# Xharlie/pointnerf

Hardware: AMD Instinct MI355X
Metric: rays/sec (render+bwd) NeRF-synth lego 800^2, K=8, 128 samp/ray (higher is better)
Workload: dtype f32 in / out / accumulate; forward GEMM operands as 2 x f16 planes (22-bit) on the f16 MFMA, 3 products per multiply-add; input-gradient GEMMs: f16 leading product + e4m3 cross terms (csrc/mixq.h), 2 product equivalents; weight-gradient GEMM operands as one f16 plane each

## Files before the change

include/pnerf.h:

```cpp
#ifndef PNERF_H
#define PNERF_H
#include <stddef.h>
#include <stdint.h>

#ifdef __cplusplus
extern "C" {
#endif

#define PNERF_E_INVAL   (-1)
#define PNERF_E_WS      (-2)
#define PNERF_E_LAUNCH  (-3)
#define PNERF_E_UNSUP   (-4)

#define PNERF_MAX_K 16

typedef struct pnerf_grid_params {
    float ranges[6];
    float vsize[3];
    int32_t vdim[3];
    int32_t kernel_size[3];
    int32_t query_size[3];
    int32_t P;
    int32_t max_o;
    float radius;
} pnerf_grid_params;

enum { PNERF_GI_N_IN_GRID = 0, PNERF_GI_N_OCC = 1, PNERF_GI_MAX_CNT = 2, PNERF_GI_CELL0 = 3,
       PNERF_GI_FIRST_IDX = 4, PNERF_GI_OSTART_OFF = 5 , PNERF_GI_LEN = 8 };

int pnerf_version(void);
const char *pnerf_arch(void);

size_t pnerf_grid_workspace_bytes(const pnerf_grid_params *gp, int n_points);
int pnerf_grid_build(const pnerf_grid_params *gp, const float *d_xyz, int n_points,
                     void *d_grid_ws, size_t ws_bytes, void *stream);
int pnerf_grid_info(const void *d_grid_ws, int32_t *host_info, void *stream);
int pnerf_points_minmax(const float *d_xyz, int64_t n_points, float *d_out6, void *stream);

size_t pnerf_query_workspace_bytes(int R, int SR);
int pnerf_query(const pnerf_grid_params *gp, const void *d_grid_ws,
                const float *d_raypos,
                const float *campos3_host, const float *d_raydir, const float *d_mid,
                float near_depth, float far_depth, float jitter, uint64_t seed,
                int R, int D, int SR, int K,
                float *d_sample_loc, int32_t *d_sample_pidx, int32_t *d_sample_nn,
                int32_t *d_ray_hit, int32_t *d_valid_list, int32_t *d_counters,
                void *d_query_ws, size_t ws_bytes, void *stream);

int pnerf_gather_rows(const float *d_src, int n_src, int width, const int32_t *d_idx, int64_t n_idx,
                      float *d_dst, void *stream);
int pnerf_scatter_add_rows(const float *d_grad_rows, const int32_t *d_idx, int64_t n_idx, int width,
                           float *d_grad_src, int n_src, void *stream);

int pnerf_zero_one_blocks(int64_t n_idx);
int pnerf_zero_one_forward(const float *d_conf, int n_points, const int32_t *d_idx, int64_t n_idx, float eps,
                           float *d_partial, void *stream);
int pnerf_zero_one_backward(const float *d_conf, int n_points, const int32_t *d_idx, int64_t n_idx, float eps,
                            const float *d_gscale, float *d_grad_conf, void *stream);
int pnerf_zero_one_forward_rays(const float *d_conf, int n_points, const int32_t *d_idx, const int32_t *d_ray_hit, int R, int slots_per_ray, float eps,
                                float *d_partial, void *stream);
int pnerf_zero_one_backward_rays(const float *d_conf, int n_points, const int32_t *d_idx, const int32_t *d_ray_hit, int R, int slots_per_ray, float eps,
                                 const float *d_gscale, float *d_grad_conf, void *stream);
int pnerf_color_loss_blocks(int R);
int pnerf_color_loss_forward_rays(const float *d_ray_color, const float *d_gt, const int32_t *d_ray_hit, int R, float *d_partial, void *stream);
int pnerf_color_loss_backward_rays(const float *d_ray_color, const float *d_gt, const int32_t *d_ray_hit, int R, const float *d_gscale,
                                   float *d_grad_ray_color, void *stream);


#define PNERF_MLP_NTENSORS 18
int pnerf_mlp_layout(int feat_dim, int64_t *offsets );
size_t pnerf_mlp_packed_bytes(void);
int pnerf_mlp_pack(const float *d_params, void *d_packed, void *stream);

typedef struct pnerf_camera {
    float campos[3];
    float camrot[9];
    float rw2c[9];
    float vsize_z;
    int32_t raydist_mode_unit;
    float bg[3];
    int32_t has_bg;
} pnerf_camera;

typedef struct pnerf_points {
    const float *xyz;
    const float *embedding;
    const float *conf;
    const float *dir;
    const float *color;
    int32_t n, feat_dim;
} pnerf_points;

typedef struct pnerf_point_grads {
    float *embedding, *conf, *dir, *color;
    void *ready_event;
    const float *zero_one_gscale;
    float zero_one_eps;
    float *xyz;
} pnerf_point_grads;

size_t pnerf_agg_saved_bytes(int64_t n_valid_samples, int K);
size_t pnerf_agg_workspace_bytes(int64_t n_valid_max, int K);
size_t pnerf_render_backward_workspace_bytes(int R, int SR);

int pnerf_render_forward(const pnerf_camera *cam, const pnerf_points *pts, const void *d_packed_mlp,
                         const float *d_params, const float *d_raydir, const float *d_sample_loc, const int32_t *d_sample_pidx,
                         const int32_t *d_sample_nn, const int32_t *d_valid_list, const int32_t *d_counters,
                         int R, int SR, int K,
                         float *d_decoded, float *d_weight, float *d_ray_color, float *d_opacity,
                         float *d_bg_trans, float *d_blend_w,
                         void *d_saved, int64_t n_valid_max, void *d_ws, size_t ws_bytes, void *stream);

int pnerf_set_inference_products(int n);

int pnerf_set_wgrad_planes(int n);
int pnerf_set_cross_terms(int bits);
int pnerf_set_cross_terms_where(int mask);

int pnerf_render_backward(const pnerf_camera *cam, const pnerf_points *pts, const void *d_packed_mlp,
                          const float *d_params,
                          const float *d_raydir, const float *d_sample_loc, const int32_t *d_sample_pidx,
                          const int32_t *d_sample_nn, const int32_t *d_valid_list, const int32_t *d_counters,
                          int R, int SR, int K, int64_t n_valid,
                          const float *d_decoded, const float *d_weight, const float *d_opacity,
                          const float *d_grad_ray_color,
                          void *d_saved, float *d_grad_params, const pnerf_point_grads *pg,
                          void *d_ws, size_t ws_bytes, void *stream);


size_t pnerf_compact_workspace_bytes(int64_t n);
int pnerf_touched_flags(const int32_t *d_pidx, int64_t n, int32_t n_points, int32_t *d_flags, void *stream);
int pnerf_compact_valid(const int32_t *d_nn, int64_t n, int32_t *d_list, int32_t *d_counters, void *d_ws, size_t ws_bytes, void *stream);

int pnerf_agg_forward(const pnerf_camera *cam, const pnerf_points *pts, const void *d_packed_mlp, const float *d_params,
                      const float *d_raydir, const float *d_sample_loc, const float *d_xyz_pers, const float *d_loc_pers,
                      const int32_t *d_sample_pidx, const int32_t *d_valid_list, const int32_t *d_counters,
                      int R, int SR, int K, float *d_decoded, float *d_weight,
                      void *d_saved, int64_t n_valid_max, void *d_ws, size_t ws_bytes, void *stream);
int pnerf_agg_backward(const pnerf_camera *cam, const pnerf_points *pts, const void *d_packed_mlp, const float *d_params,
                       const float *d_raydir, const float *d_sample_loc, const int32_t *d_sample_pidx,
                       const int32_t *d_valid_list, const int32_t *d_counters, int R, int SR, int K, int64_t n_valid,
                       const float *d_decoded, const float *d_weight, const float *d_grad_decoded,
                       void *d_saved, float *d_grad_params, const pnerf_point_grads *pg, void *d_ws, size_t ws_bytes, void *stream);

int pnerf_raymarch_forward(const float *d_ray_dist, const uint8_t *d_ray_valid, const float *d_features, const float *bg3_host,
                           int R, int SR, float *d_ray_color, float *d_opacity, float *d_acc_trans, float *d_blend_w,
                           float *d_bg_trans, void *stream);
int pnerf_raymarch_backward(const float *d_ray_dist, const uint8_t *d_ray_valid, const float *d_features, const float *bg3_host,
                            int R, int SR, const float *d_grad_ray_color, float *d_grad_features, void *stream);

int pnerf_adam_step(float *d_param, const float *d_grad, float *d_exp_avg, float *d_exp_avg_sq, int64_t n,
                    double lr, double beta1, double beta2, double eps, int64_t step, void *stream);
typedef struct pnerf_adam_tensor {
    float *param; const float *grad; float *exp_avg; float *exp_avg_sq;
    int64_t n; double lr; int64_t step;
} pnerf_adam_tensor;
int pnerf_adam_step_multi(const pnerf_adam_tensor *tensors, int count, double beta1, double beta2, double eps, void *stream);

size_t pnerf_voxel_downsample_workspace_bytes(int64_t n_points, int rx, int ry, int rz);
int pnerf_voxel_downsample(const float *d_xyz, int64_t n_points, const float *space_min3_host, const float *vox_size3_host,
                           int rx, int ry, int rz, float *d_centroid, int32_t *d_grid_idx, int64_t *d_min_idx, int32_t *d_counts,
                           void *d_ws, size_t ws_bytes, void *stream);

#define PNERF_EX2D_MAX_VIEWS 8
#define PNERF_EX2D_MAX_MAPS 32
typedef struct pnerf_view_desc {
    float c2w[16];
    float w2c[16];
    float intrinsic[9];
    int32_t has_w2c;
} pnerf_view_desc;
typedef struct pnerf_map_desc {
    const float *d_map;
    int32_t view;
    int32_t C, H, W;
    int32_t out_col;
    int32_t is_color;
    int32_t first_of_view;
} pnerf_map_desc;
size_t pnerf_extract_2d_workspace_bytes(int64_t n_points, int n_views, int HD, int WD, int depth_occ);
int pnerf_extract_2d(const float *d_cam_xyz, int64_t n_points, const pnerf_view_desc *views, int n_views, const pnerf_map_desc *maps,
                     int n_maps, int HD, int WD, int depth_occ, float tolerate, float *d_feats, int feat_cols, float *d_colors,
                     int color_cols, uint8_t *d_mask, void *d_ws, size_t ws_bytes, void *stream);
int pnerf_point_dirs(const float *d_cam_xyz, int64_t n_points, const float *cam_pos_cam_host, int n_views, const float *rot1_host9,
                     const float *rot2_host9, float *d_dirs, void *stream);

int pnerf_debug_mfma_f16(const void *d_a, const void *d_b, float *d_out, void *stream);
int pnerf_debug_mix_gemm(const float *d_w, int K, const float *d_x, void *d_img, float *d_out, void *stream);
int pnerf_debug_mfma_rate(int mode, int iters, float *d_scratch, double *flop_out, void *stream);
int pnerf_debug_uniform(uint64_t seed, uint64_t first, int64_t n, float *d_out, void *stream);
int pnerf_debug_split(const float *d_x, int64_t n, void *d_h, void *d_m, int sat, void *stream);
int pnerf_debug_pe(const float *d_x, int64_t n, int nfreq, float *d_out, void *stream);

int pnerf_prof_enable(int on);
int pnerf_prof_kernel_count(void);
const char *pnerf_prof_kernel_name(int id);
int pnerf_prof_collect(double *total_ms, int64_t *launches);

#ifdef __cplusplus
}
#endif
#endif
```

pointnerf_amd/_lib.py:

```python
import ctypes
import os

import torch

_HERE = os.path.dirname(os.path.abspath(__file__))
LIB_PATH = os.path.join(_HERE, "libpnerf_hip.so")

c_int, c_i64, c_f32, c_void_p, c_size_t = ctypes.c_int, ctypes.c_int64, ctypes.c_float, ctypes.c_void_p, ctypes.c_size_t

PNERF_MAX_K = 16
GI_N_IN_GRID, GI_N_OCC, GI_MAX_CNT, GI_CELL0, GI_FIRST_IDX, GI_LEN = 0, 1, 2, 3, 4, 8
MLP_NTENSORS = 18

ERRORS = {-1: "PNERF_E_INVAL (bad argument)", -2: "PNERF_E_WS (workspace too small)",
          -3: "PNERF_E_LAUNCH (HIP launch/runtime error)", -4: "PNERF_E_UNSUP (unsupported configuration)"}


class GridParams(ctypes.Structure):
    _fields_ = [("ranges", c_f32 * 6), ("vsize", c_f32 * 3), ("vdim", ctypes.c_int32 * 3),
                ("kernel_size", ctypes.c_int32 * 3), ("query_size", ctypes.c_int32 * 3),
                ("P", ctypes.c_int32), ("max_o", ctypes.c_int32), ("radius", c_f32)]


class Camera(ctypes.Structure):
    _fields_ = [("campos", c_f32 * 3), ("camrot", c_f32 * 9), ("rw2c", c_f32 * 9), ("vsize_z", c_f32),
                ("raydist_mode_unit", ctypes.c_int32), ("bg", c_f32 * 3), ("has_bg", ctypes.c_int32)]


class Points(ctypes.Structure):
    _fields_ = [("xyz", c_void_p), ("embedding", c_void_p), ("conf", c_void_p), ("dir", c_void_p),
                ("color", c_void_p), ("n", ctypes.c_int32), ("feat_dim", ctypes.c_int32)]


class AdamTensor(ctypes.Structure):
    _fields_ = [("param", c_void_p), ("grad", c_void_p), ("exp_avg", c_void_p), ("exp_avg_sq", c_void_p),
                ("n", ctypes.c_int64), ("lr", ctypes.c_double), ("step", ctypes.c_int64)]


class ViewDesc(ctypes.Structure):
    _fields_ = [("c2w", c_f32 * 16), ("w2c", c_f32 * 16), ("intrinsic", c_f32 * 9), ("has_w2c", ctypes.c_int32)]


class MapDesc(ctypes.Structure):
    _fields_ = [("d_map", c_void_p), ("view", ctypes.c_int32), ("C", ctypes.c_int32), ("H", ctypes.c_int32), ("W", ctypes.c_int32),
                ("out_col", ctypes.c_int32), ("is_color", ctypes.c_int32), ("first_of_view", ctypes.c_int32)]


class PointGrads(ctypes.Structure):
    _fields_ = [("embedding", c_void_p), ("conf", c_void_p), ("dir", c_void_p), ("color", c_void_p), ("ready_event", c_void_p),
                ("zero_one_gscale", c_void_p), ("zero_one_eps", c_f32), ("xyz", c_void_p)]


PROTOTYPES = {
    "pnerf_version": (c_int, []),
    "pnerf_arch": (ctypes.c_char_p, []),
    "pnerf_grid_workspace_bytes": (c_size_t, [ctypes.POINTER(GridParams), c_int]),
    "pnerf_grid_build": (c_int, [ctypes.POINTER(GridParams), c_void_p, c_int, c_void_p, c_size_t, c_void_p]),
    "pnerf_grid_info": (c_int, [c_void_p, ctypes.POINTER(ctypes.c_int32), c_void_p]),
    "pnerf_points_minmax": (c_int, [c_void_p, c_i64, c_void_p, c_void_p]),
    "pnerf_query_workspace_bytes": (c_size_t, [c_int, c_int]),
    "pnerf_query": (c_int, [ctypes.POINTER(GridParams), c_void_p, c_void_p, ctypes.POINTER(c_f32), c_void_p, c_void_p,
                            c_f32, c_f32, c_f32, ctypes.c_uint64, c_int, c_int, c_int, c_int,
                            c_void_p, c_void_p, c_void_p, c_void_p, c_void_p, c_void_p, c_void_p, c_size_t, c_void_p]),
    "pnerf_gather_rows": (c_int, [c_void_p, c_int, c_int, c_void_p, c_i64, c_void_p, c_void_p]),
    "pnerf_scatter_add_rows": (c_int, [c_void_p, c_void_p, c_i64, c_int, c_void_p, c_int, c_void_p]),
    "pnerf_zero_one_blocks": (c_int, [c_i64]),
    "pnerf_zero_one_forward": (c_int, [c_void_p, c_int, c_void_p, c_i64, c_f32, c_void_p, c_void_p]),
    "pnerf_zero_one_backward": (c_int, [c_void_p, c_int, c_void_p, c_i64, c_f32, c_void_p, c_void_p, c_void_p]),
    "pnerf_color_loss_blocks": (c_int, [c_int]),
    "pnerf_color_loss_forward_rays": (c_int, [c_void_p, c_void_p, c_void_p, c_int, c_void_p, c_void_p]),
    "pnerf_color_loss_backward_rays": (c_int, [c_void_p, c_void_p, c_void_p, c_int, c_void_p, c_void_p, c_void_p]),
    "pnerf_zero_one_forward_rays": (c_int, [c_void_p, c_int, c_void_p, c_void_p, c_int, c_int, c_f32, c_void_p, c_void_p]),
    "pnerf_zero_one_backward_rays": (c_int, [c_void_p, c_int, c_void_p, c_void_p, c_int, c_int, c_f32, c_void_p, c_void_p, c_void_p]),
    "pnerf_voxel_downsample_workspace_bytes": (c_size_t, [c_i64, c_int, c_int, c_int]),
    "pnerf_voxel_downsample": (c_int, [c_void_p, c_i64, c_void_p, c_void_p, c_int, c_int, c_int, c_void_p, c_void_p, c_void_p, c_void_p, c_void_p, c_size_t, c_void_p]),
    "pnerf_extract_2d_workspace_bytes": (c_size_t, [c_i64, c_int, c_int, c_int, c_int]),
    "pnerf_extract_2d": (c_int, [c_void_p, c_i64, ctypes.POINTER(ViewDesc), c_int, ctypes.POINTER(MapDesc), c_int, c_int, c_int, c_int, c_f32,
                                 c_void_p, c_int, c_void_p, c_int, c_void_p, c_void_p, c_size_t, c_void_p]),
    "pnerf_point_dirs": (c_int, [c_void_p, c_i64, ctypes.POINTER(c_f32), c_int, ctypes.POINTER(c_f32), ctypes.POINTER(c_f32), c_void_p, c_void_p]),
    "pnerf_adam_step": (c_int, [c_void_p, c_void_p, c_void_p, c_void_p, c_i64, ctypes.c_double, ctypes.c_double, ctypes.c_double, ctypes.c_double, c_i64, c_void_p]),
    "pnerf_adam_step_multi": (c_int, [ctypes.POINTER(AdamTensor), c_int, ctypes.c_double, ctypes.c_double, ctypes.c_double, c_void_p]),
    "pnerf_mlp_layout": (c_int, [c_int, ctypes.POINTER(c_i64)]),
    "pnerf_mlp_packed_bytes": (c_size_t, []),
    "pnerf_mlp_pack": (c_int, [c_void_p, c_void_p, c_void_p]),
    "pnerf_agg_saved_bytes": (c_size_t, [c_i64, c_int]),
    "pnerf_agg_workspace_bytes": (c_size_t, [c_i64, c_int]),
    "pnerf_render_backward_workspace_bytes": (c_size_t, [c_int, c_int]),
    "pnerf_render_forward": (c_int, [ctypes.POINTER(Camera), ctypes.POINTER(Points), c_void_p, c_void_p,
                                     c_void_p, c_void_p, c_void_p, c_void_p, c_void_p, c_void_p,
                                     c_int, c_int, c_int,
                                     c_void_p, c_void_p, c_void_p, c_void_p, c_void_p, c_void_p,
                                     c_void_p, c_i64, c_void_p, c_size_t, c_void_p]),
    "pnerf_set_inference_products": (c_int, [c_int]),
    "pnerf_set_wgrad_planes": (c_int, [c_int]),
    "pnerf_set_cross_terms": (c_int, [c_int]),
    "pnerf_set_cross_terms_where": (c_int, [c_int]),
    "pnerf_compact_workspace_bytes": (c_size_t, [c_i64]),
    "pnerf_touched_flags": (c_int, [c_void_p, c_i64, c_int, c_void_p, c_void_p]),
    "pnerf_compact_valid": (c_int, [c_void_p, c_i64, c_void_p, c_void_p, c_void_p, c_size_t, c_void_p]),
    "pnerf_agg_forward": (c_int, [ctypes.POINTER(Camera), ctypes.POINTER(Points), c_void_p, c_void_p,
                                  c_void_p, c_void_p, c_void_p, c_void_p, c_void_p, c_void_p, c_void_p,
                                  c_int, c_int, c_int, c_void_p, c_void_p, c_void_p, c_i64, c_void_p, c_size_t, c_void_p]),
    "pnerf_agg_backward": (c_int, [ctypes.POINTER(Camera), ctypes.POINTER(Points), c_void_p, c_void_p,
                                   c_void_p, c_void_p, c_void_p, c_void_p, c_void_p, c_int, c_int, c_int, c_i64,
                                   c_void_p, c_void_p, c_void_p, c_void_p, c_void_p, ctypes.POINTER(PointGrads),
                                   c_void_p, c_size_t, c_void_p]),
    "pnerf_raymarch_forward": (c_int, [c_void_p, c_void_p, c_void_p, ctypes.POINTER(c_f32), c_int, c_int,
                                       c_void_p, c_void_p, c_void_p, c_void_p, c_void_p, c_void_p]),
    "pnerf_raymarch_backward": (c_int, [c_void_p, c_void_p, c_void_p, ctypes.POINTER(c_f32), c_int, c_int,
                                        c_void_p, c_void_p, c_void_p]),
    "pnerf_debug_mfma_f16": (c_int, [c_void_p, c_void_p, c_void_p, c_void_p]),
    "pnerf_debug_mix_gemm": (c_int, [c_void_p, c_int, c_void_p, c_void_p, c_void_p, c_void_p]),
    "pnerf_debug_mfma_rate": (c_int, [c_int, c_int, c_void_p, ctypes.POINTER(ctypes.c_double), c_void_p]),
    "pnerf_debug_uniform": (c_int, [ctypes.c_uint64, ctypes.c_uint64, c_i64, c_void_p, c_void_p]),
    "pnerf_debug_split": (c_int, [c_void_p, c_i64, c_void_p, c_void_p, c_int, c_void_p]),
    "pnerf_debug_pe": (c_int, [c_void_p, c_i64, c_int, c_void_p, c_void_p]),
    "pnerf_prof_enable": (c_int, [c_int]),
    "pnerf_prof_kernel_count": (c_int, []),
    "pnerf_prof_kernel_name": (ctypes.c_char_p, [c_int]),
    "pnerf_prof_collect": (c_int, [ctypes.POINTER(ctypes.c_double), ctypes.POINTER(c_i64)]),
    "pnerf_render_backward": (c_int, [ctypes.POINTER(Camera), ctypes.POINTER(Points), c_void_p, c_void_p,
                                      c_void_p, c_void_p, c_void_p, c_void_p, c_void_p, c_void_p,
                                      c_int, c_int, c_int, c_i64,
                                      c_void_p, c_void_p, c_void_p, c_void_p,
                                      c_void_p, c_void_p, ctypes.POINTER(PointGrads),
                                      c_void_p, c_size_t, c_void_p]),
}

_lib = None


def lib():
    global _lib
    if _lib is None:
        if not os.path.exists(LIB_PATH):
            raise RuntimeError(
                "pointnerf_amd: %s not found. Build it with `python -c 'import __graft_entry__ as g; g.build()'` "
                "(hipcc --offload-arch=gfx950). There is no CPU/PyTorch fallback for this path." % LIB_PATH)
        handle = ctypes.CDLL(LIB_PATH)
        for name, (res, args) in PROTOTYPES.items():
            try:
                fn = getattr(handle, name)
            except AttributeError as e:
                raise RuntimeError("pointnerf_amd: libpnerf_hip.so lacks symbol %s (stale build?)" % name) from e
            fn.restype, fn.argtypes = res, args
        _lib = handle
    return _lib


def check(rc, what):
    if rc != 0:
        raise RuntimeError("pointnerf_amd: %s failed: %s" % (what, ERRORS.get(rc, rc)))
```

pointnerf_amd/csrc/aggregate.hip:

```cpp
#include "mixq.h"
#include <stdlib.h>

extern "C" int pnerf_mlp_layout(int feat_dim, int64_t *offsets) {
    if (feat_dim != PN_F || !offsets) return PNERF_E_UNSUP;
    const int64_t o[PNERF_MLP_NTENSORS + 1] = {PO_W1, PO_B1, PO_W2, PO_B2, PO_W3, PO_B3, PO_W4, PO_B4, PO_W5, PO_B5,
                                               PO_WC1, PO_BC1, PO_WC2, PO_BC2, PO_WC3, PO_BC3, PO_WC4, PO_BC4, PO_TOTAL};
    for (int i = 0; i <= PNERF_MLP_NTENSORS; ++i) offsets[i] = o[i];
    return 0;
}
extern "C" size_t pnerf_mlp_packed_bytes(void) { return (size_t)PKX_END; }

namespace {
struct PackHDesc { int src, ld, trans, Mreal, Kreal, NCH, MB, dst; };
struct PackHTable { PackHDesc d[15]; };
__global__ __launch_bounds__(256) void k_pack_h(PackHTable t, const float *__restrict__ params, char *__restrict__ packed) {
    const PackHDesc d = t.d[blockIdx.y];
    const int total = d.NCH * d.MB * 64;
    for (int e = blockIdx.x * 256 + threadIdx.x; e < total; e += gridDim.x * 256) {
        const int lane = e & 63, mb = (e >> 6) % d.MB, c = (e >> 6) / d.MB;
        const int m = 32 * mb + (lane & 31), k0 = 16 * c + 8 * (lane >> 5);
        unsigned h[4], lo[4];
#pragma unroll
        for (int j = 0; j < 4; ++j) {
            float v[2];
#pragma unroll
            for (int i = 0; i < 2; ++i) {
                const int k = k0 + 2 * j + i;
                v[i] = 0.f;
                if (m < d.Mreal && k < d.Kreal) v[i] = d.trans ? params[d.src + k * d.ld + m] : params[d.src + m * d.ld + k];
            }
            pn_split2_sat(v[0], v[1], h[j], lo[j]);
        }
        uint4 *o = reinterpret_cast<uint4 *>(packed + d.dst) + ((size_t)(c * d.MB + mb) * 2) * 64 + lane;
        o[0] = make_uint4(h[0], h[1], h[2], h[3]);
        o[64] = make_uint4(lo[0], lo[1], lo[2], lo[3]);
    }
}

struct PackMDesc { int src, ld, trans, Mreal, Kreal, NT, MB, dst; };
struct PackMTable { PackMDesc d[9]; };
__global__ __launch_bounds__(256) void k_pack_mix(PackMTable t, const float *__restrict__ params, char *__restrict__ packed) {
    pn_mode_saturate();
    const PackMDesc d = t.d[blockIdx.y];
    auto W = [&](int m, int k) -> float { return (m < d.Mreal && k < d.Kreal) ? (d.trans ? params[d.src + k * d.ld + m] : params[d.src + m * d.ld + k]) : 0.f; };
    uint4 *img = reinterpret_cast<uint4 *>(packed + d.dst);
    unsigned *sc = reinterpret_cast<unsigned *>(img + PN_MIMG_U4(d.NT, d.MB));
    const int nsup = PN_MIX_NS * d.MB * 64, ntail = d.NT * d.MB * 64;
    for (int e = blockIdx.x * 256 + threadIdx.x; e < nsup + ntail; e += gridDim.x * 256) {
        if (e < nsup) {
            const int lane = e & 63, mb = (e >> 6) % d.MB, s = (e >> 6) / d.MB, m = 32 * mb + (lane & 31), hf = lane >> 5;
            uint4 *o = img + ((size_t)(s * d.MB + mb) * 8) * 64 + lane;
#pragma unroll
            for (int r = 0; r < 4; ++r) {
                const int k0 = 64 * s + 16 * r + 8 * hf;
                unsigned h[4], lo[4];
#pragma unroll
                for (int j = 0; j < 4; ++j) pn_split2_rne(W(m, k0 + 2 * j), W(m, k0 + 2 * j + 1), h[j], lo[j]);
                o[r * 64] = make_uint4(h[0], h[1], h[2], h[3]);
            }
            unsigned scw = 0u;
#pragma unroll
            for (int j = 0; j < 2; ++j) {
                float wh[16], wm[16], mx = 0.f;
#pragma unroll
                for (int i = 0; i < 32; ++i) {
                    const float w = W(m, 64 * s + 32 * j + i);
#ifdef PN_EMU
                    const float wc = fmaxf(fminf(w, 65504.f), -65504.f);
#else
                    const float wc = w;
#endif
                    const float h = (float)(_Float16)wc;
                    mx = fmaxf(mx, fmaxf(fabsf(h), fabsf(w - h) * 2048.f));
                }
#pragma unroll
                for (int i = 0; i < 16; ++i) {
                    const float w = W(m, 8 * (8 * s + 4 * j + 2 * hf + (i >> 3)) + (i & 7));
#ifdef PN_EMU
                    const float wc = fmaxf(fminf(w, 65504.f), -65504.f);
#else
                    const float wc = w;
#endif
                    wh[i] = (float)(_Float16)wc; wm[i] = w - wh[i];
                }
                int ex = 0;
                const float fr = frexpf(mx, &ex);
                int be = mx > 0.f ? (fr > 0.875f ? ex - 8 : ex - 9) : 0;
                be = be < -100 ? -100 : (be > 100 ? 100 : be);
                const float sh = __uint_as_float((unsigned)(be + 127) << 23), sm = __uint_as_float((unsigned)(be + 127 - 11) << 23);
                scw |= (unsigned)(be + 127) << (8 * j);
#pragma unroll
                for (int tt = 0; tt < 2; ++tt) {
                    unsigned q[4];
#pragma unroll
                    for (int w4 = 0; w4 < 4; ++w4) {
                        const float *src = (w4 < 2 ? wm : wh) + 8 * tt + 4 * (w4 & 1);
                        const float scl = w4 < 2 ? sm : sh;
                        pn_s2 r = {0, 0};
                        r = __builtin_amdgcn_cvt_scalef32_pk_fp8_f32(r, src[0], src[1], scl, false);
                        r = __builtin_amdgcn_cvt_scalef32_pk_fp8_f32(r, src[2], src[3], scl, true);
                        q[w4] = __builtin_bit_cast(unsigned, r);
                    }
                    o[(4 + 2 * j + tt) * 64] = make_uint4(q[0], q[1], q[2], q[3]);
                }
            }
            sc[(size_t)(s * d.MB + mb) * 64 + lane] = scw;
        } else {
            const int e2 = e - nsup, lane = e2 & 63, mb = (e2 >> 6) % d.MB, tc = (e2 >> 6) / d.MB, m = 32 * mb + (lane & 31);
            const int k0 = 256 + 16 * tc + 8 * (lane >> 5);
            unsigned h[4], lo[4];
#pragma unroll
            for (int j = 0; j < 4; ++j) pn_split2_sat(W(m, k0 + 2 * j), W(m, k0 + 2 * j + 1), h[j], lo[j]);
            uint4 *o = img + (size_t)PN_MIX_NS * d.MB * 8 * 64 + ((size_t)(tc * d.MB + mb) * 2) * 64 + lane;
            o[0] = make_uint4(h[0], h[1], h[2], h[3]);
            o[64] = make_uint4(lo[0], lo[1], lo[2], lo[3]);
        }
    }
}
}

extern "C" int pnerf_mlp_pack(const float *d_params, void *d_packed, void *stream) {
    if (!d_params || !d_packed) return PNERF_E_INVAL;
    PackHTable th = {{
        {PO_W1, PN_IN1, 0, PN_H, PN_IN1, 18, 8, PKH_F1},
        {PO_W2, PN_H, 0, PN_H, PN_H, 16, 8, PKH_F2},
        {PO_W3, PN_IN3, 0, PN_H, PN_IN3, 17, 8, PKH_F3},
        {PO_W4, PN_H, 0, PN_H, PN_H, 16, 8, PKH_F4},
        {PO_W4, PN_H, 1, PN_H, PN_H, 16, 8, PKH_D4},
        {PO_W3, PN_IN3, 1, PN_IN3, PN_H, 16, 9, PKH_D3},
        {PO_W2, PN_H, 1, PN_H, PN_H, 16, 8, PKH_D2},
        {PO_W1, PN_IN1, 1, 32 * PN_MB_D1, PN_H, 16, PN_MB_D1, PKH_D1},
        {PO_WC1, PN_INC, 0, PN_HC, PN_INC, 18, 4, PKH_FC1},
        {PO_WC2, PN_HC, 0, PN_HC, PN_HC, 8, 4, PKH_FC2},
        {PO_WC3, PN_HC, 0, PN_HC, PN_HC, 8, 4, PKH_FC3},
        {PO_WC3, PN_HC, 1, PN_HC, PN_HC, 8, 4, PKH_DC3},
        {PO_WC2, PN_HC, 1, PN_HC, PN_HC, 8, 4, PKH_DC2},
        {PO_WC1, PN_INC, 1, PN_H, PN_HC, 8, 8, PKH_DC1},
        {PO_W1 + 32 * PN_MB_D1, PN_IN1, 1, PN_IN1 - 32 * PN_MB_D1, PN_H, 16, 2, PKH_D1T},
    }};
    PnProfScope prof(PNK_PACK, (hipStream_t)stream);
    hipLaunchKernelGGL(k_pack_h, dim3(40, 15), dim3(256), 0, (hipStream_t)stream, th, d_params, (char *)d_packed);
    PackMTable tm = {{
        {PO_W1, PN_IN1, 0, PN_H, PN_IN1, 2, 8, PKM_F1},
        {PO_W2, PN_H, 0, PN_H, PN_H, 0, 8, PKM_F2},
        {PO_W3, PN_IN3, 0, PN_H, PN_IN3, 1, 8, PKM_F3},
        {PO_W4, PN_H, 0, PN_H, PN_H, 0, 8, PKM_F4},
        {PO_W4, PN_H, 1, PN_H, PN_H, 0, 8, PKM_D4},
        {PO_W3, PN_IN3, 1, PN_IN3, PN_H, 0, 9, PKM_D3},
        {PO_W2, PN_H, 1, PN_H, PN_H, 0, 8, PKM_D2},
        {PO_W1, PN_IN1, 1, 32 * PN_MB_D1, PN_H, 0, PN_MB_D1, PKM_D1},
        {PO_W1 + 32 * PN_MB_D1, PN_IN1, 1, PN_IN1 - 32 * PN_MB_D1, PN_H, 0, 2, PKM_D1T},
    }};
    hipLaunchKernelGGL(k_pack_mix, dim3(12, 9), dim3(256), 0, (hipStream_t)stream, tm, d_params, (char *)d_packed);
    PN_CHECK_LAUNCH();
    return 0;
}

namespace {
template <int NT>
__global__ __launch_bounds__(256) void k_debug_mix_gemm(const float *__restrict__ x, const char *__restrict__ img, float *__restrict__ out) {
    extern __shared__ __attribute__((aligned(16))) char smem_d[];
    pn_mode_saturate();
    constexpr int K = 256 + 16 * NT;
    char *X = smem_d;
    const int tid = threadIdx.x, lane = tid & 63, wave = __builtin_amdgcn_readfirstlane(tid >> 6);
    for (int e = tid; e < PN_TILE * (K / 4); e += 256) {
        const int row = e / (K / 4), col = 4 * (e % (K / 4));
        const float4 v = *reinterpret_cast<const float4 *>(x + row * K + col);
        if (col < 256) pn_xq_store4(X, row, col, v.x, v.y, v.z, v.w);
        else pn_xt_store4(X, row, col, v.x, v.y, v.z, v.w);
    }
    __syncthreads();
    f32x16 acc[2][2];
#pragma unroll
    for (int i = 0; i < 2; ++i)
#pragma unroll
        for (int j = 0; j < 2; ++j)
#pragma unroll
            for (int r = 0; r < 16; ++r) acc[i][j][r] = 0.f;
    pn_gemm_mix<PN_MIX_NS, NT, 8, 2>(X, img, 2 * wave, lane, acc);
#pragma unroll
    for (int fb = 0; fb < 2; ++fb)
#pragma unroll
        for (int rb = 0; rb < 2; ++rb)
#pragma unroll
            for (int g = 0; g < 4; ++g)
#pragma unroll
                for (int i = 0; i < 4; ++i) out[(32 * rb + (lane & 31)) * PN_H + pn_d_feat(2 * wave + fb, g, lane) + i] = acc[fb][rb][4 * g + i];
}
}

extern "C" int pnerf_debug_mix_gemm(const float *d_w, int K, const float *d_x, void *d_img, float *d_out, void *stream) {
    if (!d_w || !d_x || !d_img || !d_out || (K != 256 && K != 272 && K != 288)) return PNERF_E_INVAL;
    hipStream_t s = (hipStream_t)stream;
    const int NT = (K - 256) / 16;
    PackMTable tm = {{{0, K, 0, PN_H, K, NT, 8, 0}}};
    hipLaunchKernelGGL(k_pack_mix, dim3(12, 1), dim3(256), 0, s, tm, d_w, (char *)d_img);
    const void *fn = NT == 0 ? (const void *)k_debug_mix_gemm<0> : NT == 1 ? (const void *)k_debug_mix_gemm<1> : (const void *)k_debug_mix_gemm<2>;
    if (hipFuncSetAttribute(fn, hipFuncAttributeMaxDynamicSharedMemorySize, PN_XBYTES) != hipSuccess) return PNERF_E_LAUNCH;
    if (NT == 0) hipLaunchKernelGGL(k_debug_mix_gemm<0>, dim3(1), dim3(256), PN_XBYTES, s, d_x, (const char *)d_img, d_out);
    else if (NT == 1) hipLaunchKernelGGL(k_debug_mix_gemm<1>, dim3(1), dim3(256), PN_XBYTES, s, d_x, (const char *)d_img, d_out);
    else hipLaunchKernelGGL(k_debug_mix_gemm<2>, dim3(1), dim3(256), PN_XBYTES, s, d_x, (const char *)d_img, d_out);
    PN_CHECK_LAUNCH();
    return 0;
}

namespace {
__global__ __launch_bounds__(64) void k_debug_mfma_f16(const uint4 *__restrict__ a, const uint4 *__restrict__ b, float *__restrict__ d) {
    f32x16 acc;
#pragma unroll
    for (int r = 0; r < 16; ++r) acc[r] = 0.f;
    acc = __builtin_amdgcn_mfma_f32_32x32x16_f16(__builtin_bit_cast(pn_h8, a[threadIdx.x]), __builtin_bit_cast(pn_h8, b[threadIdx.x]), acc, 0, 0, 0);
#pragma unroll
    for (int r = 0; r < 16; ++r) d[threadIdx.x * 16 + r] = acc[r];
}
}
namespace {
__global__ __launch_bounds__(256) void k_debug_split(const float *__restrict__ x, long long n, unsigned *__restrict__ h, unsigned *__restrict__ m, int sat) {
    for (long long i = (long long)blockIdx.x * 256 + threadIdx.x; 2 * i < n; i += (long long)gridDim.x * 256) {
        unsigned hh, mm;
        if (sat) pn_split2_sat(x[2 * i], x[2 * i + 1], hh, mm);
        else pn_split2(x[2 * i], x[2 * i + 1], hh, mm);
        h[i] = hh; m[i] = mm;
    }
}
}
extern "C" int pnerf_debug_split(const float *d_x, int64_t n, void *d_h, void *d_m, int sat, void *stream) {
    if (!d_x || !d_h || !d_m || n < 0 || (n & 1)) return PNERF_E_INVAL;
    if (n == 0) return 0;
    hipLaunchKernelGGL(k_debug_split, dim3(64), dim3(256), 0, (hipStream_t)stream, d_x, (long long)n, (unsigned *)d_h, (unsigned *)d_m, sat);
    PN_CHECK_LAUNCH();
    return 0;
}

namespace {
template <int NF> __global__ __launch_bounds__(256) void k_debug_pe(const float *__restrict__ x, long long n, float *__restrict__ out) {
    for (long long i = (long long)blockIdx.x * 256 + threadIdx.x; i < n; i += (long long)gridDim.x * 256) {
        float s[NF], c[NF];
        pn_pe_octaves<NF>(x[i], s, c);
#pragma unroll
        for (int f = 0; f < NF; ++f) { out[(i * NF + f) * 2] = s[f]; out[(i * NF + f) * 2 + 1] = c[f]; }
    }
}
}
extern "C" int pnerf_debug_pe(const float *d_x, int64_t n, int nfreq, float *d_out, void *stream) {
    if (!d_x || !d_out || n < 0 || nfreq < 1 || nfreq > 5) return PNERF_E_INVAL;
    if (n == 0) return 0;
    hipStream_t s = (hipStream_t)stream;
    switch (nfreq) {
        case 1: hipLaunchKernelGGL(k_debug_pe<1>, dim3(64), dim3(256), 0, s, d_x, (long long)n, d_out); break;
        case 2: hipLaunchKernelGGL(k_debug_pe<2>, dim3(64), dim3(256), 0, s, d_x, (long long)n, d_out); break;
        case 3: hipLaunchKernelGGL(k_debug_pe<3>, dim3(64), dim3(256), 0, s, d_x, (long long)n, d_out); break;
        case 4: hipLaunchKernelGGL(k_debug_pe<4>, dim3(64), dim3(256), 0, s, d_x, (long long)n, d_out); break;
        default: hipLaunchKernelGGL(k_debug_pe<5>, dim3(64), dim3(256), 0, s, d_x, (long long)n, d_out); break;
    }
    PN_CHECK_LAUNCH();
    return 0;
}

extern "C" int pnerf_debug_mfma_f16(const void *d_a, const void *d_b, float *d_out, void *stream) {
    if (!d_a || !d_b || !d_out) return PNERF_E_INVAL;
    hipLaunchKernelGGL(k_debug_mfma_f16, dim3(1), dim3(64), 0, (hipStream_t)stream, (const uint4 *)d_a, (const uint4 *)d_b, d_out);
    PN_CHECK_LAUNCH();
    return 0;
}

size_t pn_saved_bytes(long long n_valid, int K, long long *rows_out, long long *samples_out) {
    const int TS = pn_tile_samples(K);
    const long long tiles = (n_valid + TS - 1) / TS + 2 * PN_NCLS + 1;
    const long long rows = tiles * PN_TILE;
    const long long samples = ((tiles * TS + PN_CTILE - 1) / PN_CTILE + 1) * PN_CTILE;
    if (rows_out) *rows_out = rows;
    if (samples_out) *samples_out = samples;
    size_t b = 0;
    b += 2 * pn_align((size_t)rows / 8 * PN_NF1 * 16) + 2 * pn_align((size_t)rows / 8 * PN_H * 16);
    b += 4 * pn_align((size_t)rows / 8 * PN_H * 16) + pn_align((size_t)rows * 32 * 32);
    b += pn_align((size_t)rows * 4) + pn_align((size_t)rows * 16) + pn_align((size_t)tiles * 3 * 512 * 4) + pn_align(16);
    b += pn_cls_bytes(samples);
    b += 2 * pn_align((size_t)samples * PN_H * 4) + pn_align((size_t)samples * PN_HC * 4);
    b += pn_align((size_t)samples / 8 * PN_NF1 * 16) + 2 * pn_align((size_t)samples / 8 * PN_HC * 16);
    b += 3 * pn_align((size_t)samples / 8 * PN_HC * 16) + pn_align((size_t)samples / PN_CTILE * 2 * 256 * 4);
    if (pn_wgrad_planes() == 2) {
        b += 2 * pn_align((size_t)rows / 8 * PN_NF1 * 16) + 6 * pn_align((size_t)rows / 8 * PN_H * 16);
        b += pn_align((size_t)samples / 8 * PN_NF1 * 16) + 5 * pn_align((size_t)samples / 8 * PN_HC * 16);
    }
    return b;
}

PnSaved pn_saved_carve(void *base, long long n_valid, int K) {
    PnSaved s;
    size_t total = pn_saved_bytes(n_valid, K, &s.rows, &s.samples);
    PnCarver cv(base, total);
    const size_t rg = (size_t)s.rows / 8;
    s.x0k = cv.take<uint4>(rg * PN_NF1); s.h2k = cv.take<uint4>(rg * PN_NF1);
    s.h1k = cv.take<uint4>(rg * PN_H); s.h3k = cv.take<uint4>(rg * PN_H);
    s.dy1k = cv.take<uint4>(rg * PN_H); s.dy2k = cv.take<uint4>(rg * PN_H);
    s.dy3k = cv.take<uint4>(rg * PN_H); s.dy4k = cv.take<uint4>(rg * PN_H);
    s.h4r = cv.take<uint4>((size_t)s.rows * 32 * 2);
    s.arow = cv.take<float>((size_t)s.rows); s.rmeta = cv.take<int4>((size_t)s.rows);
    s.lmask = cv.take<unsigned>((size_t)(s.rows / PN_TILE) * 3 * 512);
    s.gscale = cv.take<unsigned>(4);
    s.fs = cv.take<float>((size_t)s.samples * PN_H); s.dfs = cv.take<float>((size_t)s.samples * PN_H);
    s.c3 = cv.take<float>((size_t)s.samples * PN_HC);
    const size_t rgc = (size_t)s.samples / 8;
    s.xck = cv.take<uint4>(rgc * PN_NF1); s.c1k = cv.take<uint4>(rgc * PN_HC); s.c2k = cv.take<uint4>(rgc * PN_HC);
    s.dc1k = cv.take<uint4>(rgc * PN_HC); s.dc2k = cv.take<uint4>(rgc * PN_HC); s.dc3k = cv.take<uint4>(rgc * PN_HC);
    s.cmask = cv.take<unsigned>((size_t)s.samples / PN_CTILE * 2 * 256);
    s.wg2 = pn_wgrad_planes() == 2 ? 1 : 0;
    s.x0m = s.h1m = s.h2m = s.h3m = s.dy1m = s.dy2m = s.dy3m = s.dy4m = nullptr;
    s.xcm = s.c1m = s.c2m = s.dc1m = s.dc2m = s.dc3m = nullptr;
    if (s.wg2) {
        s.x0m = cv.take<uint4>(rg * PN_NF1); s.h2m = cv.take<uint4>(rg * PN_NF1);
        s.h1m = cv.take<uint4>(rg * PN_H); s.h3m = cv.take<uint4>(rg * PN_H);
        s.dy1m = cv.take<uint4>(rg * PN_H); s.dy2m = cv.take<uint4>(rg * PN_H);
        s.dy3m = cv.take<uint4>(rg * PN_H); s.dy4m = cv.take<uint4>(rg * PN_H);
        s.xcm = cv.take<uint4>(rgc * PN_NF1); s.c1m = cv.take<uint4>(rgc * PN_HC); s.c2m = cv.take<uint4>(rgc * PN_HC);
        s.dc1m = cv.take<uint4>(rgc * PN_HC); s.dc2m = cv.take<uint4>(rgc * PN_HC); s.dc3m = cv.take<uint4>(rgc * PN_HC);
    }
    pn_cls_carve(cv.take<char>(pn_cls_bytes(s.samples)), s.samples, s);
    return s;
}

size_t pn_cls_bytes(long long samples) {
    return pn_align((size_t)samples * 4) + pn_align(PN_CI_WORDS * 4) + pn_align(((size_t)2 * samples + pn_scan_scratch_ints(samples) + 8) * 4);
}
void pn_cls_carve(void *base, long long samples, PnSaved &s) {
    PnCarver cv(base, pn_cls_bytes(samples));
    s.cls_list = cv.take<int>((size_t)samples);
    s.cls_info = cv.take<int>(PN_CI_WORDS);
    s.cls_tmp = cv.take<int>((size_t)2 * samples + pn_scan_scratch_ints(samples) + 8);
}

extern "C" size_t pnerf_agg_saved_bytes(int64_t n_valid_samples, int K) {
    if (K <= 0 || K > PNERF_MAX_K || n_valid_samples < 0) return 0;
    return pn_saved_bytes(n_valid_samples, K, nullptr, nullptr);
}

namespace {
constexpr int TPR = PN_TPR;
constexpr int EPT = PN_F / TPR;

struct FwdArgs {
    pnerf_camera cam;
    const float *xyz, *emb, *conf, *dir, *color;
    const float *params;
    const float4 *packed;
    const float *raydir, *sample_loc;
    const float *xyz_pers, *loc_pers;
    const int *pidx, *valid_list, *counters;
    const int *cls_list, *cls_info;
    int cls, Kstride;
    int save_x0;
    int R, SR, K, TS;
    long long cap_samples;
    float *decoded, *weight;
    PnSaved sv;
};

__device__ __forceinline__ void rot3(const float *M , float x, float y, float z, bool transpose, float &ox, float &oy, float &oz) {
    if (!transpose) { ox = x * M[0] + y * M[3] + z * M[6]; oy = x * M[1] + y * M[4] + z * M[7]; oz = x * M[2] + y * M[5] + z * M[8]; }
    else { ox = x * M[0] + y * M[1] + z * M[2]; oy = x * M[3] + y * M[4] + z * M[5]; oz = x * M[6] + y * M[7] + z * M[8]; }
}

template <int N> __device__ __forceinline__ float group_sum(float v) {
#pragma unroll
    for (int off = 1; off < N; off <<= 1) v += __shfl_xor(v, off, 64);
    return v;
}

namespace {
struct ClsArgs { const int *valid_list, *counters, *pidx; int K, n, ncls; int kc[PN_NCLS], ts[PN_NCLS]; };

__global__ void k_cls_flags(ClsArgs c, int which, int *__restrict__ flags) {
    const int vs = blockIdx.x * blockDim.x + threadIdx.x;
    if (vs >= c.n) return;
    const int Ns = c.counters[0] < c.n ? c.counters[0] : c.n;
    int f = 0;
    if (vs < Ns) {
        const long long si = c.valid_list[vs];
        int hv = 0;
        for (int k = 0; k < c.K; ++k)
            if (c.pidx[si * c.K + k] >= 0) hv = k + 1;
        int cl = 0;
        for (int j = 1; j < c.ncls; ++j)
            if (hv <= c.kc[j]) cl = j;
        f = cl == which;
    }
    flags[vs] = f;
}

__global__ void k_cls_gather(ClsArgs c, int which, const int *__restrict__ pos, const int *__restrict__ count, int *__restrict__ cls_list,
                             int *__restrict__ info) {
    const int n = *count, base = info[PN_CI_VBASE + which];
    for (int i = blockIdx.x * blockDim.x + threadIdx.x; i < n; i += gridDim.x * blockDim.x) cls_list[base + i] = c.valid_list[pos[i]];
    if (blockIdx.x == 0 && threadIdx.x == 0) {
        const int tiles = (n + c.ts[which] - 1) / c.ts[which], tb = info[PN_CI_TBASE + which];
        info[PN_CI_COUNT + which] = n;
        if (which + 1 < PN_NCLS) { info[PN_CI_VBASE + which + 1] = base + n; info[PN_CI_TBASE + which + 1] = tb + tiles + 1; }
        info[PN_CI_TILES] = tb + tiles + 1;
    }
}

__global__ void k_cls_zero_gaps(PnSaved sv, int ncls, int save_x0) {
    const int c = blockIdx.y;
    if (c >= ncls) return;
    if ((blockIdx.x == 0 && !save_x0) || (blockIdx.x == 8 && save_x0)) return;
    const long long gap = (c + 1 < PN_NCLS ? sv.cls_info[PN_CI_TBASE + c + 1] : sv.cls_info[PN_CI_TILES]) - 1;
    uint4 *arrs[9] = {sv.x0k, sv.h2k, sv.h1k, sv.h3k, sv.dy1k, sv.dy2k, sv.dy3k, sv.dy4k, sv.x0k};
    uint4 *arrm[9] = {sv.x0m, sv.h2m, sv.h1m, sv.h3m, sv.dy1m, sv.dy2m, sv.dy3m, sv.dy4m, nullptr};
    const int which = blockIdx.x;
    const int nf = which == 8 ? 64 : which < 2 ? PN_NF1 : PN_H;
    uint4 *p = arrs[which] + gap * 8 * nf;
    for (int i = threadIdx.x; i < 8 * nf; i += blockDim.x) p[i] = make_uint4(0u, 0u, 0u, 0u);
    if (sv.wg2 && arrm[which]) {
        uint4 *pm = arrm[which] + gap * 8 * nf;
        for (int i = threadIdx.x; i < 8 * nf; i += blockDim.x) pm[i] = make_uint4(0u, 0u, 0u, 0u);
    }
}
}

}

int pn_class_slots(int K, int kc[PN_NCLS]) {
    if (K % 4 == 0) { kc[0] = K; kc[1] = K / 2; kc[2] = K / 4; return 3; }
    kc[0] = K; kc[1] = kc[2] = 0;
    return 1;
}

int pn_classify(const PnSaved &sv, const int32_t *d_valid_list, const int32_t *d_counters, const int32_t *d_pidx, int K, long long n_valid,
                bool train, bool save_x0, hipStream_t s) {
    ClsArgs c;
    c.valid_list = d_valid_list; c.counters = d_counters; c.pidx = d_pidx; c.K = K; c.n = (int)n_valid;
    c.ncls = pn_class_slots(K, c.kc);
    for (int j = 0; j < PN_NCLS; ++j) c.ts[j] = c.kc[j] > 0 ? pn_tile_samples(c.kc[j]) : 1;
    if (hipMemsetAsync(sv.cls_info, 0, PN_CI_WORDS * sizeof(int), s) != hipSuccess) return PNERF_E_LAUNCH;
    if (n_valid <= 0) return 0;
    int *flags = sv.cls_tmp, *pos = flags + n_valid, *cnt = pos + n_valid, *scratch = cnt + 8;
    PnProfScope prof(PNK_COMPACT, s);
    for (int j = 0; j < c.ncls; ++j) {
        hipLaunchKernelGGL(k_cls_flags, dim3(pn_cdiv(n_valid, 256)), dim3(256), 0, s, c, j, flags);
        int rc = pn_compact_gt0_i32(flags, n_valid, pos, cnt, scratch, s);
        if (rc) return rc;
        hipLaunchKernelGGL(k_cls_gather, dim3(256), dim3(256), 0, s, c, j, pos, cnt, sv.cls_list, sv.cls_info);
    }
    if (train) hipLaunchKernelGGL(k_cls_zero_gaps, dim3(9, c.ncls), dim3(256), 0, s, sv, c.ncls, save_x0 ? 1 : 0);
    PN_CHECK_LAUNCH();
    return 0;
}


namespace {

constexpr int FL_EX = PN_XBYTES, FL_W5 = FL_EX + PN_TILE * 8 * 4, FL_ROW = FL_W5 + PN_H * 4, FL_BYTES = FL_ROW + 4 * PN_TILE * 4;
static_assert(2 * FL_BYTES <= 160 * 1024, "two forward workgroups must fit the 160 KB LDS");

struct FGather {
    float4 e0, e1;
    float px, py, pz, lx, ly, lz, cf;
    float ppx, ppy, ppz, lpx, lpy, lpz;
    float dxv, dyv, dzv, cx, cy, cz, rx, ry, rz;
};

__device__ __forceinline__ int f_sample_of(const FwdArgs &a, long long tile, int row, int Ns, unsigned kinv) {
    const int ls = pn_row_div(row, kinv);
    const long long vs = tile * a.TS + ls;
    return (ls < a.TS && vs < Ns) ? a.valid_list[vs] : -1;
}

template <bool PERS>
__device__ __forceinline__ void f_gather(const FwdArgs &a, FGather &G, int si_, int p_, int q) {
    const int p = p_ > 0 ? p_ : 0, si = si_ > 0 ? si_ : 0;
    const float *ep = a.emb + (long long)p * PN_F + EPT * q;
    G.e0 = *reinterpret_cast<const float4 *>(ep); G.e1 = *reinterpret_cast<const float4 *>(ep + 4);
    G.px = a.xyz[3 * p]; G.py = a.xyz[3 * p + 1]; G.pz = a.xyz[3 * p + 2];
    G.lx = a.sample_loc[(long long)si * 3]; G.ly = a.sample_loc[(long long)si * 3 + 1]; G.lz = a.sample_loc[(long long)si * 3 + 2];
    if (PERS) {
        G.ppx = a.xyz_pers[3 * p]; G.ppy = a.xyz_pers[3 * p + 1]; G.ppz = a.xyz_pers[3 * p + 2];
        G.lpx = a.loc_pers[(long long)si * 3]; G.lpy = a.loc_pers[(long long)si * 3 + 1]; G.lpz = a.loc_pers[(long long)si * 3 + 2];
    }
    G.cf = a.conf[p];
    if (q == 0) {
        const int r = si / a.SR;
        G.dxv = a.dir[3 * p]; G.dyv = a.dir[3 * p + 1]; G.dzv = a.dir[3 * p + 2];
        G.cx = a.color[3 * p]; G.cy = a.color[3 * p + 1]; G.cz = a.color[3 * p + 2];
        G.rx = a.raydir[3 * r]; G.ry = a.raydir[3 * r + 1]; G.rz = a.raydir[3 * r + 2];
    }
}

template <bool PERS, bool MIX = false, bool HR = false>
__device__ __forceinline__ void f_build(const FwdArgs &a, const FGather &G, char *X, float *exb, float *wraw, int *sidx, int si, int p, int row, int q) {
    const float dwx = G.px - G.lx, dwy = G.py - G.ly, dwz = G.pz - G.lz;
    float ppx, ppy, pcz, spx, spy, scz;
    if (PERS) {
        ppx = G.ppx; ppy = G.ppy; pcz = G.ppz; spx = G.lpx; spy = G.lpy; scz = G.lpz;
    } else {
        float pcx, pcy, scx, scy;
        rot3(a.cam.camrot, G.px - a.cam.campos[0], G.py - a.cam.campos[1], G.pz - a.cam.campos[2], false, pcx, pcy, pcz);
        rot3(a.cam.camrot, G.lx - a.cam.campos[0], G.ly - a.cam.campos[1], G.lz - a.cam.campos[2], false, scx, scy, scz);
        ppx = pcx / pcz; ppy = pcy / pcz; spx = scx / scz; spy = scy / scz;
    }
    float d0, d1, d2;
    rot3(a.cam.rw2c, dwx, dwy, dwz, true, d0, d1, d2);
    const float d3 = ppx * pcz - spx * scz, d4 = ppy * pcz - spy * scz, d5 = pcz - scz;
    const float da = q == 0 ? d0 : q == 1 ? d1 : q == 2 ? d2 : d3;
    const float db = q == 0 ? d4 : d5;
    const float e[8] = {G.e0.x, G.e0.y, G.e0.z, G.e0.w, G.e1.x, G.e1.y, G.e1.z, G.e1.w};
    if (MIX) {
        pn_xq_store4(X, row, EPT * q, e[0], e[1], e[2], e[3]);
        pn_xq_store4(X, row, EPT * q + 4, e[4], e[5], e[6], e[7]);
#pragma unroll
        for (int i = 0; i < 8; i += 2) {
            const int col = PN_F + (EPT * q + i) * 6;
            float s0[3], c0[3], s1[3], c1[3];
            pn_pe_octaves<3>(e[i], s0, c0);
            pn_pe_octaves<3>(e[i + 1], s1, c1);
            pn_xq_store4(X, row, col, s0[0], c0[0], s0[1], c0[1]);
            pn_xq_store4(X, row, col + 4, s0[2], c0[2], s1[0], c1[0]);
            pn_xq_store4(X, row, col + 8, s1[1], c1[1], s1[2], c1[2]);
        }
    } else {
    if (HR) { pn_xt_store4(X, row, EPT * q, e[0], e[1], e[2], e[3]); pn_xt_store4(X, row, EPT * q + 4, e[4], e[5], e[6], e[7]); }
    else { pn_x_store4<false>(X, row, EPT * q, e[0], e[1], e[2], e[3]); pn_x_store4<false>(X, row, EPT * q + 4, e[4], e[5], e[6], e[7]); }
#pragma unroll
    for (int i = 0; i < 8; ++i) {
        const int dd = EPT * q + i;
        float s[3], c[3];
        pn_pe_octaves<3>(e[i], s, c);
        if (HR) {
            pn_xt_store2(X, row, PN_F + dd * 6, s[0], c[0]);
            pn_xt_store2(X, row, PN_F + dd * 6 + 2, s[1], c[1]);
            pn_xt_store2(X, row, PN_F + dd * 6 + 4, s[2], c[2]);
        } else {
            pn_x_store2(X, row, PN_F + dd * 6, s[0], c[0]);
            pn_x_store2(X, row, PN_F + dd * 6 + 2, s[1], c[1]);
            pn_x_store2(X, row, PN_F + dd * 6 + 4, s[2], c[2]);
        }
    }
    }
#pragma unroll
    for (int j = 0; j < 2; ++j) {
        const int comp = q + 4 * j;
        if (comp < 6) {
            float s[5], c[5];
            pn_pe_octaves<5>(j == 0 ? da : db, s, c);
#pragma unroll
            for (int f = 0; f < 5; ++f) {
                if (MIX) pn_xa_store2(X, row, PN_F * 7 + (comp * 5 + f) * 2, s[f], c[f]);
                else if (HR) pn_xt_store2(X, row, PN_F * 7 + (comp * 5 + f) * 2, s[f], c[f]);
                else pn_x_store2(X, row, PN_F * 7 + (comp * 5 + f) * 2, s[f], c[f]);
            }
        }
    }
    if (q == 3) {
        if (MIX || HR) pn_xt_store4(X, row, PN_ONES1, 1.f, 0.f, 0.f, 0.f);
        else pn_x_store4<false>(X, row, PN_ONES1, 1.f, 0.f, 0.f, 0.f);
    }
    if (q == 0) {
        float vx, vy, vz, qx, qy, qz;
        rot3(a.cam.rw2c, G.rx, G.ry, G.rz, true, vx, vy, vz);
        rot3(a.cam.rw2c, G.dxv, G.dyv, G.dzv, true, qx, qy, qz);
        float *ex = exb + row * 8;
        *reinterpret_cast<float4 *>(ex) = make_float4(G.cx, G.cy, G.cz, qx - vx);
        *reinterpret_cast<float4 *>(ex + 4) = make_float4(qy - vy, qz - vz, qx * vx + qy * vy + qz * vz, 1.f);
        wraw[row] = p >= 0 ? 1.0f / fmaxf(sqrtf(dwx * dwx + dwy * dwy + dwz * dwz), 1e-6f) : 0.f;
        sidx[row] = si;
    }
}

__device__ __forceinline__ void f_acc_bias(const float *__restrict__ bias, int wave, int lane, f32x16 (&acc)[PN_NFB][2]) {
#pragma unroll
    for (int fb = 0; fb < PN_NFB; ++fb)
#pragma unroll
        for (int g = 0; g < 4; ++g) {
            const float4 b = *reinterpret_cast<const float4 *>(bias + pn_d_feat(PN_NFB * wave + fb, g, lane));
#pragma unroll
            for (int rb = 0; rb < 2; ++rb) { acc[fb][rb][4 * g] = b.x; acc[fb][rb][4 * g + 1] = b.y; acc[fb][rb][4 * g + 2] = b.z; acc[fb][rb][4 * g + 3] = b.w; }
        }
}
template <bool BITS, bool MIX = false, bool HR = false>
__device__ __forceinline__ void f_epilogue(const f32x16 (&acc)[PN_NFB][2], char *X, int wave, int lane, unsigned (&mw)[PN_NFB]) {
#pragma unroll
    for (int fb = 0; fb < PN_NFB; ++fb) mw[fb] = 0u;
#pragma unroll
    for (int fb = 0; fb < PN_NFB; ++fb)
#pragma unroll
        for (int rb = 0; rb < 2; ++rb)
#pragma unroll
            for (int g = 0; g < 4; ++g) {
                const int f0 = pn_d_feat(PN_NFB * wave + fb, g, lane);
                float v[4] = {acc[fb][rb][4 * g], acc[fb][rb][4 * g + 1], acc[fb][rb][4 * g + 2], acc[fb][rb][4 * g + 3]};
                if (BITS) {
#pragma unroll
                    for (int i = 0; i < 4; ++i) mw[fb] = __builtin_amdgcn_alignbit(mw[fb], __float_as_uint(v[i]), 31);
                }
#pragma unroll
                for (int i = 0; i < 4; ++i) v[i] = fmaxf(v[i], 0.01f * v[i]);
                if (MIX) pn_xq_store4(X, 32 * rb + (lane & 31), f0, v[0], v[1], v[2], v[3]);
                else if (HR) pn_xt_store4(X, 32 * rb + (lane & 31), f0, v[0], v[1], v[2], v[3]);
                else pn_x_store4<false>(X, 32 * rb + (lane & 31), f0, v[0], v[1], v[2], v[3]);
            }
}
__device__ __forceinline__ void f_store_masks(unsigned *__restrict__ lmask, long long gtile, int layer, int wave, int lane, const unsigned (&mw)[PN_NFB]) {
#pragma unroll
    for (int fb = 0; fb < PN_NFB; ++fb) lmask[((gtile * 3 + layer) * 8 + PN_NFB * wave + fb) * 64 + lane] = mw[fb];
}

__device__ __forceinline__ void f_acc_zero(f32x16 (&acc)[PN_NFB][2]) {
#pragma unroll
    for (int i = 0; i < PN_NFB; ++i)
#pragma unroll
        for (int j = 0; j < 2; ++j)
#pragma unroll
            for (int r = 0; r < 16; ++r) acc[i][j][r] = 0.f;
}

__device__ __forceinline__ float pn_softplus(float x) {
#ifdef PN_EMU
    return x > 20.f ? x : log1pf(expf(x));
#else
    return x > 20.f ? x : __logf(1.0f + __expf(x));
#endif
}

template <int KC, bool TRAIN>
__device__ __forceinline__ void f_tail(const FwdArgs &a, const char *X, const float *w5s, const float *wrow, const int *sidx, float b5,
                                       long long tile, long long gtile, int tid, float *wraw = nullptr) {
    constexpr int NS = KC == 0 ? 1 : 8 / (KC == 0 ? 1 : KC);
    const int lane = tid & 63, cg = tid & 31, r0 = 8 * (tid >> 5);
    const float4 wa = *reinterpret_cast<const float4 *>(w5s + 8 * cg), wb = *reinterpret_cast<const float4 *>(w5s + 8 * cg + 4);
    float pa[8];
    float4 fa[NS], fb[NS];
#pragma unroll
    for (int j = 0; j < NS; ++j) fa[j] = fb[j] = make_float4(0.f, 0.f, 0.f, 0.f);
#pragma unroll
    for (int i = 0; i < 8; ++i) {
        const int r = r0 + i;
        const uint4 h = *reinterpret_cast<const uint4 *>(X + r * PN_XRS + cg * 16);
        const uint4 m = *reinterpret_cast<const uint4 *>(X + PN_XPLANE + r * PN_XRS + cg * 16);
        if (TRAIN) {
            pn_f4 th = {__uint_as_float(h.x), __uint_as_float(h.y), __uint_as_float(h.z), __uint_as_float(h.w)};
            pn_f4 tm = {__uint_as_float(m.x), __uint_as_float(m.y), __uint_as_float(m.z), __uint_as_float(m.w)};
            PN_STREAM_STORE(th, reinterpret_cast<pn_f4 *>(a.sv.h4r + (gtile * PN_TILE + r) * 32 + cg));
            PN_STREAM_STORE(tm, reinterpret_cast<pn_f4 *>(a.sv.h4r + (a.sv.rows + gtile * PN_TILE + r) * 32 + cg));
        }
        float s = 0.f;
        s = pn_fma2_lo(h.x, m.x, wa.x, s); s = pn_fma2_hi(h.x, m.x, wa.y, s); s = pn_fma2_lo(h.y, m.y, wa.z, s); s = pn_fma2_hi(h.y, m.y, wa.w, s);
        s = pn_fma2_lo(h.z, m.z, wb.x, s); s = pn_fma2_hi(h.z, m.z, wb.y, s); s = pn_fma2_lo(h.w, m.w, wb.z, s); s = pn_fma2_hi(h.w, m.w, wb.w, s);
        pa[i] = s;
        if (KC != 0) {
            const float w = wrow[r];
            float4 &f0 = fa[i / (KC == 0 ? 1 : KC)], &f1 = fb[i / (KC == 0 ? 1 : KC)];
            f0.x = pn_fma2_lo(h.x, m.x, w, f0.x); f0.y = pn_fma2_hi(h.x, m.x, w, f0.y); f0.z = pn_fma2_lo(h.y, m.y, w, f0.z); f0.w = pn_fma2_hi(h.y, m.y, w, f0.w);
            f1.x = pn_fma2_lo(h.z, m.z, w, f1.x); f1.y = pn_fma2_hi(h.z, m.z, w, f1.y); f1.z = pn_fma2_lo(h.w, m.w, w, f1.z); f1.w = pn_fma2_hi(h.w, m.w, w, f1.w);
        }
    }
#pragma unroll
    for (int j = 0; j < (KC == 0 ? 0 : NS); ++j) {
        const long long vs = tile * (PN_TILE / (KC == 0 ? 1 : KC)) + (r0 / (KC == 0 ? 1 : KC)) + j;
        if (vs < a.cap_samples) {
            *reinterpret_cast<float4 *>(a.sv.fs + vs * PN_H + 8 * cg) = fa[j];
            *reinterpret_cast<float4 *>(a.sv.fs + vs * PN_H + 8 * cg + 4) = fb[j];
        }
    }
    {
        const bool b4 = lane & 16, b3 = lane & 8, b2 = lane & 4;
#pragma unroll
        for (int j = 0; j < 4; ++j) { const float send = b4 ? pa[j] : pa[j + 4], keep = b4 ? pa[j + 4] : pa[j]; pa[j] = keep + __shfl_xor(send, 16, 64); }
#pragma unroll
        for (int j = 0; j < 2; ++j) { const float send = b3 ? pa[j] : pa[j + 2], keep = b3 ? pa[j + 2] : pa[j]; pa[j] = keep + __shfl_xor(send, 8, 64); }
        { const float send = b2 ? pa[0] : pa[1], keep = b2 ? pa[1] : pa[0]; pa[0] = keep + __shfl_xor(send, 4, 64); }
        pa[0] += __shfl_xor(pa[0], 2, 64);
        pa[0] += __shfl_xor(pa[0], 1, 64);
        const int i = ((lane >> 4) & 1) * 4 + ((lane >> 3) & 1) * 2 + ((lane >> 2) & 1), r = r0 + i;
        const float x = pa[0] + b5 - 1.0f;
        float sg = pn_softplus(x) * wrow[r];
        if (TRAIN && (lane & 3) == 0) a.sv.arow[gtile * PN_TILE + r] = x;
        if (KC == 0) {
            if ((lane & 3) == 0) wraw[r] = sg;
            return;
        }
        if (KC >= 2) sg += __shfl_xor(sg, 4, 64);
        if (KC >= 4) sg += __shfl_xor(sg, 8, 64);
        if (KC >= 8) sg += __shfl_xor(sg, 16, 64);
        if ((lane & 3) == 0 && (i % (KC == 0 ? 1 : KC)) == 0) {
            const int si = sidx[r];
            if (si >= 0) a.decoded[(long long)si * 4] = sg;
        }
    }
}

#ifdef PN_PHASE_TRACE
PN_TR_DECL(pn_trace_fwd);
#endif
template <bool TRAIN, bool PERS, int NP, bool WG2 = false>
__global__ __launch_bounds__(PN_NTHR, PN_NW / 2) void k_agg_forward(FwdArgs a) {
    constexpr bool MIX = NP == 4;
    constexpr bool HR = !MIX;
    constexpr bool HC = TRAIN && !WG2;
    constexpr int NPC = MIX ? 3 : NP;
    static_assert(!(MIX && WG2), "the two-plane weight-gradient mode keeps f16x3.h's arithmetic everywhere");
    pn_mode_saturate();
    extern __shared__ __attribute__((aligned(16))) char smem_f[];
    char *X = smem_f;
    float *exb = reinterpret_cast<float *>(smem_f + FL_EX), *w5s = reinterpret_cast<float *>(smem_f + FL_W5);
    float *wraw = reinterpret_cast<float *>(smem_f + FL_ROW), *wrow = wraw + PN_TILE, *wnrm = wrow + PN_TILE;
    int *sidx = reinterpret_cast<int *>(wnrm + PN_TILE);
    const int tid0 = threadIdx.x;
    const int K = a.K, TS = a.TS;
    const unsigned kinv = pn_kinv(K);
    const int Ns = a.cls_info[PN_CI_COUNT + a.cls];
    const long long vb = a.cls_info[PN_CI_VBASE + a.cls], tb = a.cls_info[PN_CI_TBASE + a.cls];
    a.valid_list = a.cls_list + vb; a.cap_samples = Ns;
    a.sv.fs += vb * PN_H;
    const long long ntiles = ((long long)Ns + TS - 1) / TS;
    const float *P = a.params;
    const char *img = reinterpret_cast<const char *>(a.packed);
    if (tid0 < PN_H) w5s[tid0] = P[PO_W5 + tid0];
    const float b5 = P[PO_B5];
    const long long stride = gridDim.x, tile_first = blockIdx.x, tile_last = ntiles;
    if (tile_first >= tile_last) return;

    long long tile = tile_first;
    int si0, si1, si2, p0, p1;
    FGather G;
    {
        const int row = tid0 / TPR, q = tid0 % TPR, k = row - pn_row_div(row, kinv) * K;
        si0 = f_sample_of(a, tile, row, Ns, kinv); si1 = tile + stride < tile_last ? f_sample_of(a, tile + stride, row, Ns, kinv) : -1;
        si2 = tile + 2 * stride < tile_last ? f_sample_of(a, tile + 2 * stride, row, Ns, kinv) : -1;
        p0 = si0 >= 0 ? a.pidx[(long long)si0 * a.Kstride + k] : -1;
        p1 = si1 >= 0 ? a.pidx[(long long)si1 * a.Kstride + k] : -1;
        f_gather<PERS>(a, G, si0, p0, q);
    }

    f32x16 acc[PN_NFB][2];
    PN_TR_ITER_DECL;
    for (; tile < tile_last; tile += stride) {
        PN_TR_ITER_NEXT;
        int tid = threadIdx.x;
        asm volatile("" : "+v"(tid));
        const int lane = tid & 63, wave = __builtin_amdgcn_readfirstlane(tid >> 6);
        const int row = tid / TPR, q = tid % TPR, k = row - pn_row_div(row, kinv) * K;
        const long long gtile = tb + tile;
        PN_LDS_BARRIER();
        PN_TR(pn_trace_fwd, 0); PN_TR_HWID(pn_trace_fwd);
        f_build<PERS, MIX, HR>(a, G, X, exb, wraw, sidx, si0, p0, row, q);
        f_acc_bias(P + PO_B1, wave, lane, acc);
        PnGemmW<18, 8, PN_NFB, PN_WPF, NPC> W1;
        PnMixW<PN_MIX_NS, 2, 8, PN_NFB> M1;
        if constexpr (MIX) M1.prefetch(img + PKM_F1, PN_NFB * wave, lane);
        else W1.prefetch(reinterpret_cast<const uint4 *>(img + PKH_F1), PN_NFB * wave, lane);
        PN_LDS_BARRIER();
        if (q == 0) {
            const int ls = pn_row_div(row, kinv);
            float wn = 0.f, w = 0.f;
            if (si0 >= 0) {
                float sum = 0.f;
                for (int kk = 0; kk < K; ++kk) sum += wraw[ls * K + kk];
                wn = wraw[row] / fmaxf(sum, 1e-8f);
                w = wn * fminf(fmaxf(G.cf, 1e-4f), 1.0f);
                a.weight[(long long)si0 * a.Kstride + k] = wn;
            }
            wnrm[row] = wn; wrow[row] = w;
            if (TRAIN) a.sv.rmeta[gtile * PN_TILE + row] = make_int4(si0, si0 >= 0 ? p0 : -1, __float_as_int(wn), __float_as_int(w));
        }
        unsigned mask[PN_NFB];
        PN_TR(pn_trace_fwd, 1);
        PN_TR(pn_trace_fwd, 2);
        if constexpr (MIX) pn_gemm_mix_run<PN_MIX_NS, 2, 8, PN_NFB>(X, M1, lane, acc);
        else pn_gemm_f16x3_run<18, 8, PN_NFB, PN_WPF, NPC>(X, W1, lane, acc);
        if (TRAIN) {
            if (HC) {
                if (a.save_x0) pn_copy_out_kmajor_h<PN_NF1>(X, a.sv.x0k, gtile * 8, tid);
                else pn_copy_out_kmajor_cols64_h<224>(X, a.sv.x0k, gtile * 8, tid);
            } else if (WG2) pn_copy_out_kmajor<PN_NF1, true>(X, a.sv.x0k, gtile * 8, tid, a.sv.x0m);
            else if (a.save_x0) pn_copy_out_kmajor<PN_NF1, false>(X, a.sv.x0k, gtile * 8, tid);
            else pn_copy_out_kmajor_cols64<224>(X, a.sv.x0k, gtile * 8, tid);
        }
        PN_LDS_BARRIER();
        PN_TR(pn_trace_fwd, 3);
        f_epilogue<TRAIN, MIX, HR>(acc, X, wave, lane, mask);
        if (TRAIN) f_store_masks(a.sv.lmask, gtile, 0, wave, lane, mask);
        f_acc_bias(P + PO_B2, wave, lane, acc);
        PnGemmW<16, 8, PN_NFB, PN_WPF, NPC> W2;
        PnMixW<PN_MIX_NS, 0, 8, PN_NFB> M2;
        if constexpr (MIX) M2.prefetch(img + PKM_F2, PN_NFB * wave, lane);
        else W2.prefetch(reinterpret_cast<const uint4 *>(img + PKH_F2), PN_NFB * wave, lane);
        PN_LDS_BARRIER();
        PN_TR(pn_trace_fwd, 4);
        PN_TR(pn_trace_fwd, 5);
        if constexpr (MIX) pn_gemm_mix_run<PN_MIX_NS, 0, 8, PN_NFB>(X, M2, lane, acc);
        else pn_gemm_f16x3_run<16, 8, PN_NFB, PN_WPF, NPC>(X, W2, lane, acc);
        if (TRAIN) {
            if (HC) pn_copy_out_kmajor_h<PN_H>(X, a.sv.h1k, gtile * 8, tid);
            else pn_copy_out_kmajor<PN_H, WG2>(X, a.sv.h1k, gtile * 8, tid, a.sv.h1m);
        }
        PN_LDS_BARRIER();
        PN_TR(pn_trace_fwd, 6);
        f_epilogue<TRAIN, MIX, HR>(acc, X, wave, lane, mask);
        if (TRAIN) f_store_masks(a.sv.lmask, gtile, 1, wave, lane, mask);
        if (tid < PN_TILE) {
            const float4 u = *reinterpret_cast<const float4 *>(exb + tid * 8), v = *reinterpret_cast<const float4 *>(exb + tid * 8 + 4);
            if (MIX || HR) {
                pn_xt_store4(X, tid, PN_H, u.x, u.y, u.z, u.w);
                pn_xt_store4(X, tid, PN_H + 4, v.x, v.y, v.z, v.w);
                pn_xt_store4(X, tid, PN_H + 8, 0.f, 0.f, 0.f, 0.f);
                pn_xt_store4(X, tid, PN_H + 12, 0.f, 0.f, 0.f, 0.f);
            } else {
                pn_x_store4<false>(X, tid, PN_H, u.x, u.y, u.z, u.w);
                pn_x_store4<false>(X, tid, PN_H + 4, v.x, v.y, v.z, v.w);
                pn_x_store4<false>(X, tid, PN_H + 8, 0.f, 0.f, 0.f, 0.f);
                pn_x_store4<false>(X, tid, PN_H + 12, 0.f, 0.f, 0.f, 0.f);
            }
        }
        f_acc_bias(P + PO_B3, wave, lane, acc);
        PnGemmW<17, 8, PN_NFB, PN_WPF, NPC> W3;
        PnMixW<PN_MIX_NS, 1, 8, PN_NFB> M3;
        if constexpr (MIX) M3.prefetch(img + PKM_F3, PN_NFB * wave, lane);
        else W3.prefetch(reinterpret_cast<const uint4 *>(img + PKH_F3), PN_NFB * wave, lane);
        PN_LDS_BARRIER();
        PN_TR(pn_trace_fwd, 7);
        PN_TR(pn_trace_fwd, 8);
        if constexpr (MIX) pn_gemm_mix_run<PN_MIX_NS, 1, 8, PN_NFB>(X, M3, lane, acc);
        else pn_gemm_f16x3_run<17, 8, PN_NFB, PN_WPF, NPC>(X, W3, lane, acc);
        if (TRAIN) {
            if (HC) pn_copy_out_kmajor_h<PN_NF1>(X, a.sv.h2k, gtile * 8, tid);
            else pn_copy_out_kmajor<PN_NF1, WG2>(X, a.sv.h2k, gtile * 8, tid, a.sv.h2m);
        }
        PN_LDS_BARRIER();
        PN_TR(pn_trace_fwd, 9);
        f_epilogue<TRAIN, MIX, HR>(acc, X, wave, lane, mask);
        if (TRAIN) f_store_masks(a.sv.lmask, gtile, 2, wave, lane, mask);
        f_acc_bias(P + PO_B4, wave, lane, acc);
        PnGemmW<16, 8, PN_NFB, PN_WPF, NPC> W4;
        PnMixW<PN_MIX_NS, 0, 8, PN_NFB> M4;
        if constexpr (MIX) M4.prefetch(img + PKM_F4, PN_NFB * wave, lane);
        else W4.prefetch(reinterpret_cast<const uint4 *>(img + PKH_F4), PN_NFB * wave, lane);
        PN_LDS_BARRIER();
        PN_TR(pn_trace_fwd, 10);
        PN_TR(pn_trace_fwd, 11);
        if constexpr (MIX) pn_gemm_mix_run<PN_MIX_NS, 0, 8, PN_NFB>(X, M4, lane, acc);
        else pn_gemm_f16x3_run<16, 8, PN_NFB, PN_WPF, NPC>(X, W4, lane, acc);
        if (TRAIN) {
            if (HC) pn_copy_out_kmajor_h<PN_H>(X, a.sv.h3k, gtile * 8, tid);
            else pn_copy_out_kmajor<PN_H, WG2>(X, a.sv.h3k, gtile * 8, tid, a.sv.h3m);
        }
        PN_TR(pn_trace_fwd, 12);
        const float cf_cur = G.cf;
        (void)cf_cur;
        const int si_next = si1, p_next = p1;
        if (tile + stride < tile_last) f_gather<PERS>(a, G, si1, p1, q);
        const int p2 = si2 >= 0 ? a.pidx[(long long)si2 * a.Kstride + k] : -1;
        const int si3 = tile + 3 * stride < tile_last ? f_sample_of(a, tile + 3 * stride, row, Ns, kinv) : -1;
        PN_LDS_BARRIER();
        PN_TR(pn_trace_fwd, 13);
        f_epilogue<false>(acc, X, wave, lane, mask);
        PN_LDS_BARRIER();
        PN_TR(pn_trace_fwd, 14);
        if (K == 8 || K == 4 || K == 2 || K == 1) {
            if (K == 8) f_tail<8, TRAIN>(a, X, w5s, wrow, sidx, b5, tile, gtile, tid);
            else if (K == 4) f_tail<4, TRAIN>(a, X, w5s, wrow, sidx, b5, tile, gtile, tid);
            else if (K == 2) f_tail<2, TRAIN>(a, X, w5s, wrow, sidx, b5, tile, gtile, tid);
            else f_tail<1, TRAIN>(a, X, w5s, wrow, sidx, b5, tile, gtile, tid);
            PN_TR(pn_trace_fwd, 15);
        } else {
        f_tail<0, TRAIN>(a, X, w5s, wrow, sidx, b5, tile, gtile, tid, wraw);
        PN_LDS_BARRIER();
        PN_TR(pn_trace_fwd, 15);
        for (int e = tid; e < TS * 32; e += PN_NTHR) {
            const int ls = e >> 5, cg = e & 31;
            float4 f0 = make_float4(0.f, 0.f, 0.f, 0.f), f1 = f0;
            for (int kk = 0; kk < K; ++kk) {
                const int r = ls * K + kk;
                const uint4 h = *reinterpret_cast<const uint4 *>(X + r * PN_XRS + cg * 16);
                const uint4 m = *reinterpret_cast<const uint4 *>(X + PN_XPLANE + r * PN_XRS + cg * 16);
                const float w = wrow[r];
                f0.x = pn_fma2_lo(h.x, m.x, w, f0.x); f0.y = pn_fma2_hi(h.x, m.x, w, f0.y); f0.z = pn_fma2_lo(h.y, m.y, w, f0.z); f0.w = pn_fma2_hi(h.y, m.y, w, f0.w);
                f1.x = pn_fma2_lo(h.z, m.z, w, f1.x); f1.y = pn_fma2_hi(h.z, m.z, w, f1.y); f1.z = pn_fma2_lo(h.w, m.w, w, f1.z); f1.w = pn_fma2_hi(h.w, m.w, w, f1.w);
            }
            const long long vs = tile * TS + ls;
            if (vs < a.cap_samples) {
                *reinterpret_cast<float4 *>(a.sv.fs + vs * PN_H + 8 * cg) = f0;
                *reinterpret_cast<float4 *>(a.sv.fs + vs * PN_H + 8 * cg + 4) = f1;
            }
        }
        if (tid < TS) {
            const int si = sidx[tid * K];
            if (si >= 0) {
                float sg = 0.f;
                for (int kk = 0; kk < K; ++kk) sg += wraw[tid * K + kk];
                a.decoded[(long long)si * 4] = sg;
            }
        }
        }
        si0 = si_next; p0 = p_next; si1 = si2; p1 = p2; si2 = si3;
        PN_TR(pn_trace_fwd, 16);
    }
}

constexpr int CL_W4 = PN_XBYTES, CL_BYTES = CL_W4 + 3 * PN_HC * 4;
static_assert(2 * CL_BYTES <= 160 * 1024, "two colour workgroups must fit the 160 KB LDS");

__device__ __forceinline__ void c_load_bias(const float *__restrict__ bias, int wave, int lane, float4 (&b)[4]) {
#pragma unroll
    for (int g = 0; g < 4; ++g) {
        const float *p = bias + pn_d_feat(wave, g, lane);
        b[g] = make_float4(p[0], p[1], p[2], p[3]);
    }
}
template <bool TRAIN, bool SAVE32>
__device__ __forceinline__ unsigned c_epilogue(const f32x16 (&acc)[2][2], const float4 (&bias)[4], char *X, int wave, int lane, float *__restrict__ save, long long grow0) {
    unsigned mw = 0u;
#pragma unroll
    for (int rb = 0; rb < 2; ++rb)
#pragma unroll
        for (int g = 0; g < 4; ++g) {
            const int f0 = pn_d_feat(wave, g, lane), row = 32 * rb + (lane & 31);
            const float4 b = bias[g];
            float v[4] = {acc[0][rb][4 * g] + b.x, acc[0][rb][4 * g + 1] + b.y, acc[0][rb][4 * g + 2] + b.z, acc[0][rb][4 * g + 3] + b.w};
            if (TRAIN && !SAVE32) {
#pragma unroll
                for (int i = 0; i < 4; ++i) mw = __builtin_amdgcn_alignbit(mw, __float_as_uint(v[i]), 31);
            }
#pragma unroll
            for (int i = 0; i < 4; ++i) v[i] = fmaxf(v[i], 0.01f * v[i]);
            if (TRAIN && SAVE32) {
                pn_f4 t = {v[0], v[1], v[2], v[3]};
                PN_REG_STORE(t, reinterpret_cast<pn_f4 *>(save + (grow0 + row) * PN_HC + f0));
            }
            pn_x_store4<false>(X, row, f0, v[0], v[1], v[2], v[3]);
        }
    return mw;
}
__device__ __forceinline__ void c_acc_zero(f32x16 (&acc)[2][2]) {
#pragma unroll
    for (int j = 0; j < 2; ++j)
#pragma unroll
        for (int r = 0; r < 16; ++r) acc[0][j][r] = 0.f;
}

template <bool TRAIN, int NP, bool WG2 = false>
__global__ __launch_bounds__(256, 2) void k_color_forward(FwdArgs a) {
    extern __shared__ __attribute__((aligned(16))) char smem_c[];
    char *X = smem_c;
    float *w4s = reinterpret_cast<float *>(smem_c + CL_W4);
    const int Ns = a.counters[0] < a.cap_samples ? a.counters[0] : (int)a.cap_samples;
    const float *P = a.params;
    const char *img = reinterpret_cast<const char *>(a.packed);
    for (int i = threadIdx.x; i < 3 * PN_HC; i += 256) w4s[i] = P[PO_WC4 + i];
    const float b40 = P[PO_BC4], b41 = P[PO_BC4 + 1], b42 = P[PO_BC4 + 2];

    f32x16 acc[2][2];
    for (long long tile = blockIdx.x; tile * PN_CTILE < Ns; tile += gridDim.x) {
        int tid = threadIdx.x;
        asm volatile("" : "+v"(tid));
        const int lane = tid & 63, wave = __builtin_amdgcn_readfirstlane(tid >> 6), row = tid >> 2, q = tid & 3;
        const long long grow0 = tile * PN_CTILE, vs = grow0 + row;
        const int si = vs < Ns ? a.valid_list[vs] : -1;
        PnGemmW<18, 4, 1, 7, NP> WC1;
        WC1.prefetch(reinterpret_cast<const uint4 *>(img + PKH_FC1), wave, lane);
        PN_LDS_BARRIER();
        if (si >= 0) {
            const float4 *f = reinterpret_cast<const float4 *>(a.sv.fs + vs * PN_H);
            float4 fv[16];
#pragma unroll
            for (int c = 0; c < 16; ++c) fv[c] = f[4 * c + q];
#pragma unroll
            for (int c = 0; c < 16; ++c) pn_x_store4<false>(X, row, 16 * c + 4 * q, fv[c].x, fv[c].y, fv[c].z, fv[c].w);
            {
                const int r = si / a.SR;
                float v[3], sn[4], cs[4];
                rot3(a.cam.rw2c, a.raydir[3 * r], a.raydir[3 * r + 1], a.raydir[3 * r + 2], true, v[0], v[1], v[2]);
                const float vq = q == 0 ? v[0] : (q == 1 ? v[1] : v[2]);
                pn_pe_octaves<4>(vq, sn, cs);
                if (q < 3) {
                    pn_x_store4<false>(X, row, PN_H + 4 * q, sn[0], sn[1], sn[2], sn[3]);
                    pn_x_store4<false>(X, row, PN_H + 12 + 4 * q, cs[0], cs[1], cs[2], cs[3]);
                } else {
                    pn_x_store4<false>(X, row, PN_H + 24, 0.f, 0.f, 0.f, 0.f);
                    pn_x_store4<false>(X, row, PN_H + 28, 0.f, 0.f, 0.f, 0.f);
                }
            }
        } else {
#pragma unroll
            for (int c = 0; c < 18; ++c) pn_x_store4<false>(X, row, 16 * c + 4 * q, 0.f, 0.f, 0.f, 0.f);
        }
        PN_LDS_BARRIER();
        float4 bias[4];
        if (TRAIN) pn_copy_out_kmajor<PN_NF1, WG2>(X, a.sv.xck, tile * 8, tid, a.sv.xcm);
        c_acc_zero(acc);
        pn_gemm_f16x3_run<18, 4, 1, 7, NP>(X, WC1, lane, acc);
        c_load_bias(P + PO_BC1, wave, lane, bias);
        PN_LDS_BARRIER();
        unsigned mw = c_epilogue<TRAIN, false>(acc, bias, X, wave, lane, nullptr, grow0);
        if (TRAIN) a.sv.cmask[(tile * 2 + 0) * 256 + tid] = mw;
        PnGemmW<8, 4, 1, 7, NP> WC2;
        WC2.prefetch(reinterpret_cast<const uint4 *>(img + PKH_FC2), wave, lane);
        PN_LDS_BARRIER();
        if (TRAIN) pn_copy_out_kmajor<PN_HC, WG2>(X, a.sv.c1k, tile * 8, tid, a.sv.c1m);
        c_acc_zero(acc);
        pn_gemm_f16x3_run<8, 4, 1, 7, NP>(X, WC2, lane, acc);
        c_load_bias(P + PO_BC2, wave, lane, bias);
        PN_LDS_BARRIER();
        mw = c_epilogue<TRAIN, false>(acc, bias, X, wave, lane, nullptr, grow0);
        if (TRAIN) a.sv.cmask[(tile * 2 + 1) * 256 + tid] = mw;
        PnGemmW<8, 4, 1, 7, NP> WC3;
        WC3.prefetch(reinterpret_cast<const uint4 *>(img + PKH_FC3), wave, lane);
        PN_LDS_BARRIER();
        if (TRAIN) pn_copy_out_kmajor<PN_HC, WG2>(X, a.sv.c2k, tile * 8, tid, a.sv.c2m);
        c_acc_zero(acc);
        pn_gemm_f16x3_run<8, 4, 1, 7, NP>(X, WC3, lane, acc);
        c_load_bias(P + PO_BC3, wave, lane, bias);
        PN_LDS_BARRIER();
        c_epilogue<TRAIN, true>(acc, bias, X, wave, lane, a.sv.c3, grow0);
        PN_LDS_BARRIER();
        {
            float o0 = 0.f, o1 = 0.f, o2 = 0.f;
#pragma unroll
            for (int j = 0; j < 4; ++j) {
                const int c0 = q * 32 + 8 * j;
                o0 = pn_x_dot8(X, row, c0, *reinterpret_cast<const float4 *>(w4s + c0), *reinterpret_cast<const float4 *>(w4s + c0 + 4), o0);
                o1 = pn_x_dot8(X, row, c0, *reinterpret_cast<const float4 *>(w4s + PN_HC + c0), *reinterpret_cast<const float4 *>(w4s + PN_HC + c0 + 4), o1);
                o2 = pn_x_dot8(X, row, c0, *reinterpret_cast<const float4 *>(w4s + 2 * PN_HC + c0), *reinterpret_cast<const float4 *>(w4s + 2 * PN_HC + c0 + 4), o2);
            }
            o0 = group_sum<4>(o0); o1 = group_sum<4>(o1); o2 = group_sum<4>(o2);
            if (q == 0 && si >= 0) {
                float *o = a.decoded + (long long)si * 4;
                o[1] = 1.0f / (1.0f + expf(-(o0 + b40))) * 1.002f - 0.001f;
                o[2] = 1.0f / (1.0f + expf(-(o1 + b41))) * 1.002f - 0.001f;
                o[3] = 1.0f / (1.0f + expf(-(o2 + b42))) * 1.002f - 0.001f;
            }
        }
    }
}
}

static int pn_inference_products = 3;
extern "C" int pnerf_set_inference_products(int n) {
    if (n != 2 && n != 3) return PNERF_E_INVAL;
    const int old = pn_inference_products;
    pn_inference_products = n;
    return old;
}

static int pn_wgrad_planes_ = 1;
int pn_wgrad_planes() { return pn_wgrad_planes_; }
extern "C" int pnerf_set_wgrad_planes(int n) {
    if (n != 1 && n != 2) return PNERF_E_INVAL;
    const int old = pn_wgrad_planes_;
    pn_wgrad_planes_ = n;
    return old;
}

static int pn_cross_terms_ = 8;
int pn_cross_terms() { return pn_cross_terms_; }
extern "C" int pnerf_set_cross_terms(int bits) {
    if (bits != 8 && bits != 16) return PNERF_E_INVAL;
    const int old = pn_cross_terms_;
    pn_cross_terms_ = bits;
    return old;
}
#ifndef PN_MIX_DEFAULT_MASK
#define PN_MIX_DEFAULT_MASK 4
#endif
static int pn_mix_mask_ = -1;
int pn_mix_mask() {
    if (pn_mix_mask_ < 0) {
        const char *e = getenv("PNERF_MIX_MASK");
        pn_mix_mask_ = e ? atoi(e) & 7 : PN_MIX_DEFAULT_MASK;
    }
    return pn_cross_terms_ == 8 ? pn_mix_mask_ : 0;
}
extern "C" int pnerf_set_cross_terms_where(int mask) {
    if (mask < 0 || mask > 7) return PNERF_E_INVAL;
    (void)pn_mix_mask();
    const int old = pn_mix_mask_;
    pn_mix_mask_ = mask;
    return old;
}

int pn_agg_forward_launch(const pnerf_camera *cam, const pnerf_points *pts, const float *d_params, const void *d_packed,
                          const float *d_raydir, const float *d_sample_loc, const float *d_xyz_pers, const float *d_loc_pers,
                          const int32_t *d_sample_pidx,
                          const int32_t *d_valid_list, const int32_t *d_counters, int R, int SR, int K,
                          float *d_decoded, float *d_weight, const PnSaved &sv, long long cap_samples, bool train, bool save_x0,
                          hipStream_t s) {
    FwdArgs a;
    const bool wg2 = train && sv.wg2;
    if (wg2) save_x0 = true;
    a.save_x0 = save_x0 ? 1 : 0;
    a.cam = *cam;
    a.xyz = pts->xyz; a.emb = pts->embedding; a.conf = pts->conf; a.dir = pts->dir; a.color = pts->color;
    a.params = d_params; a.packed = (const float4 *)d_packed;
    a.raydir = d_raydir; a.sample_loc = d_sample_loc; a.xyz_pers = d_xyz_pers; a.loc_pers = d_loc_pers; a.pidx = d_sample_pidx; a.valid_list = d_valid_list; a.counters = d_counters;
    a.R = R; a.SR = SR; a.K = K; a.TS = pn_tile_samples(K);
    a.cap_samples = cap_samples;
    a.decoded = d_decoded; a.weight = d_weight; a.sv = sv;
    int dev = 0, ncu = 256;
    if (hipGetDevice(&dev) != hipSuccess) return PNERF_E_LAUNCH;
    if (hipDeviceGetAttribute(&ncu, hipDeviceAttributeMultiprocessorCount, dev) != hipSuccess) ncu = 256;
    const long long ctiles = (cap_samples + PN_CTILE - 1) / PN_CTILE;
    const int grid_c = (int)(ctiles < 2 * ncu ? (ctiles > 0 ? ctiles : 1) : 2 * ncu);
    const size_t lds_a = FL_BYTES, lds_c = CL_BYTES;
    const bool pers = d_xyz_pers != nullptr;
    const bool np2 = !train && pn_inference_products == 2;
    const bool mix = !wg2 && !np2 && (pn_mix_mask() & (train ? 2 : 1));
    using FwdKernel = void (*)(FwdArgs);
    const FwdKernel kfn = wg2   ? (pers ? k_agg_forward<true, true, 3, true> : k_agg_forward<true, false, 3, true>)
                        : mix   ? (train ? (pers ? k_agg_forward<true, true, 4> : k_agg_forward<true, false, 4>)
                                         : (pers ? k_agg_forward<false, true, 4> : k_agg_forward<false, false, 4>))
                        : train ? (pers ? k_agg_forward<true, true, 3> : k_agg_forward<true, false, 3>)
                        : np2   ? (pers ? k_agg_forward<false, true, 2> : k_agg_forward<false, false, 2>)
                                : (pers ? k_agg_forward<false, true, 3> : k_agg_forward<false, false, 3>);
    const FwdKernel cfn = wg2 ? k_color_forward<true, 3, true> : train ? k_color_forward<true, 3> : np2 ? k_color_forward<false, 2> : k_color_forward<false, 3>;
    if (hipFuncSetAttribute(reinterpret_cast<const void *>(kfn), hipFuncAttributeMaxDynamicSharedMemorySize, (int)lds_a) != hipSuccess) return PNERF_E_LAUNCH;
    if (hipFuncSetAttribute(reinterpret_cast<const void *>(cfn), hipFuncAttributeMaxDynamicSharedMemorySize, (int)lds_c) != hipSuccess) return PNERF_E_LAUNCH;
    int rc = pn_classify(sv, d_valid_list, d_counters, d_sample_pidx, K, cap_samples, train, save_x0, s);
    if (rc) return rc;
    a.cls_list = sv.cls_list; a.cls_info = sv.cls_info; a.Kstride = K;
    int kc[PN_NCLS];
    const int ncls = pn_class_slots(K, kc);
    {
        PnProfScope prof(PNK_AGG_FWD, s);
        for (int j = 0; j < ncls; ++j) {
            a.cls = j; a.K = kc[j]; a.TS = pn_tile_samples(kc[j]);
            const long long tiles = (cap_samples + a.TS - 1) / a.TS;
            const int grid_a = (int)(tiles < 2LL * ncu ? (tiles > 0 ? tiles : 1) : 2LL * ncu);
            hipLaunchKernelGGL(kfn, dim3(grid_a), dim3(PN_NTHR), lds_a, s, a);
        }
    }
    a.K = K; a.TS = pn_tile_samples(K); a.valid_list = sv.cls_list;
    {
        PnProfScope prof(PNK_COLOR_FWD, s);
        hipLaunchKernelGGL(cfn, dim3(grid_c), dim3(256), lds_c, s, a);
    }
    PN_CHECK_LAUNCH();
    return 0;
}

#ifdef PN_PHASE_TRACE
extern "C" int pnerf_debug_trace_fwd(void *host, size_t bytes) {
    return hipMemcpyFromSymbol(host, HIP_SYMBOL(pn_trace_fwd), bytes < sizeof(pn_trace_fwd) ? bytes : sizeof(pn_trace_fwd)) == hipSuccess ? 0 : -1;
}
#endif
```

pointnerf_amd/csrc/pn_common.h:

```cpp
#pragma once
#include <hip/hip_runtime.h>
#include <stdint.h>
#include <stddef.h>
#include "pnerf.h"

#define PN_WAVE 64

#define PN_CHECK_LAUNCH()                                         \
    do {                                                          \
        if (hipGetLastError() != hipSuccess) return PNERF_E_LAUNCH; \
    } while (0)

static inline size_t pn_align(size_t x, size_t a = 256) { return (x + a - 1) / a * a; }
static inline int pn_cdiv(long long a, long long b) { return (int)((a + b - 1) / b); }

struct PnCarver {
    char *base; size_t off, cap;
    PnCarver(void *p, size_t c) : base((char *)p), off(0), cap(c) {}
    template <class T> T *take(size_t n) {
        T *r = (T *)(base + off);
        off += pn_align(n * sizeof(T));
        return r;
    }
    bool ok() const { return off <= cap; }
};

enum PnKernelId { PNK_GRID = 0, PNK_PROBE, PNK_NEIGHBORS, PNK_COMPACT, PNK_PACK, PNK_AGG_FWD, PNK_COLOR_FWD, PNK_RAYMARCH_FWD,
                  PNK_RAYMARCH_BWD, PNK_COLOR_BWD, PNK_AGG_BWD, PNK_WGRAD, PNK_WGRAD_REDUCE, PNK_GATHER, PNK_ADAM, PNK_COUNT };
extern int pn_prof_enabled;
void pn_prof_mark(int id, bool begin, hipStream_t s);
struct PnProfScope {
    int id; hipStream_t s;
    PnProfScope(int id_, hipStream_t s_) : id(id_), s(s_) { if (pn_prof_enabled) pn_prof_mark(id, true, s); }
    ~PnProfScope() { if (pn_prof_enabled) pn_prof_mark(id, false, s); }
};

size_t pn_scan_scratch_ints(long long n);
int pn_exclusive_scan_i32(const int *in, int *out, long long n, int *scratch, hipStream_t s);
int pn_compact_gt0_i32(const int *in, long long n, int *list, int *count_out, int *scratch, hipStream_t s);

struct PnGridDev {
    float ox, oy, oz;
    float vx, vy, vz;
    int gx, gy, gz;
    int by, bz;
    int P;
    const char *base;
    const int *info;
    const uint4 *bricks;
    const uint32_t *occ;
    const float4 *pts;
};

struct PnGridLayout {
    size_t info, bricks, occ, pts, ostart, keys, cnt, tmp_idx, ocell, bocc, bpts, brank, bbase, scan, total;
    long long G, NB;
};
PnGridLayout pn_grid_layout(const pnerf_grid_params *gp, int n);
PnGridDev pn_grid_dev(const pnerf_grid_params *gp, const void *ws, int n_unused);

__device__ __forceinline__ int pn_cell(float p, float o, float v) {
    return (int)floorf((p - o) / v);
}
__host__ __device__ __forceinline__ int pn_brick_of(int x, int y, int z, int by, int bz) { return ((x >> 2) * by + (y >> 2)) * bz + (z >> 2); }
__host__ __device__ __forceinline__ int pn_cell_in_brick(int x, int y, int z) { return ((x & 3) << 4) | ((y & 3) << 2) | (z & 3); }
__device__ __forceinline__ const int *pn_grid_ostart(const PnGridDev &g) { return (const int *)(g.base + (size_t)g.info[PNERF_GI_OSTART_OFF] * 256); }
__device__ __forceinline__ int pn_cell_points(const PnGridDev &g, const int *__restrict__ ostart, int cell0, int x, int y, int z, int &st) {
    const int brick = pn_brick_of(x, y, z, g.by, g.bz), local = pn_cell_in_brick(x, y, z);
    const uint4 rec = g.bricks[brick];
    const unsigned long long bits = ((unsigned long long)rec.y << 32) | rec.x;
    if (!((bits >> local) & 1ull) || brick * 64 + local == cell0) return 0;
    const int o = (int)rec.z + __popcll(bits & ((1ull << local) - 1ull));
    st = ostart[o];
    return min(g.P, ostart[o + 1] - st);
}
```

pointnerf_amd/csrc/prof.hip:

```cpp
#include <vector>
#include "pn_common.h"

int pn_prof_enabled = 0;
namespace {
struct Rec { int id; hipEvent_t a, b; };
std::vector<Rec> g_recs;
std::vector<hipEvent_t> g_pool;
hipEvent_t g_open[PNK_COUNT];
hipEvent_t get_event() {
    if (!g_pool.empty()) { hipEvent_t e = g_pool.back(); g_pool.pop_back(); return e; }
    hipEvent_t e;
    if (hipEventCreate(&e) != hipSuccess) return nullptr;
    return e;
}
const char *kNames[PNK_COUNT] = {"grid_build", "probe", "neighbors", "compact", "mlp_pack", "agg_forward", "color_forward",
                                 "raymarch_forward", "raymarch_backward", "color_backward", "agg_backward", "wgrad",
                                 "wgrad_reduce", "gather", "adam"};
}

void pn_prof_mark(int id, bool begin, hipStream_t s) {
    if (id < 0 || id >= PNK_COUNT) return;
    hipEvent_t e = get_event();
    if (!e) return;
    (void)hipEventRecord(e, s);
    if (begin) g_open[id] = e;
    else { g_recs.push_back({id, g_open[id], e}); g_open[id] = nullptr; }
}

extern "C" int pnerf_prof_enable(int on) {
    pn_prof_enabled = on ? 1 : 0;
    return 0;
}

extern "C" int pnerf_prof_kernel_count(void) { return PNK_COUNT; }
extern "C" const char *pnerf_prof_kernel_name(int id) { return (id >= 0 && id < PNK_COUNT) ? kNames[id] : ""; }

extern "C" int pnerf_prof_collect(double *total_ms, int64_t *launches) {
    if (!total_ms || !launches) return PNERF_E_INVAL;
    if (hipDeviceSynchronize() != hipSuccess) return PNERF_E_LAUNCH;
    for (int i = 0; i < PNK_COUNT; ++i) { total_ms[i] = 0.0; launches[i] = 0; }
    for (const Rec &r : g_recs) {
        float ms = 0.f;
        if (r.a && r.b && hipEventElapsedTime(&ms, r.a, r.b) == hipSuccess) { total_ms[r.id] += ms; launches[r.id] += 1; }
        if (r.a) g_pool.push_back(r.a);
        if (r.b) g_pool.push_back(r.b);
    }
    g_recs.clear();
    return 0;
}

namespace {
typedef _Float16 pk_h8 __attribute__((ext_vector_type(8)));
typedef float pk_f16v __attribute__((ext_vector_type(16)));
__device__ __forceinline__ unsigned pk_prn(unsigned x) { x ^= x >> 16; x *= 0x7feb352du; x ^= x >> 15; x *= 0x846ca68bu; x ^= x >> 16; return x; }
__global__ __launch_bounds__(256, 2) void k_mfma_rate(int mode, int iters, float *__restrict__ out) {
    uint4 ra[4], rb[4];
    for (int i = 0; i < 4; ++i) {
        unsigned w[8];
        for (int j = 0; j < 8; ++j) {
            const unsigned r = pk_prn(threadIdx.x * 64 + blockIdx.x * 7919 + i * 8 + j);
            w[j] = mode == 0 ? 0u : mode == 1 ? 0x2c002c00u : ((r & 0x83ff83ffu) | 0x38003800u);
        }
        ra[i] = make_uint4(w[0], w[1], w[2], w[3]); rb[i] = make_uint4(w[4], w[5], w[6], w[7]);
    }
    pk_f16v acc[4];
    for (int i = 0; i < 4; ++i) for (int r = 0; r < 16; ++r) acc[i][r] = 0.f;
    for (int it = 0; it < iters; ++it) {
#pragma unroll
        for (int s = 0; s < 4; ++s) {
            const pk_h8 a = __builtin_bit_cast(pk_h8, ra[s]), b = __builtin_bit_cast(pk_h8, rb[(s + it) & 3]);
#pragma unroll
            for (int k = 0; k < 4; ++k) acc[k] = __builtin_amdgcn_mfma_f32_32x32x16_f16(a, b, acc[k], 0, 0, 0);
#pragma unroll
            for (int k = 0; k < 4; ++k) acc[k] = __builtin_amdgcn_mfma_f32_32x32x16_f16(b, a, acc[k], 0, 0, 0);
        }
        if ((it & 63) == 63) for (int k = 0; k < 4; ++k) for (int r = 0; r < 16; ++r) acc[k][r] *= 1e-3f;
    }
    float s = 0.f;
    for (int k = 0; k < 4; ++k) for (int r = 0; r < 16; ++r) s += acc[k][r];
    if (s == 123.456f) out[threadIdx.x] = s;
}
}

extern "C" int pnerf_debug_mfma_rate(int mode, int iters, float *d_scratch, double *flop_out, void *stream) {
    if (mode < 0 || mode > 2 || iters <= 0 || !d_scratch) return PNERF_E_INVAL;
    int dev = 0, cus = 256;
    if (hipGetDevice(&dev) == hipSuccess) (void)hipDeviceGetAttribute(&cus, hipDeviceAttributeMultiprocessorCount, dev);
    const int wgs = 2 * cus;
    hipLaunchKernelGGL(k_mfma_rate, dim3(wgs), dim3(256), 0, (hipStream_t)stream, mode, iters, d_scratch);
    PN_CHECK_LAUNCH();
    if (flop_out) *flop_out = (double)wgs * 4.0 * iters * 32.0 * (2.0 * 32 * 32 * 16);
    return 0;
}
```

pointnerf_amd/csrc/render.hip:

```cpp
#include "mlp_common.h"

int pn_agg_forward_launch(const pnerf_camera *cam, const pnerf_points *pts, const float *d_params, const void *d_packed,
                          const float *d_raydir, const float *d_sample_loc, const float *d_xyz_pers, const float *d_loc_pers,
                          const int32_t *d_sample_pidx,
                          const int32_t *d_valid_list, const int32_t *d_counters, int R, int SR, int K,
                          float *d_decoded, float *d_weight, const PnSaved &sv, long long cap_samples, bool train, bool save_x0,
                          hipStream_t s);
int pn_agg_backward_launch(const pnerf_camera *cam, const pnerf_points *pts, const float *d_params, const void *d_packed,
                           const float *d_raydir, const float *d_sample_loc, const int32_t *d_sample_pidx,
                           const int32_t *d_valid_list, const int32_t *d_counters, int R, int SR, int K,
                           const float *d_decoded, const float *d_weight, const float *d_grad_decoded,
                           const PnSaved &sv, long long n_valid, float *d_grad_params, const pnerf_point_grads *pg,
                           float *d_partials, bool x0_saved, hipStream_t s);
size_t pn_wgrad_partials_bytes();

namespace {
constexpr int TPB = 256;

struct RmArgs {
    pnerf_camera cam;
    const float *sample_loc, *decoded;
    const int *nn;
    const float *ray_dist;
    const unsigned char *valid8;
    int R, SR;
};

__device__ __forceinline__ float wave_incl_max(float v, int lane) {
#pragma unroll
    for (int off = 1; off < 64; off <<= 1) { float y = __shfl_up(v, off, 64); if (lane >= off) v = fmaxf(v, y); }
    return v;
}
__device__ __forceinline__ float wave_incl_prod(float v, int lane) {
#pragma unroll
    for (int off = 1; off < 64; off <<= 1) { float y = __shfl_up(v, off, 64); if (lane >= off) v *= y; }
    return v;
}
__device__ __forceinline__ float wave_incl_sum(float v, int lane) {
#pragma unroll
    for (int off = 1; off < 64; off <<= 1) { float y = __shfl_up(v, off, 64); if (lane >= off) v += y; }
    return v;
}
__device__ __forceinline__ float wave_sum(float v) {
#pragma unroll
    for (int off = 32; off > 0; off >>= 1) v += __shfl_xor(v, off, 64);
    return v;
}

__device__ __forceinline__ float pers_z(const pnerf_camera &c, const float *p) {
    return (p[0] - c.campos[0]) * c.camrot[2] + (p[1] - c.campos[1]) * c.camrot[5] + (p[2] - c.campos[2]) * c.camrot[8];
}

__device__ __forceinline__ void chunk_raydist(const RmArgs &a, int r, int s, int lane, float &cm_prev, float &delta, bool &valid) {
    const int SR = a.SR;
    if (a.ray_dist) {
        valid = s < SR && a.valid8[(long long)r * SR + s] != 0;
        delta = s < SR ? a.ray_dist[(long long)r * SR + s] : 0.f;
        return;
    }
    float z = -INFINITY, znext = -INFINITY;
    if (s < SR) z = pers_z(a.cam, a.sample_loc + ((long long)r * SR + s) * 3);
    if (s + 1 < SR) znext = pers_z(a.cam, a.sample_loc + ((long long)r * SR + s + 1) * 3);
    float cm = fmaxf(wave_incl_max(z, lane), cm_prev);
    const float vs = a.cam.vsize_z;
    float d = (s + 1 < SR) ? fmaxf(cm, znext) - cm : vs;
    bool m = d < 1e-8f;
    if (a.cam.raydist_mode_unit > 0) m = m || (d > 2.f * vs);
    if (m) d = vs;
    valid = s < SR && a.nn[(long long)r * SR + s] > 0;
    delta = valid ? d : 0.f;
    cm_prev = __shfl(cm, 63, 64);
}

__global__ __launch_bounds__(TPB) void k_raymarch_forward(RmArgs a, float *__restrict__ ray_color, float *__restrict__ opacity_out,
                                                          float *__restrict__ bg_trans, float *__restrict__ blend_w,
                                                          float *__restrict__ acc_trans) {
    const int lane = threadIdx.x & 63;
    const int r = blockIdx.x * (TPB / 64) + (threadIdx.x >> 6);
    if (r >= a.R) return;
    const int SR = a.SR;
    float cm_prev = -INFINITY, T_carry = 1.f;
    float cr = 0.f, cg = 0.f, cb = 0.f;
    for (int base = 0; base < SR; base += 64) {
        const int s = base + lane;
        float delta; bool valid;
        chunk_raydist(a, r, s, lane, cm_prev, delta, valid);
        float sigma = 0.f, rr = 0.f, gg = 0.f, bb = 0.f;
        if (s < SR) {
            const float4 f = *reinterpret_cast<const float4 *>(a.decoded + ((long long)r * SR + s) * 4);
            sigma = valid ? f.x : 0.f; rr = f.y; gg = f.z; bb = f.w;
        }
        const float op = 1.f - expf(-sigma * delta);
        const float u = s < SR ? (1.f - op + 1e-10f) : 1.f;
        const float incl = wave_incl_prod(u, lane);
        float Tx = __shfl_up(incl, 1, 64);
        if (lane == 0) Tx = 1.f;
        Tx *= T_carry;
        const float bw = op * Tx;
        if (s < SR) {
            opacity_out[(long long)r * SR + s] = op;
            blend_w[(long long)r * SR + s] = bw;
            if (acc_trans) acc_trans[(long long)r * SR + s] = Tx;
        }
        cr += bw * rr; cg += bw * gg; cb += bw * bb;
        T_carry *= __shfl(incl, 63, 64);
    }
    cr = wave_sum(cr); cg = wave_sum(cg); cb = wave_sum(cb);
    if (lane == 0) {
        if (a.cam.has_bg) { cr += a.cam.bg[0] * T_carry; cg += a.cam.bg[1] * T_carry; cb += a.cam.bg[2] * T_carry; }
        ray_color[3 * r] = cr; ray_color[3 * r + 1] = cg; ray_color[3 * r + 2] = cb;
        bg_trans[r] = T_carry;
    }
}

__global__ __launch_bounds__(TPB) void k_raymarch_backward(RmArgs a, const float *__restrict__ grad_color, float *__restrict__ grad_decoded) {
    const int lane = threadIdx.x & 63;
    const int r = blockIdx.x * (TPB / 64) + (threadIdx.x >> 6);
    if (r >= a.R) return;
    const int SR = a.SR;
    const float g0 = grad_color[3 * r], g1 = grad_color[3 * r + 1], g2 = grad_color[3 * r + 2];
    float cm_prev = -INFINITY, T_carry = 1.f, tot = 0.f;
    for (int base = 0; base < SR; base += 64) {
        const int s = base + lane;
        float delta; bool valid;
        chunk_raydist(a, r, s, lane, cm_prev, delta, valid);
        float sigma = 0.f, c = 0.f;
        if (s < SR) {
            const float4 f = *reinterpret_cast<const float4 *>(a.decoded + ((long long)r * SR + s) * 4);
            sigma = valid ? f.x : 0.f; c = g0 * f.y + g1 * f.z + g2 * f.w;
        }
        const float op = 1.f - expf(-sigma * delta);
        const float u = s < SR ? (1.f - op + 1e-10f) : 1.f;
        const float incl = wave_incl_prod(u, lane);
        float Tx = __shfl_up(incl, 1, 64);
        if (lane == 0) Tx = 1.f;
        Tx *= T_carry;
        tot += op * Tx * c;
        T_carry *= __shfl(incl, 63, 64);
    }
    tot = wave_sum(tot);
    const float T_end = T_carry;
    const float gbg = a.cam.has_bg ? (g0 * a.cam.bg[0] + g1 * a.cam.bg[1] + g2 * a.cam.bg[2]) * T_end : 0.f;
    cm_prev = -INFINITY; T_carry = 1.f;
    float pre_carry = 0.f;
    for (int base = 0; base < SR; base += 64) {
        const int s = base + lane;
        float delta; bool valid;
        chunk_raydist(a, r, s, lane, cm_prev, delta, valid);
        float sigma = 0.f, c = 0.f;
        if (s < SR) {
            const float4 f = *reinterpret_cast<const float4 *>(a.decoded + ((long long)r * SR + s) * 4);
            sigma = valid ? f.x : 0.f; c = g0 * f.y + g1 * f.z + g2 * f.w;
        }
        const float e = expf(-sigma * delta);
        const float op = 1.f - e;
        const float u = s < SR ? (1.f - op + 1e-10f) : 1.f;
        const float incl = wave_incl_prod(u, lane);
        float Tx = __shfl_up(incl, 1, 64);
        if (lane == 0) Tx = 1.f;
        Tx *= T_carry;
        const float bwc = op * Tx * c;
        const float incl_sum = wave_incl_sum(bwc, lane) + pre_carry;
        const float suffix = tot - incl_sum + gbg;
        const float dop = Tx * c - suffix / u;
        if (s < SR) {
            const float bw = op * Tx;
            float4 o;
            o.x = valid ? dop * delta * e : 0.f;
            o.y = bw * g0; o.z = bw * g1; o.w = bw * g2;
            *reinterpret_cast<float4 *>(grad_decoded + ((long long)r * SR + s) * 4) = o;
        }
        pre_carry = __shfl(incl_sum, 63, 64);
        T_carry *= __shfl(incl, 63, 64);
    }
}

__global__ __launch_bounds__(TPB) void k_gather_rows(const float *__restrict__ src, int n_src, int width, const int *__restrict__ idx,
                                                     long long n_idx, float *__restrict__ dst) {
    const long long total = n_idx * width;
    for (long long e = (long long)blockIdx.x * TPB + threadIdx.x; e < total; e += (long long)gridDim.x * TPB) {
        const long long i = e / width;
        const int c = (int)(e - i * width);
        int p = idx[i];
        p = p < 0 ? 0 : (p >= n_src ? n_src - 1 : p);
        dst[e] = src[(long long)p * width + c];
    }
}
template <int W4>
__global__ __launch_bounds__(TPB) void k_gather_rows_v4(const float4 *__restrict__ src, int n_src, const int *__restrict__ idx, long long n_idx, float4 *__restrict__ dst) {
    const int c = threadIdx.x & (W4 - 1);
    for (long long i = ((long long)blockIdx.x * TPB + threadIdx.x) / W4; i < n_idx; i += (long long)gridDim.x * (TPB / W4)) {
        int p = idx[i];
        p = p < 0 ? 0 : (p >= n_src ? n_src - 1 : p);
        const float4 v = src[(long long)p * W4 + c];
        pn_f4 t = {v.x, v.y, v.z, v.w};
        __builtin_nontemporal_store(t, reinterpret_cast<pn_f4 *>(dst + i * W4 + c));
    }
}
__global__ __launch_bounds__(TPB) void k_scatter_add_rows(const float *__restrict__ grad_rows, const int *__restrict__ idx, long long n_idx,
                                                          int width, float *__restrict__ grad_src, int n_src) {
    __shared__ float row0[64];
    const bool use_lds = width <= 64;
    if (use_lds && threadIdx.x < 64) row0[threadIdx.x] = 0.f;
    __syncthreads();
    const long long total = n_idx * width;
    for (long long e = (long long)blockIdx.x * TPB + threadIdx.x; e < total; e += (long long)gridDim.x * TPB) {
        const long long i = e / width;
        const int c = (int)(e - i * width);
        int p = idx[i];
        const float g = grad_rows[e];
        if (p <= 0 && use_lds) { atomicAdd(&row0[c], g); continue; }
        p = p < 0 ? 0 : (p >= n_src ? n_src - 1 : p);
        atomicAdd(&grad_src[(long long)p * width + c], g);
    }
    __syncthreads();
    if (use_lds && threadIdx.x < width && row0[threadIdx.x] != 0.f) atomicAdd(&grad_src[threadIdx.x], row0[threadIdx.x]);
}

__device__ __forceinline__ float pn_zero_one_value(const float *__restrict__ conf, int n, int p, float eps, bool &inside) {
    p = p < 0 ? 0 : (p >= n ? n - 1 : p);
    const float c = fminf(fmaxf(conf[p], 1e-4f), 1.0f);
    inside = c >= eps && c <= 1.f - eps;
    return fminf(fmaxf(c, eps), 1.f - eps);
}
__global__ __launch_bounds__(TPB) void k_zero_one_forward(const float *__restrict__ conf, int n, const int *__restrict__ idx, long long n_idx, float eps,
                                                          float *__restrict__ partial) {
    __shared__ float red[TPB / 64];
    float acc = 0.f;
    for (long long e = (long long)blockIdx.x * TPB + threadIdx.x; e < n_idx; e += (long long)gridDim.x * TPB) {
        bool inside;
        const float v = pn_zero_one_value(conf, n, idx[e], eps, inside);
        acc += logf(v) + logf(1.f - v);
    }
#pragma unroll
    for (int off = 32; off > 0; off >>= 1) acc += __shfl_xor(acc, off, 64);
    if ((threadIdx.x & 63) == 0) red[threadIdx.x >> 6] = acc;
    __syncthreads();
    if (threadIdx.x == 0) {
        float t = 0.f;
        for (int w = 0; w < TPB / 64; ++w) t += red[w];
        partial[blockIdx.x] = t;
    }
}
__global__ __launch_bounds__(TPB) void k_zero_one_backward(const float *__restrict__ conf, int n, const int *__restrict__ idx, long long n_idx, float eps,
                                                           const float *__restrict__ gscale, float *__restrict__ grad_conf) {
    __shared__ float row0;
    if (threadIdx.x == 0) row0 = 0.f;
    __syncthreads();
    const float gs = gscale[0];
    float mine0 = 0.f;
    for (long long e = (long long)blockIdx.x * TPB + threadIdx.x; e < n_idx; e += (long long)gridDim.x * TPB) {
        const int p = idx[e];
        bool inside;
        const float v = pn_zero_one_value(conf, n, p, eps, inside);
        if (!inside) continue;
        const float g = gs * (1.f / v - 1.f / (1.f - v));
        if (p <= 0) mine0 += g;
        else atomicAdd(&grad_conf[p >= n ? n - 1 : p], g);
    }
#pragma unroll
    for (int off = 32; off > 0; off >>= 1) mine0 += __shfl_xor(mine0, off, 64);
    if ((threadIdx.x & 63) == 0 && mine0 != 0.f) atomicAdd(&row0, mine0);
    __syncthreads();
    if (threadIdx.x == 0 && row0 != 0.f) atomicAdd(&grad_conf[0], row0);
}
__global__ __launch_bounds__(TPB) void k_zero_one_forward_rays(const float *__restrict__ conf, int n, const int *__restrict__ idx, const int *__restrict__ hit, int R, int slots,
                                                               float eps, float *__restrict__ partial) {
    __shared__ float red[TPB / 64];
    float acc = 0.f;
    for (int r = blockIdx.x; r < R; r += gridDim.x) {
        if (hit[r] <= 0) continue;
        const int *row = idx + (long long)r * slots;
        for (int e = threadIdx.x; e < slots; e += TPB) {
            bool inside;
            const float v = pn_zero_one_value(conf, n, row[e], eps, inside);
            acc += logf(v) + logf(1.f - v);
        }
    }
#pragma unroll
    for (int off = 32; off > 0; off >>= 1) acc += __shfl_xor(acc, off, 64);
    if ((threadIdx.x & 63) == 0) red[threadIdx.x >> 6] = acc;
    __syncthreads();
    if (threadIdx.x == 0) {
        float t = 0.f;
        for (int w = 0; w < TPB / 64; ++w) t += red[w];
        partial[blockIdx.x] = t;
    }
}
__global__ __launch_bounds__(TPB) void k_zero_one_backward_rays(const float *__restrict__ conf, int n, const int *__restrict__ idx, const int *__restrict__ hit, int R, int slots,
                                                                float eps, const float *__restrict__ gscale, float *__restrict__ grad_conf) {
    __shared__ float row0;
    if (threadIdx.x == 0) row0 = 0.f;
    __syncthreads();
    const float gs = gscale[0];
    float mine0 = 0.f;
    for (int r = blockIdx.x; r < R; r += gridDim.x) {
        if (hit[r] <= 0) continue;
        const int *row = idx + (long long)r * slots;
        for (int e = threadIdx.x; e < slots; e += TPB) {
            const int p = row[e];
            bool inside;
            const float v = pn_zero_one_value(conf, n, p, eps, inside);
            if (!inside) continue;
            const float g = gs * (1.f / v - 1.f / (1.f - v));
            if (p <= 0) mine0 += g;
            else atomicAdd(&grad_conf[p >= n ? n - 1 : p], g);
        }
    }
#pragma unroll
    for (int off = 32; off > 0; off >>= 1) mine0 += __shfl_xor(mine0, off, 64);
    if ((threadIdx.x & 63) == 0 && mine0 != 0.f) atomicAdd(&row0, mine0);
    __syncthreads();
    if (threadIdx.x == 0 && row0 != 0.f) atomicAdd(&grad_conf[0], row0);
}
}

namespace {
__global__ __launch_bounds__(256) void k_color_loss_forward_rays(const float *__restrict__ col, const float *__restrict__ gt, const int *__restrict__ hit, int R,
                                                                 float *__restrict__ partial) {
    __shared__ float red[4];
    float acc = 0.f;
    for (int r = blockIdx.x * 256 + threadIdx.x; r < R; r += gridDim.x * 256)
        if (hit[r] > 0) {
            const float dx = col[3 * r] - gt[3 * r], dy = col[3 * r + 1] - gt[3 * r + 1], dz = col[3 * r + 2] - gt[3 * r + 2];
            acc += (dx * dx + dy * dy) + dz * dz;
        }
#pragma unroll
    for (int off = 32; off > 0; off >>= 1) acc += __shfl_xor(acc, off, 64);
    if ((threadIdx.x & 63) == 0) red[threadIdx.x >> 6] = acc;
    __syncthreads();
    if (threadIdx.x == 0) partial[blockIdx.x] = (red[0] + red[1]) + (red[2] + red[3]);
}
__global__ __launch_bounds__(256) void k_color_loss_backward_rays(const float *__restrict__ col, const float *__restrict__ gt, const int *__restrict__ hit, int R,
                                                                  const float *__restrict__ gscale, float *__restrict__ gcol) {
    const int r = blockIdx.x * 256 + threadIdx.x;
    if (r >= R) return;
    const float g = hit[r] > 0 ? 2.f * gscale[0] : 0.f;
#pragma unroll
    for (int c = 0; c < 3; ++c) gcol[3 * r + c] = g == 0.f ? 0.f : g * (col[3 * r + c] - gt[3 * r + c]);
}
}
extern "C" int pnerf_color_loss_blocks(int R) {
    const int b = (R + 255) / 256;
    return b < 1 ? 1 : (b > 1024 ? 1024 : b);
}
extern "C" int pnerf_color_loss_forward_rays(const float *d_ray_color, const float *d_gt, const int32_t *d_ray_hit, int R, float *d_partial, void *stream) {
    if (!d_ray_color || !d_gt || !d_ray_hit || !d_partial || R < 0) return PNERF_E_INVAL;
    PnProfScope prof(PNK_GATHER, (hipStream_t)stream);
    hipLaunchKernelGGL(k_color_loss_forward_rays, dim3(pnerf_color_loss_blocks(R)), dim3(256), 0, (hipStream_t)stream, d_ray_color, d_gt, d_ray_hit, R, d_partial);
    PN_CHECK_LAUNCH();
    return 0;
}
extern "C" int pnerf_color_loss_backward_rays(const float *d_ray_color, const float *d_gt, const int32_t *d_ray_hit, int R, const float *d_gscale,
                                              float *d_grad_ray_color, void *stream) {
    if (R == 0) return 0;
    if (!d_ray_color || !d_gt || !d_ray_hit || !d_gscale || !d_grad_ray_color || R < 0) return PNERF_E_INVAL;
    PnProfScope prof(PNK_GATHER, (hipStream_t)stream);
    hipLaunchKernelGGL(k_color_loss_backward_rays, dim3((R + 255) / 256), dim3(256), 0, (hipStream_t)stream, d_ray_color, d_gt, d_ray_hit, R, d_gscale, d_grad_ray_color);
    PN_CHECK_LAUNCH();
    return 0;
}

extern "C" int pnerf_zero_one_forward_rays(const float *d_conf, int n_points, const int32_t *d_idx, const int32_t *d_ray_hit, int R, int slots_per_ray, float eps,
                                           float *d_partial, void *stream) {
    if (!d_conf || !d_partial || !d_idx || !d_ray_hit || n_points <= 0 || R < 0 || slots_per_ray <= 0) return PNERF_E_INVAL;
    PnProfScope prof(PNK_GATHER, (hipStream_t)stream);
    hipLaunchKernelGGL(k_zero_one_forward_rays, dim3(pnerf_zero_one_blocks((int64_t)R * TPB)), dim3(TPB), 0, (hipStream_t)stream, d_conf, n_points, d_idx, d_ray_hit, R, slots_per_ray, eps, d_partial);
    PN_CHECK_LAUNCH();
    return 0;
}
extern "C" int pnerf_zero_one_backward_rays(const float *d_conf, int n_points, const int32_t *d_idx, const int32_t *d_ray_hit, int R, int slots_per_ray, float eps,
                                            const float *d_gscale, float *d_grad_conf, void *stream) {
    if (R == 0) return 0;
    if (!d_conf || !d_idx || !d_ray_hit || !d_gscale || !d_grad_conf || n_points <= 0 || R < 0 || slots_per_ray <= 0) return PNERF_E_INVAL;
    PnProfScope prof(PNK_GATHER, (hipStream_t)stream);
    hipLaunchKernelGGL(k_zero_one_backward_rays, dim3(pnerf_zero_one_blocks((int64_t)R * TPB)), dim3(TPB), 0, (hipStream_t)stream, d_conf, n_points, d_idx, d_ray_hit, R, slots_per_ray, eps, d_gscale, d_grad_conf);
    PN_CHECK_LAUNCH();
    return 0;
}

extern "C" int pnerf_zero_one_blocks(int64_t n_idx) {
    const long long b = (n_idx + TPB - 1) / TPB;
    return (int)(b < 1 ? 1 : (b > 2048 ? 2048 : b));
}
extern "C" int pnerf_zero_one_forward(const float *d_conf, int n_points, const int32_t *d_idx, int64_t n_idx, float eps, float *d_partial, void *stream) {
    if (!d_conf || !d_partial || n_points <= 0 || n_idx < 0 || (n_idx > 0 && !d_idx)) return PNERF_E_INVAL;
    PnProfScope prof(PNK_GATHER, (hipStream_t)stream);
    hipLaunchKernelGGL(k_zero_one_forward, dim3(pnerf_zero_one_blocks(n_idx)), dim3(TPB), 0, (hipStream_t)stream, d_conf, n_points, d_idx, (long long)n_idx, eps, d_partial);
    PN_CHECK_LAUNCH();
    return 0;
}
extern "C" int pnerf_zero_one_backward(const float *d_conf, int n_points, const int32_t *d_idx, int64_t n_idx, float eps, const float *d_gscale,
                                       float *d_grad_conf, void *stream) {
    if (n_idx == 0) return 0;
    if (!d_conf || !d_idx || !d_gscale || !d_grad_conf || n_points <= 0 || n_idx < 0) return PNERF_E_INVAL;
    PnProfScope prof(PNK_GATHER, (hipStream_t)stream);
    hipLaunchKernelGGL(k_zero_one_backward, dim3(pnerf_zero_one_blocks(n_idx)), dim3(TPB), 0, (hipStream_t)stream, d_conf, n_points, d_idx, (long long)n_idx, eps, d_gscale, d_grad_conf);
    PN_CHECK_LAUNCH();
    return 0;
}

extern "C" int pnerf_gather_rows(const float *d_src, int n_src, int width, const int32_t *d_idx, int64_t n_idx, float *d_dst, void *stream) {
    if (n_idx == 0) return 0;
    if (!d_src || !d_idx || !d_dst || n_src <= 0 || width <= 0 || n_idx < 0) return PNERF_E_INVAL;
    long long total = n_idx * width;
    int grid = (int)((total + TPB - 1) / TPB < 16384 ? (total + TPB - 1) / TPB : 16384);
    PnProfScope prof(PNK_GATHER, (hipStream_t)stream);
    const bool al = ((uintptr_t)d_src % 16 == 0) && ((uintptr_t)d_dst % 16 == 0);
    const long long rows_per_block = TPB / (width / 4 > 0 ? width / 4 : 1);
    const int gridv = (int)((n_idx + rows_per_block - 1) / rows_per_block < 16384 ? (n_idx + rows_per_block - 1) / rows_per_block : 16384);
    if (al && width == 32) hipLaunchKernelGGL(k_gather_rows_v4<8>, dim3(gridv), dim3(TPB), 0, (hipStream_t)stream, (const float4 *)d_src, n_src, d_idx, (long long)n_idx, (float4 *)d_dst);
    else if (al && width == 4) hipLaunchKernelGGL(k_gather_rows_v4<1>, dim3(gridv), dim3(TPB), 0, (hipStream_t)stream, (const float4 *)d_src, n_src, d_idx, (long long)n_idx, (float4 *)d_dst);
    else hipLaunchKernelGGL(k_gather_rows, dim3(grid), dim3(TPB), 0, (hipStream_t)stream, d_src, n_src, width, d_idx, (long long)n_idx, d_dst);
    PN_CHECK_LAUNCH();
    return 0;
}

extern "C" int pnerf_scatter_add_rows(const float *d_grad_rows, const int32_t *d_idx, int64_t n_idx, int width, float *d_grad_src, int n_src, void *stream) {
    if (n_idx == 0) return 0;
    if (!d_grad_rows || !d_idx || !d_grad_src || n_src <= 0 || width <= 0 || n_idx < 0) return PNERF_E_INVAL;
    long long total = n_idx * width;
    int grid = (int)((total + TPB - 1) / TPB < 4096 ? (total + TPB - 1) / TPB : 4096);
    PnProfScope prof(PNK_GATHER, (hipStream_t)stream);
    hipLaunchKernelGGL(k_scatter_add_rows, dim3(grid), dim3(TPB), 0, (hipStream_t)stream, d_grad_rows, d_idx, (long long)n_idx, width, d_grad_src, n_src);
    PN_CHECK_LAUNCH();
    return 0;
}

namespace {
__global__ __launch_bounds__(256) void k_touched_flags(const int *__restrict__ pidx, long long n, int n_points, int *__restrict__ flags) {
    for (long long i = (long long)blockIdx.x * 256 + threadIdx.x; i < n; i += (long long)gridDim.x * 256) {
        const int p = pidx[i];
        if (p >= 0 && p < n_points) flags[p] = 1;
        else if (p < 0) flags[0] = 1;
    }
}
}
extern "C" int pnerf_touched_flags(const int32_t *d_pidx, int64_t n, int32_t n_points, int32_t *d_flags, void *stream) {
    if (n < 0 || n_points < 0 || (n > 0 && !d_pidx) || (n_points > 0 && !d_flags)) return PNERF_E_INVAL;
    hipStream_t s = (hipStream_t)stream;
    if (n_points == 0) return 0;
    if (hipMemsetAsync(d_flags, 0, (size_t)n_points * sizeof(int32_t), s) != hipSuccess) return PNERF_E_LAUNCH;
    if (n == 0) return 0;
    const long long blocks = (n + 255) / 256;
    PnProfScope prof(PNK_GATHER, s);
    hipLaunchKernelGGL(k_touched_flags, dim3((unsigned)(blocks < 8192 ? blocks : 8192)), dim3(256), 0, s, d_pidx, (long long)n, n_points, d_flags);
    PN_CHECK_LAUNCH();
    return 0;
}

extern "C" size_t pnerf_agg_workspace_bytes(int64_t n_valid_max, int K) {
    if (K <= 0 || K > PNERF_MAX_K || n_valid_max < 0) return 0;
    long long rows, samples;
    pn_saved_bytes(n_valid_max, K, &rows, &samples);
    return pn_align((size_t)samples * PN_H * sizeof(float)) + pn_cls_bytes(samples) + pn_wgrad_partials_bytes();
}

static int check_common(const pnerf_camera *cam, const pnerf_points *pts, int R, int SR, int K) {
    if (!cam || !pts || R < 0 || SR <= 0 || K <= 0 || K > PNERF_MAX_K) return PNERF_E_INVAL;
    if (pts->feat_dim != PN_F) return PNERF_E_UNSUP;
    if (!pts->xyz || !pts->embedding || !pts->conf || !pts->dir || !pts->color) return PNERF_E_UNSUP;
    return 0;
}

extern "C" int pnerf_render_forward(const pnerf_camera *cam, const pnerf_points *pts, const void *d_packed_mlp, const float *d_params,
                                    const float *d_raydir, const float *d_sample_loc, const int32_t *d_sample_pidx,
                                    const int32_t *d_sample_nn, const int32_t *d_valid_list, const int32_t *d_counters,
                                    int R, int SR, int K,
                                    float *d_decoded, float *d_weight, float *d_ray_color, float *d_opacity,
                                    float *d_bg_trans, float *d_blend_w,
                                    void *d_saved, int64_t n_valid_max, void *d_ws, size_t ws_bytes, void *stream) {
    int rc = check_common(cam, pts, R, SR, K);
    if (rc) return rc;
    if (!d_packed_mlp || !d_params || !d_raydir || !d_sample_loc || !d_sample_pidx || !d_sample_nn || !d_valid_list || !d_counters) return PNERF_E_INVAL;
    if (!d_decoded || !d_weight || !d_ray_color || !d_opacity || !d_bg_trans || !d_blend_w) return PNERF_E_INVAL;
    if (R == 0) return 0;
    hipStream_t s = (hipStream_t)stream;
    PnSaved sv;
    const bool train = d_saved != nullptr;
    if (train) sv = pn_saved_carve(d_saved, n_valid_max, K);
    else {
        if (!d_ws || ws_bytes < pnerf_agg_workspace_bytes(n_valid_max, K)) return PNERF_E_WS;
        sv = PnSaved();
        pn_saved_bytes(n_valid_max, K, &sv.rows, &sv.samples);
        sv.fs = (float *)d_ws;
        pn_cls_carve((char *)d_ws + pn_align((size_t)sv.samples * PN_H * sizeof(float)), sv.samples, sv);
    }
    if (hipMemsetAsync(d_decoded, 0, (size_t)R * SR * 4 * sizeof(float), s) != hipSuccess) return PNERF_E_LAUNCH;
    if (hipMemsetAsync(d_weight, 0, (size_t)R * SR * K * sizeof(float), s) != hipSuccess) return PNERF_E_LAUNCH;
    if (n_valid_max > 0) {
        rc = pn_agg_forward_launch(cam, pts, d_params, d_packed_mlp, d_raydir, d_sample_loc, nullptr, nullptr, d_sample_pidx, d_valid_list, d_counters,
                                   R, SR, K, d_decoded, d_weight, sv, n_valid_max, train, false, s);
        if (rc) return rc;
    }
    RmArgs ra;
    ra.cam = *cam; ra.sample_loc = d_sample_loc; ra.decoded = d_decoded; ra.nn = d_sample_nn; ra.ray_dist = nullptr; ra.valid8 = nullptr; ra.R = R; ra.SR = SR;
    { PnProfScope prof(PNK_RAYMARCH_FWD, s);
    hipLaunchKernelGGL(k_raymarch_forward, dim3(pn_cdiv(R, TPB / 64)), dim3(TPB), 0, s, ra, d_ray_color, d_opacity, d_bg_trans, d_blend_w, (float *)nullptr); }
    PN_CHECK_LAUNCH();
    return 0;
}

extern "C" int pnerf_render_backward(const pnerf_camera *cam, const pnerf_points *pts, const void *d_packed_mlp, const float *d_params,
                                     const float *d_raydir, const float *d_sample_loc, const int32_t *d_sample_pidx,
                                     const int32_t *d_sample_nn, const int32_t *d_valid_list, const int32_t *d_counters,
                                     int R, int SR, int K, int64_t n_valid,
                                     const float *d_decoded, const float *d_weight, const float *d_opacity,
                                     const float *d_grad_ray_color,
                                     void *d_saved, float *d_grad_params, const pnerf_point_grads *pg,
                                     void *d_ws, size_t ws_bytes, void *stream) {
    (void)d_opacity;
    int rc = check_common(cam, pts, R, SR, K);
    if (rc) return rc;
    if (!d_packed_mlp || !d_params || !d_raydir || !d_sample_loc || !d_sample_pidx || !d_sample_nn || !d_valid_list || !d_counters) return PNERF_E_INVAL;
    if (!d_decoded || !d_weight || !d_grad_ray_color || !d_saved || !d_grad_params || !pg || !d_ws) return PNERF_E_INVAL;
    const size_t gd_bytes = pn_align((size_t)R * SR * 4 * sizeof(float));
    if (ws_bytes < gd_bytes + pn_wgrad_partials_bytes()) return PNERF_E_WS;
    if (R == 0 || n_valid == 0) return 0;
    hipStream_t s = (hipStream_t)stream;
    float *grad_decoded = (float *)d_ws;
    float *partials = (float *)((char *)d_ws + gd_bytes);
    RmArgs ra;
    ra.cam = *cam; ra.sample_loc = d_sample_loc; ra.decoded = d_decoded; ra.nn = d_sample_nn; ra.ray_dist = nullptr; ra.valid8 = nullptr; ra.R = R; ra.SR = SR;
    { PnProfScope prof(PNK_RAYMARCH_BWD, s);
    hipLaunchKernelGGL(k_raymarch_backward, dim3(pn_cdiv(R, TPB / 64)), dim3(TPB), 0, s, ra, d_grad_ray_color, grad_decoded); }
    PN_CHECK_LAUNCH();
    PnSaved sv = pn_saved_carve(d_saved, n_valid, K);
    return pn_agg_backward_launch(cam, pts, d_params, d_packed_mlp, d_raydir, d_sample_loc, d_sample_pidx, d_valid_list, d_counters,
                                  R, SR, K, d_decoded, d_weight, grad_decoded, sv, n_valid, d_grad_params, pg, partials, false, s);
}

extern "C" size_t pnerf_render_backward_workspace_bytes(int R, int SR) {
    return pn_align((size_t)R * SR * 4 * sizeof(float)) + pn_wgrad_partials_bytes();
}


extern "C" size_t pnerf_compact_workspace_bytes(int64_t n) { return pn_align(pn_scan_scratch_ints(n) * sizeof(int)); }

extern "C" int pnerf_compact_valid(const int32_t *d_nn, int64_t n, int32_t *d_list, int32_t *d_counters, void *d_ws, size_t ws_bytes, void *stream) {
    if (!d_nn || !d_list || !d_counters || !d_ws || n < 0) return PNERF_E_INVAL;
    if (ws_bytes < pnerf_compact_workspace_bytes(n)) return PNERF_E_WS;
    hipStream_t s = (hipStream_t)stream;
    if (hipMemsetAsync(d_counters, 0, 8 * sizeof(int), s) != hipSuccess) return PNERF_E_LAUNCH;
    if (n == 0) return 0;
    PnProfScope prof(PNK_COMPACT, s);
    return pn_compact_gt0_i32(d_nn, n, d_list, d_counters, (int *)d_ws, s);
}

extern "C" int pnerf_agg_forward(const pnerf_camera *cam, const pnerf_points *pts, const void *d_packed_mlp, const float *d_params,
                                 const float *d_raydir, const float *d_sample_loc, const float *d_xyz_pers, const float *d_loc_pers,
                                 const int32_t *d_sample_pidx, const int32_t *d_valid_list, const int32_t *d_counters,
                                 int R, int SR, int K, float *d_decoded, float *d_weight,
                                 void *d_saved, int64_t n_valid_max, void *d_ws, size_t ws_bytes, void *stream) {
    int rc = check_common(cam, pts, R, SR, K);
    if (rc) return rc;
    if (!d_packed_mlp || !d_params || !d_raydir || !d_sample_loc || !d_sample_pidx || !d_valid_list || !d_counters || !d_decoded || !d_weight) return PNERF_E_INVAL;
    if ((d_xyz_pers == nullptr) != (d_loc_pers == nullptr)) return PNERF_E_INVAL;
    if (R == 0) return 0;
    hipStream_t s = (hipStream_t)stream;
    PnSaved sv;
    const bool train = d_saved != nullptr;
    if (train) sv = pn_saved_carve(d_saved, n_valid_max, K);
    else {
        if (!d_ws || ws_bytes < pnerf_agg_workspace_bytes(n_valid_max, K)) return PNERF_E_WS;
        sv = PnSaved();
        pn_saved_bytes(n_valid_max, K, &sv.rows, &sv.samples);
        sv.fs = (float *)d_ws;
        pn_cls_carve((char *)d_ws + pn_align((size_t)sv.samples * PN_H * sizeof(float)), sv.samples, sv);
    }
    if (hipMemsetAsync(d_decoded, 0, (size_t)R * SR * 4 * sizeof(float), s) != hipSuccess) return PNERF_E_LAUNCH;
    if (hipMemsetAsync(d_weight, 0, (size_t)R * SR * K * sizeof(float), s) != hipSuccess) return PNERF_E_LAUNCH;
    if (n_valid_max == 0) return 0;
    return pn_agg_forward_launch(cam, pts, d_params, d_packed_mlp, d_raydir, d_sample_loc, d_xyz_pers, d_loc_pers, d_sample_pidx,
                                 d_valid_list, d_counters, R, SR, K, d_decoded, d_weight, sv, n_valid_max, train, train, s);
}

extern "C" int pnerf_agg_backward(const pnerf_camera *cam, const pnerf_points *pts, const void *d_packed_mlp, const float *d_params,
                                  const float *d_raydir, const float *d_sample_loc, const int32_t *d_sample_pidx,
                                  const int32_t *d_valid_list, const int32_t *d_counters, int R, int SR, int K, int64_t n_valid,
                                  const float *d_decoded, const float *d_weight, const float *d_grad_decoded,
                                  void *d_saved, float *d_grad_params, const pnerf_point_grads *pg, void *d_ws, size_t ws_bytes, void *stream) {
    int rc = check_common(cam, pts, R, SR, K);
    if (rc) return rc;
    if (!d_packed_mlp || !d_params || !d_raydir || !d_sample_loc || !d_sample_pidx || !d_valid_list || !d_counters) return PNERF_E_INVAL;
    if (!d_decoded || !d_weight || !d_grad_decoded || !d_saved || !d_grad_params || !pg || !d_ws) return PNERF_E_INVAL;
    if (ws_bytes < pn_wgrad_partials_bytes()) return PNERF_E_WS;
    if (R == 0 || n_valid == 0) return 0;
    PnSaved sv = pn_saved_carve(d_saved, n_valid, K);
    return pn_agg_backward_launch(cam, pts, d_params, d_packed_mlp, d_raydir, d_sample_loc, d_sample_pidx, d_valid_list, d_counters,
                                  R, SR, K, d_decoded, d_weight, d_grad_decoded, sv, n_valid, d_grad_params, pg, (float *)d_ws,
                                  true, (hipStream_t)stream);
}

extern "C" int pnerf_raymarch_forward(const float *d_ray_dist, const uint8_t *d_ray_valid, const float *d_features, const float *bg3_host,
                                      int R, int SR, float *d_ray_color, float *d_opacity, float *d_acc_trans, float *d_blend_w,
                                      float *d_bg_trans, void *stream) {
    if (!d_ray_dist || !d_ray_valid || !d_features || !d_ray_color || !d_opacity || !d_acc_trans || !d_blend_w || !d_bg_trans || R < 0 || SR <= 0) return PNERF_E_INVAL;
    if (R == 0) return 0;
    RmArgs ra = {};
    ra.decoded = d_features; ra.ray_dist = d_ray_dist; ra.valid8 = d_ray_valid; ra.R = R; ra.SR = SR;
    ra.cam.has_bg = bg3_host ? 1 : 0;
    if (bg3_host) { ra.cam.bg[0] = bg3_host[0]; ra.cam.bg[1] = bg3_host[1]; ra.cam.bg[2] = bg3_host[2]; }
    hipStream_t s = (hipStream_t)stream;
    PnProfScope prof(PNK_RAYMARCH_FWD, s);
    hipLaunchKernelGGL(k_raymarch_forward, dim3(pn_cdiv(R, TPB / 64)), dim3(TPB), 0, s, ra, d_ray_color, d_opacity, d_bg_trans, d_blend_w, d_acc_trans);
    PN_CHECK_LAUNCH();
    return 0;
}

extern "C" int pnerf_raymarch_backward(const float *d_ray_dist, const uint8_t *d_ray_valid, const float *d_features, const float *bg3_host,
                                       int R, int SR, const float *d_grad_ray_color, float *d_grad_features, void *stream) {
    if (!d_ray_dist || !d_ray_valid || !d_features || !d_grad_ray_color || !d_grad_features || R < 0 || SR <= 0) return PNERF_E_INVAL;
    if (R == 0) return 0;
    RmArgs ra = {};
    ra.decoded = d_features; ra.ray_dist = d_ray_dist; ra.valid8 = d_ray_valid; ra.R = R; ra.SR = SR;
    ra.cam.has_bg = bg3_host ? 1 : 0;
    if (bg3_host) { ra.cam.bg[0] = bg3_host[0]; ra.cam.bg[1] = bg3_host[1]; ra.cam.bg[2] = bg3_host[2]; }
    hipStream_t s = (hipStream_t)stream;
    PnProfScope prof(PNK_RAYMARCH_BWD, s);
    hipLaunchKernelGGL(k_raymarch_backward, dim3(pn_cdiv(R, TPB / 64)), dim3(TPB), 0, s, ra, d_grad_ray_color, d_grad_features);
    PN_CHECK_LAUNCH();
    return 0;
}
```

pointnerf_amd/ops.py:

```python
import ctypes
import math

import numpy as np
import torch

from . import _lib as L


def _stream():
    return ctypes.c_void_p(torch.cuda.current_stream().cuda_stream)


def _ptr(t):
    if t is None:
        return ctypes.c_void_p(0)
    assert t.is_cuda and t.is_contiguous(), "pointnerf_amd ops need contiguous device tensors"
    return ctypes.c_void_p(t.data_ptr())


def host_array(t):
    if not isinstance(t, torch.Tensor):
        return np.asarray(t)
    if not t.is_cuda:
        return t.detach().numpy()
    cacheable = not isinstance(t, torch.nn.Parameter) and not t.requires_grad
    ver = None
    if cacheable:
        try:
            ver = t._version
        except Exception:
            cacheable = False
    if cacheable:
        c = getattr(t, "_pnerf_host", None)
        if c is not None and c[0] == ver and c[2] == t.data_ptr():
            return c[1]
    arr = t.detach().cpu().numpy()
    arr.setflags(write=False)
    if cacheable:
        try:
            t._pnerf_host = (ver, arr, t.data_ptr())
        except Exception:
            pass
    return arr


def _need_cuda(t, name):
    if not (isinstance(t, torch.Tensor) and t.is_cuda):
        raise RuntimeError("pointnerf_amd: %s must be a device tensor (this path has no CPU implementation)" % name)


def mid_depths(D, near, far):
    t = torch.linspace(0, 1, D + 1).view(1, -1)
    t = near * (1 - t) + far * t
    seg = (t[..., 1:] - t[..., :-1]) * (1 + 0.0 * (torch.zeros(1, 1, D) - 0.5))
    end = torch.cumsum(seg, dim=2)
    end = near + torch.cat([torch.zeros(1, 1, 1), end], dim=2)
    mid = (end[:, :, :-1] + end[:, :, 1:]) / 2
    return mid.reshape(-1).contiguous(), seg.reshape(-1).contiguous()


def grid_hyperparameters(opt, xyz):
    vsize64 = np.asarray(opt.vsize, dtype=np.float64)
    vscale = np.asarray(opt.vscale, dtype=np.int32)
    scaled_vsize = (np.asarray(opt.vsize) * vscale).astype(np.float32)
    radius = np.asarray(opt.radius_limit_scale * max(opt.vsize[0], opt.vsize[1])).astype(np.float32)
    _need_cuda(xyz, "xyz")
    xyz = xyz.contiguous()
    mm6 = torch.empty(6, dtype=torch.float32, device=xyz.device)
    L.check(L.lib().pnerf_points_minmax(_ptr(xyz), int(xyz.shape[0]), _ptr(mm6), _stream()), "pnerf_points_minmax")
    mm = mm6.cpu().numpy().reshape(2, 3)
    rmin = np.asarray(opt.ranges[:3], dtype=np.float32)
    rmax = np.asarray(opt.ranges[3:], dtype=np.float32)
    mn, mx = np.maximum(mm[0], rmin), np.minimum(mm[1], rmax)
    pad = (scaled_vsize * np.asarray(opt.kernel_size) / 2).astype(np.float32)
    mn, mx = (mn - pad).astype(np.float32), (mx + pad).astype(np.float32)
    vdim = (mx - mn).astype(np.float32) / vsize64
    scaled_vdim = np.ceil(vdim / vscale).astype(np.int32)
    ranges = np.concatenate([mn, mx]).astype(np.float32)
    return ranges, scaled_vsize, scaled_vdim, float(radius)


def make_grid_params(ranges, scaled_vsize, scaled_vdim, kernel_size, query_size, P, max_o, radius):
    gp = L.GridParams()
    gp.ranges[:] = [float(x) for x in ranges]
    gp.vsize[:] = [float(x) for x in scaled_vsize]
    gp.vdim[:] = [int(x) for x in scaled_vdim]
    gp.kernel_size[:] = [int(x) for x in kernel_size]
    gp.query_size[:] = [int(x) for x in query_size]
    gp.P, gp.max_o, gp.radius = int(P), int(max_o), float(radius)
    return gp


class VoxelGrid:

    def __init__(self, gp, ws, n_points):
        self.gp, self.ws, self.n_points = gp, ws, n_points
        self._info = None

    def info(self):
        if self._info is None:
            buf = (ctypes.c_int32 * L.GI_LEN)()
            L.check(L.lib().pnerf_grid_info(_ptr(self.ws), buf, _stream()), "pnerf_grid_info")
            self._info = dict(n_in_grid=buf[0], n_occ=buf[1], max_cnt=buf[2], cell0=buf[3], first_idx=buf[4],
                              overflow_max_o=buf[1] > self.gp.max_o, overflow_P=buf[2] > self.gp.P)
        return self._info


def build_grid(gp, xyz):
    _need_cuda(xyz, "xyz")
    xyz = xyz.detach().reshape(-1, 3).contiguous().float()
    n = xyz.shape[0]
    lib = L.lib()
    nbytes = lib.pnerf_grid_workspace_bytes(ctypes.byref(gp), n)
    ws = torch.empty(nbytes, dtype=torch.uint8, device=xyz.device)
    L.check(lib.pnerf_grid_build(ctypes.byref(gp), _ptr(xyz), n, _ptr(ws), nbytes, _stream()), "pnerf_grid_build")
    return VoxelGrid(gp, ws, n)


def query_dense(grid, R, D, SR, K, raypos=None, campos=None, raydir=None, mid=None, near=0.0, far=0.0,
                jitter=0.0, seed=0):
    dev = grid.ws.device
    lib = L.lib()
    loc = torch.empty(R, SR, 3, dtype=torch.float32, device=dev)
    pidx = torch.empty(R, SR, K, dtype=torch.int32, device=dev)
    nn = torch.empty(R, SR, dtype=torch.int32, device=dev)
    hit = torch.empty(R, dtype=torch.int32, device=dev)
    vlist = torch.empty(max(R * SR, 1), dtype=torch.int32, device=dev)
    counters = torch.empty(8, dtype=torch.int32, device=dev)
    nws = lib.pnerf_query_workspace_bytes(R, SR)
    ws = torch.empty(nws, dtype=torch.uint8, device=dev)
    cam = None
    if raypos is None:
        cam = (ctypes.c_float * 3)(*[float(x) for x in campos])
        _need_cuda(raydir, "raydir"); _need_cuda(mid, "mid")
    L.check(lib.pnerf_query(ctypes.byref(grid.gp), _ptr(grid.ws), _ptr(raypos), cam, _ptr(raydir), _ptr(mid),
                            float(near), float(far), float(jitter), int(seed) & (2 ** 64 - 1), R, D, SR, K,
                            _ptr(loc), _ptr(pidx), _ptr(nn), _ptr(hit), _ptr(vlist), _ptr(counters),
                            _ptr(ws), nws, _stream()), "pnerf_query")
    return dict(sample_loc=loc, sample_pidx=pidx, sample_nn=nn, ray_hit=hit, valid_list=vlist, counters=counters)


def jitter_uniforms(seed, R, D, device):
    out = torch.empty(1, R, D, dtype=torch.float32, device=device)
    L.check(L.lib().pnerf_debug_uniform(int(seed) & (2 ** 64 - 1), 0, R * D, _ptr(out), _stream()), "pnerf_debug_uniform")
    return out


def mlp_layout():
    offs = (ctypes.c_int64 * (L.MLP_NTENSORS + 1))()
    L.check(L.lib().pnerf_mlp_layout(32, offs), "pnerf_mlp_layout")
    names = ["block1.0", "block1.2", "block3.0", "block3.2", "alpha_branch.0",
             "color_branch.0", "color_branch.2", "color_branch.4", "color_branch.6"]
    shapes = [(256, 284), (256, 256), (256, 263), (256, 256), (1, 256), (128, 280), (128, 128), (128, 128), (3, 128)]
    out, i = {}, 0
    for n, shp in zip(names, shapes):
        out[n + ".weight"] = (offs[i], shp); out[n + ".bias"] = (offs[i + 1], (shp[0],)); i += 2
    return out, offs[L.MLP_NTENSORS]


def flatten_mlp(state, device):
    lay, total = mlp_layout()
    flat = torch.empty(total, dtype=torch.float32, device=device)
    for k, (o, shp) in lay.items():
        flat[o:o + int(np.prod(shp))] = state[k].detach().reshape(-1).to(device=device, dtype=torch.float32)
    return flat


def pack_mlp(flat, out=None):
    _need_cuda(flat, "mlp parameters")
    lib = L.lib()
    if out is None:
        out = torch.empty(lib.pnerf_mlp_packed_bytes(), dtype=torch.uint8, device=flat.device)
    L.check(lib.pnerf_mlp_pack(_ptr(flat), _ptr(out), _stream()), "pnerf_mlp_pack")
    return out


def make_camera(campos, camrot, vsize_z, raydist_mode_unit=1, bg=None, rw2c=None):
    c = L.Camera()
    c.campos[:] = [float(x) for x in np.asarray(campos, dtype=np.float64).reshape(-1)[:3]]
    c.camrot[:] = [float(x) for x in np.asarray(camrot, dtype=np.float64).reshape(-1)[:9]]
    r = np.eye(3) if rw2c is None else np.asarray(rw2c, dtype=np.float64)
    c.rw2c[:] = [float(x) for x in r.reshape(-1)[:9]]
    c.vsize_z = float(vsize_z)
    c.raydist_mode_unit = int(raydist_mode_unit)
    if bg is None:
        c.has_bg = 0
        c.bg[:] = [0.0, 0.0, 0.0]
    else:
        c.has_bg = 1
        c.bg[:] = [float(x) for x in np.asarray(bg, dtype=np.float64).reshape(-1)[:3]]
    return c


def make_points(xyz, emb, conf, pdir, color):
    for n, t in (("xyz", xyz), ("points_embeding", emb), ("points_conf", conf), ("points_dir", pdir), ("points_color", color)):
        _need_cuda(t, n)
        assert t.is_contiguous() and t.dtype == torch.float32, n
    p = L.Points()
    p.xyz, p.embedding, p.conf, p.dir, p.color = xyz.data_ptr(), emb.data_ptr(), conf.data_ptr(), pdir.data_ptr(), color.data_ptr()
    p.n, p.feat_dim = int(xyz.reshape(-1, 3).shape[0]), int(emb.shape[-1])
    return p


class Arena:

    def __init__(self):
        self.free, self.headroom = [], 1.15

    def take(self, nbytes, device):
        best = None
        for t in self.free:
            if t.numel() >= nbytes and t.device == device and (best is None or t.numel() < best.numel()):
                best = t
        if best is not None:
            self.free.remove(best)
            return best
        self.free = [t for t in self.free if t.device != device]
        return torch.empty(int(nbytes * self.headroom) + 256, dtype=torch.uint8, device=device)

    def give(self, t):
        if t is not None:
            self.free.append(t)

    def capacity_samples(self, K, device):
        best = max((t.numel() for t in self.free if t.device == torch.device(device)), default=0)
        if best <= 0:
            return 0
        key = (best, int(K))
        hit = getattr(self, "_cap_cache", {}).get(key)
        if hit is not None:
            return hit
        fn = L.lib().pnerf_agg_saved_bytes
        lo, hi = 0, best // 512
        while lo < hi:
            mid = (lo + hi + 1) // 2
            if fn(mid, int(K)) <= best:
                lo = mid
            else:
                hi = mid - 1
        self._cap_cache = {key: lo}
        return lo

    def reserve(self, nbytes, device):
        if not any(t.numel() >= nbytes and t.device == device for t in self.free):
            self.give(self.take(nbytes, device))


ARENA = Arena()


def arena_budget_bytes():
    import os
    return int(float(os.environ.get("PNERF_ARENA_BUDGET_GB", "160")) * (1 << 30))


def compact_valid(sample_nn):
    lib = L.lib()
    n = sample_nn.numel()
    dev = sample_nn.device
    vlist = torch.empty(max(n, 1), dtype=torch.int32, device=dev)
    counters = torch.empty(8, dtype=torch.int32, device=dev)
    nws = lib.pnerf_compact_workspace_bytes(n)
    ws = torch.empty(nws, dtype=torch.uint8, device=dev)
    L.check(lib.pnerf_compact_valid(_ptr(sample_nn), n, _ptr(vlist), _ptr(counters), _ptr(ws), nws, _stream()), "pnerf_compact_valid")
    return vlist, counters


def touched_flags(pidx, n_points):
    _need_cuda(pidx, "pidx")
    if pidx.dtype != torch.int32 or not pidx.is_contiguous():
        raise ValueError("touched_flags: a contiguous int32 neighbor table is expected")
    flags = torch.empty(max(int(n_points), 0), dtype=torch.int32, device=pidx.device)
    L.check(L.lib().pnerf_touched_flags(_ptr(pidx), pidx.numel(), int(n_points), _ptr(flags), _stream()), "pnerf_touched_flags")
    return flags


def reserve_pool(nbytes, device):
    t = torch.empty(int(nbytes), dtype=torch.uint8, device=device)
    del t


def render_forward(cam, pts, packed, flat, raydir, dense, R, SR, K, n_valid, train):
    dev = raydir.device
    lib = L.lib()
    f32 = dict(dtype=torch.float32, device=dev)
    decoded = torch.empty(R, SR, 4, **f32); weight = torch.empty(R, SR, K, **f32)
    ray_color = torch.empty(R, 3, **f32); opacity = torch.empty(R, SR, **f32)
    bg_trans = torch.empty(R, **f32); blend_w = torch.empty(R, SR, **f32)
    saved = ws = None
    if train:
        saved = ARENA.take(lib.pnerf_agg_saved_bytes(n_valid, K), dev)
        nws = 0
    else:
        nws = lib.pnerf_agg_workspace_bytes(n_valid, K)
        ws = torch.empty(nws, dtype=torch.uint8, device=dev)
    L.check(lib.pnerf_render_forward(ctypes.byref(cam), ctypes.byref(pts), _ptr(packed), _ptr(flat), _ptr(raydir),
                                     _ptr(dense["sample_loc"]), _ptr(dense["sample_pidx"]), _ptr(dense["sample_nn"]),
                                     _ptr(dense["valid_list"]), _ptr(dense["counters"]), R, SR, K,
                                     _ptr(decoded), _ptr(weight), _ptr(ray_color), _ptr(opacity), _ptr(bg_trans), _ptr(blend_w),
                                     _ptr(saved), n_valid, _ptr(ws), nws, _stream()), "pnerf_render_forward")
    return dict(decoded=decoded, weight=weight, ray_color=ray_color, opacity=opacity, bg_trans=bg_trans,
                blend_w=blend_w, saved=saved)


def render_backward(cam, pts, packed, flat, raydir, dense, R, SR, K, n_valid, fwd, grad_ray_color, grad_flat, grads, ready_event=None, zero_one=None):
    lib = L.lib()
    pg = L.PointGrads()
    pg.embedding, pg.conf = grads["points_embeding"].data_ptr(), grads["points_conf"].data_ptr()
    pg.dir, pg.color = grads["points_dir"].data_ptr(), grads["points_color"].data_ptr()
    if grads.get("xyz") is not None:
        pg.xyz = grads["xyz"].data_ptr()
    if zero_one is not None:
        pg.zero_one_gscale, pg.zero_one_eps = zero_one[0].data_ptr(), float(zero_one[1])
    if ready_event is not None:
        pg.ready_event = ready_event.cuda_event
    nws = lib.pnerf_render_backward_workspace_bytes(R, SR)
    ws = torch.empty(nws, dtype=torch.uint8, device=raydir.device)
    g = grad_ray_color.contiguous().float()
    L.check(lib.pnerf_render_backward(ctypes.byref(cam), ctypes.byref(pts), _ptr(packed), _ptr(flat), _ptr(raydir),
                                      _ptr(dense["sample_loc"]), _ptr(dense["sample_pidx"]), _ptr(dense["sample_nn"]),
                                      _ptr(dense["valid_list"]), _ptr(dense["counters"]), R, SR, K, n_valid,
                                      _ptr(fwd["decoded"]), _ptr(fwd["weight"]), _ptr(fwd["opacity"]), _ptr(g),
                                      _ptr(fwd["saved"]), _ptr(grad_flat), ctypes.byref(pg), _ptr(ws), nws, _stream()),
            "pnerf_render_backward")


class GatherRows(torch.autograd.Function):

    @staticmethod
    def forward(ctx, src, idx):
        _need_cuda(src, "src")
        s2 = src.detach().reshape(-1, src.shape[-1]).contiguous().float()
        i2 = idx.reshape(-1).contiguous().to(torch.int32)
        out = torch.empty(i2.numel(), s2.shape[1], dtype=torch.float32, device=src.device)
        L.check(L.lib().pnerf_gather_rows(_ptr(s2), s2.shape[0], s2.shape[1], _ptr(i2), i2.numel(), _ptr(out), _stream()),
                "pnerf_gather_rows")
        ctx.save_for_backward(i2)
        ctx.src_shape = tuple(src.shape)
        return out.view(tuple(idx.shape) + (s2.shape[1],))

    @staticmethod
    def backward(ctx, g):
        (i2,) = ctx.saved_tensors
        w = ctx.src_shape[-1]
        gs = torch.zeros(ctx.src_shape, dtype=torch.float32, device=g.device)
        g2 = g.reshape(-1, w).contiguous().float()
        n_src = gs.numel() // w
        L.check(L.lib().pnerf_scatter_add_rows(_ptr(g2), _ptr(i2), i2.numel(), w, _ptr(gs), n_src, _stream()),
                "pnerf_scatter_add_rows")
        return gs, None


def gather_rows(src, idx):
    return GatherRows.apply(src, idx)


class ZeroOneConf(torch.autograd.Function):

    @staticmethod
    def forward(ctx, conf, pidx, eps):
        lib = L.lib()
        c = conf.detach().reshape(-1)
        _need_cuda(c, "points_conf")
        idx = pidx.reshape(-1)
        nb = lib.pnerf_zero_one_blocks(idx.numel())
        part = torch.empty(nb, dtype=torch.float32, device=c.device)
        L.check(lib.pnerf_zero_one_forward(_ptr(c), c.numel(), _ptr(idx), idx.numel(), float(eps), _ptr(part), _stream()), "pnerf_zero_one_forward")
        ctx.save_for_backward(c, idx)
        ctx.eps, ctx.shape = float(eps), conf.shape
        return part.sum()

    @staticmethod
    def backward(ctx, g):
        c, idx = ctx.saved_tensors
        grad = torch.zeros_like(c)
        gs = g.detach().reshape(1).to(torch.float32).contiguous()
        L.check(L.lib().pnerf_zero_one_backward(_ptr(c), c.numel(), _ptr(idx), idx.numel(), ctx.eps, _ptr(gs), _ptr(grad), _stream()), "pnerf_zero_one_backward")
        return grad.view(ctx.shape), None, None


def zero_one_conf_sum(conf, pidx, eps):
    return ZeroOneConf.apply(conf, pidx.contiguous(), eps)


class ZeroOneConfRays(torch.autograd.Function):

    @staticmethod
    def forward(ctx, conf, pidx, ray_hit, eps):
        lib = L.lib()
        c = conf.detach().reshape(-1)
        _need_cuda(c, "points_conf")
        R = int(pidx.shape[0])
        slots = int(pidx.numel() // max(R, 1))
        nb = lib.pnerf_zero_one_blocks(R * 256)
        part = torch.empty(nb, dtype=torch.float32, device=c.device)
        L.check(lib.pnerf_zero_one_forward_rays(_ptr(c), c.numel(), _ptr(pidx), _ptr(ray_hit), R, slots, float(eps), _ptr(part), _stream()), "pnerf_zero_one_forward_rays")
        ctx.save_for_backward(c, pidx, ray_hit)
        ctx.eps, ctx.shape, ctx.dims = float(eps), conf.shape, (R, slots)
        return part.sum()

    @staticmethod
    def backward(ctx, g):
        c, pidx, ray_hit = ctx.saved_tensors
        grad = torch.zeros_like(c)
        gs = g.detach().reshape(1).to(torch.float32).contiguous()
        L.check(L.lib().pnerf_zero_one_backward_rays(_ptr(c), c.numel(), _ptr(pidx), _ptr(ray_hit), ctx.dims[0], ctx.dims[1], ctx.eps, _ptr(gs), _ptr(grad), _stream()),
                "pnerf_zero_one_backward_rays")
        return grad.view(ctx.shape), None, None, None


def zero_one_conf_sum_rays(conf, pidx_dense, ray_hit, eps):
    return ZeroOneConfRays.apply(conf, pidx_dense.contiguous(), ray_hit.contiguous(), eps)


class ColorLossRays(torch.autograd.Function):

    @staticmethod
    def forward(ctx, ray_color, gt, ray_hit):
        _need_cuda(ray_color, "ray_color")
        lib = L.lib()
        c, g = ray_color.detach().reshape(-1, 3).contiguous().float(), gt.detach().reshape(-1, 3).contiguous().float()
        R = c.shape[0]
        part = torch.empty(lib.pnerf_color_loss_blocks(R), dtype=torch.float32, device=c.device)
        L.check(lib.pnerf_color_loss_forward_rays(_ptr(c), _ptr(g), _ptr(ray_hit), R, _ptr(part), _stream()), "pnerf_color_loss_forward_rays")
        ctx.save_for_backward(c, g, ray_hit)
        ctx.shape = ray_color.shape
        return part.sum()

    @staticmethod
    def backward(ctx, gout):
        c, g, ray_hit = ctx.saved_tensors
        grad = torch.empty_like(c)
        gs = gout.detach().reshape(1).to(torch.float32).contiguous()
        L.check(L.lib().pnerf_color_loss_backward_rays(_ptr(c), _ptr(g), _ptr(ray_hit), c.shape[0], _ptr(gs), _ptr(grad), _stream()),
                "pnerf_color_loss_backward_rays")
        return grad.view(ctx.shape), None, None


def color_loss_sum_rays(ray_color, gt, ray_hit):
    return ColorLossRays.apply(ray_color, gt, ray_hit.contiguous())


def set_inference_products(n):
    old = L.lib().pnerf_set_inference_products(int(n))
    if old < 0:
        raise ValueError("inference products must be 2 or 3")
    return old


def set_wgrad_planes(n):
    old = L.lib().pnerf_set_wgrad_planes(int(n))
    if old < 0:
        raise ValueError("weight-gradient planes must be 1 or 2")
    ARENA._cap_cache = {}
    return old


def set_cross_terms(bits, where=None):
    old = L.lib().pnerf_set_cross_terms(int(bits))
    if old < 0:
        raise ValueError("cross terms must be 8 or 16")
    oldw = L.lib().pnerf_set_cross_terms_where(int(where)) if where is not None else None
    if where is not None and oldw < 0:
        raise ValueError("cross-term mask must be 0..7")
    return old, oldw


def cross_terms_state():
    lib = L.lib()
    bits = lib.pnerf_set_cross_terms(8)
    lib.pnerf_set_cross_terms(bits)
    mask = lib.pnerf_set_cross_terms_where(4)
    lib.pnerf_set_cross_terms_where(mask)
    return bits, (mask if bits == 8 else 0)


def mfma_rate_tflops(mode=2, ms_target=60.0, device=None):
    import ctypes
    dev = torch.device("cuda", torch.cuda.current_device()) if device is None else device
    scratch = torch.zeros(256, dtype=torch.float32, device=dev)
    flop = ctypes.c_double(0.0)
    iters = max(int(ms_target / 1000.0 * 2.4e9 / (2 * 32 * 32)), 64)
    last = 0.0
    for _ in range(8):
        e0, e1 = torch.cuda.Event(enable_timing=True), torch.cuda.Event(enable_timing=True)
        e0.record()
        L.check(L.lib().pnerf_debug_mfma_rate(int(mode), int(iters), _ptr(scratch), ctypes.byref(flop), _stream()), "pnerf_debug_mfma_rate")
        e1.record()
        e1.synchronize()
        rate = flop.value / (e0.elapsed_time(e1) * 1e-3) / 1e12
        settled = last > 0.0 and abs(rate - last) <= 0.03 * last
        last = rate
        if settled:
            break
    return last


def prof_enable(on=True):
    L.lib().pnerf_prof_enable(1 if on else 0)


def prof_collect():
    lib = L.lib()
    n = lib.pnerf_prof_kernel_count()
    ms = (ctypes.c_double * n)()
    cnt = (ctypes.c_int64 * n)()
    L.check(lib.pnerf_prof_collect(ms, cnt), "pnerf_prof_collect")
    return {lib.pnerf_prof_kernel_name(i).decode(): (ms[i], cnt[i]) for i in range(n)}
```

Before: 2.102 million.

## Hoist point-only part of first MLP layer to a per-point precompute

Splits the first aggregation MLP layer so the columns that depend only on the point embedding (embedding and its positional encoding) are computed once per touched point in a new kernel, not once per sample-neighbor row. The forward kernel then loads the precomputed partial activations through a row-to-slot map and runs only the remaining per-sample columns in its GEMM. New marking, list and point-layer kernels plus a scratch buffer are added. The cost is extra launches, extra global traffic for the partial activations, and a possibly different X0 save path in training.

```diff
diff --git a/include/pnerf.h b/include/pnerf.h
--- a/include/pnerf.h
+++ b/include/pnerf.h
@@ -110,6 +110,19 @@
                          float *d_decoded, float *d_weight, float *d_ray_color, float *d_opacity,
                          float *d_bg_trans, float *d_blend_w,
                          void *d_saved, int64_t n_valid_max, void *d_ws, size_t ws_bytes, void *stream);
+
+size_t pnerf_hoist_bytes(int32_t n_points, int64_t n_valid_max, int K);
+int pnerf_render_forward_hoisted(const pnerf_camera *cam, const pnerf_points *pts, const void *d_packed_mlp,
+                                 const float *d_params, const float *d_raydir, const float *d_sample_loc, const int32_t *d_sample_pidx,
+                                 const int32_t *d_sample_nn, const int32_t *d_valid_list, const int32_t *d_counters,
+                                 int R, int SR, int K,
+                                 float *d_decoded, float *d_weight, float *d_ray_color, float *d_opacity,
+                                 float *d_bg_trans, float *d_blend_w,
+                                 void *d_saved, int64_t n_valid_max, void *d_ws, size_t ws_bytes,
+                                 void *d_hoist, size_t hoist_bytes, void *stream);
+int pnerf_hoist_layout(int32_t n_points, int64_t n_valid_max, int K, int64_t *offsets );
+int pnerf_debug_point_hoist(const pnerf_points *pts, const void *d_packed_mlp, const int32_t *d_sample_pidx, const int32_t *d_valid_list,
+                            const int32_t *d_counters, int64_t n_valid_max, int K, int products, void *d_hoist, size_t hoist_bytes, void *stream);
 
 int pnerf_set_inference_products(int n);
 
diff --git a/pointnerf_amd/_lib.py b/pointnerf_amd/_lib.py
--- a/pointnerf_amd/_lib.py
+++ b/pointnerf_amd/_lib.py
@@ -91,6 +91,15 @@
                                      c_int, c_int, c_int,
                                      c_void_p, c_void_p, c_void_p, c_void_p, c_void_p, c_void_p,
                                      c_void_p, c_i64, c_void_p, c_size_t, c_void_p]),
+    "pnerf_hoist_bytes": (c_size_t, [c_int, c_i64, c_int]),
+    "pnerf_hoist_layout": (c_int, [c_int, c_i64, c_int, ctypes.POINTER(c_i64)]),
+    "pnerf_render_forward_hoisted": (c_int, [ctypes.POINTER(Camera), ctypes.POINTER(Points), c_void_p, c_void_p,
+                                             c_void_p, c_void_p, c_void_p, c_void_p, c_void_p, c_void_p,
+                                             c_int, c_int, c_int,
+                                             c_void_p, c_void_p, c_void_p, c_void_p, c_void_p, c_void_p,
+                                             c_void_p, c_i64, c_void_p, c_size_t, c_void_p, c_size_t, c_void_p]),
+    "pnerf_debug_point_hoist": (c_int, [ctypes.POINTER(Points), c_void_p, c_void_p, c_void_p, c_void_p, c_i64, c_int, c_int,
+                                        c_void_p, c_size_t, c_void_p]),
     "pnerf_set_inference_products": (c_int, [c_int]),
     "pnerf_set_wgrad_planes": (c_int, [c_int]),
     "pnerf_set_cross_terms": (c_int, [c_int]),
diff --git a/pointnerf_amd/csrc/aggregate.hip b/pointnerf_amd/csrc/aggregate.hip
--- a/pointnerf_amd/csrc/aggregate.hip
+++ b/pointnerf_amd/csrc/aggregate.hip
@@ -355,6 +355,8 @@
     long long cap_samples;
     float *decoded, *weight;
     PnSaved sv;
+    const int *rowslot;
+    const float *y1p;
 };
 
 __device__ __forceinline__ void rot3(const float *M , float x, float y, float z, bool transpose, float &ox, float &oy, float &oz) {
@@ -467,11 +469,13 @@
     return (ls < a.TS && vs < Ns) ? a.valid_list[vs] : -1;
 }
 
-template <bool PERS>
+template <bool PERS, bool HOIST = false>
 __device__ __forceinline__ void f_gather(const FwdArgs &a, FGather &G, int si_, int p_, int q) {
     const int p = p_ > 0 ? p_ : 0, si = si_ > 0 ? si_ : 0;
-    const float *ep = a.emb + (long long)p * PN_F + EPT * q;
-    G.e0 = *reinterpret_cast<const float4 *>(ep); G.e1 = *reinterpret_cast<const float4 *>(ep + 4);
+    if (!HOIST) {
+        const float *ep = a.emb + (long long)p * PN_F + EPT * q;
+        G.e0 = *reinterpret_cast<const float4 *>(ep); G.e1 = *reinterpret_cast<const float4 *>(ep + 4);
+    }
     G.px = a.xyz[3 * p]; G.py = a.xyz[3 * p + 1]; G.pz = a.xyz[3 * p + 2];
     G.lx = a.sample_loc[(long long)si * 3]; G.ly = a.sample_loc[(long long)si * 3 + 1]; G.lz = a.sample_loc[(long long)si * 3 + 2];
     if (PERS) {
@@ -487,38 +491,8 @@
     }
 }
 
-template <bool PERS, bool MIX = false, bool HR = false>
-__device__ __forceinline__ void f_build(const FwdArgs &a, const FGather &G, char *X, float *exb, float *wraw, int *sidx, int si, int p, int row, int q) {
-    const float dwx = G.px - G.lx, dwy = G.py - G.ly, dwz = G.pz - G.lz;
-    float ppx, ppy, pcz, spx, spy, scz;
-    if (PERS) {
-        ppx = G.ppx; ppy = G.ppy; pcz = G.ppz; spx = G.lpx; spy = G.lpy; scz = G.lpz;
-    } else {
-        float pcx, pcy, scx, scy;
-        rot3(a.cam.camrot, G.px - a.cam.campos[0], G.py - a.cam.campos[1], G.pz - a.cam.campos[2], false, pcx, pcy, pcz);
-        rot3(a.cam.camrot, G.lx - a.cam.campos[0], G.ly - a.cam.campos[1], G.lz - a.cam.campos[2], false, scx, scy, scz);
-        ppx = pcx / pcz; ppy = pcy / pcz; spx = scx / scz; spy = scy / scz;
-    }
-    float d0, d1, d2;
-    rot3(a.cam.rw2c, dwx, dwy, dwz, true, d0, d1, d2);
-    const float d3 = ppx * pcz - spx * scz, d4 = ppy * pcz - spy * scz, d5 = pcz - scz;
-    const float da = q == 0 ? d0 : q == 1 ? d1 : q == 2 ? d2 : d3;
-    const float db = q == 0 ? d4 : d5;
-    const float e[8] = {G.e0.x, G.e0.y, G.e0.z, G.e0.w, G.e1.x, G.e1.y, G.e1.z, G.e1.w};
-    if (MIX) {
-        pn_xq_store4(X, row, EPT * q, e[0], e[1], e[2], e[3]);
-        pn_xq_store4(X, row, EPT * q + 4, e[4], e[5], e[6], e[7]);
-#pragma unroll
-        for (int i = 0; i < 8; i += 2) {
-            const int col = PN_F + (EPT * q + i) * 6;
-            float s0[3], c0[3], s1[3], c1[3];
-            pn_pe_octaves<3>(e[i], s0, c0);
-            pn_pe_octaves<3>(e[i + 1], s1, c1);
-            pn_xq_store4(X, row, col, s0[0], c0[0], s0[1], c0[1]);
-            pn_xq_store4(X, row, col + 4, s0[2], c0[2], s1[0], c1[0]);
-            pn_xq_store4(X, row, col + 8, s1[1], c1[1], s1[2], c1[2]);
-        }
-    } else {
+template <bool HR>
+__device__ __forceinline__ void f_build_emb(char *X, int row, int q, const float (&e)[8]) {
     if (HR) { pn_xt_store4(X, row, EPT * q, e[0], e[1], e[2], e[3]); pn_xt_store4(X, row, EPT * q + 4, e[4], e[5], e[6], e[7]); }
     else { pn_x_store4<false>(X, row, EPT * q, e[0], e[1], e[2], e[3]); pn_x_store4<false>(X, row, EPT * q + 4, e[4], e[5], e[6], e[7]); }
 #pragma unroll
@@ -536,6 +510,41 @@
             pn_x_store2(X, row, PN_F + dd * 6 + 4, s[2], c[2]);
         }
     }
+}
+
+template <bool PERS, bool MIX = false, bool HR = false, bool HOIST = false>
+__device__ __forceinline__ void f_build(const FwdArgs &a, const FGather &G, char *X, float *exb, float *wraw, int *sidx, int si, int p, int row, int q) {
+    const float dwx = G.px - G.lx, dwy = G.py - G.ly, dwz = G.pz - G.lz;
+    float ppx, ppy, pcz, spx, spy, scz;
+    if (PERS) {
+        ppx = G.ppx; ppy = G.ppy; pcz = G.ppz; spx = G.lpx; spy = G.lpy; scz = G.lpz;
+    } else {
+        float pcx, pcy, scx, scy;
+        rot3(a.cam.camrot, G.px - a.cam.campos[0], G.py - a.cam.campos[1], G.pz - a.cam.campos[2], false, pcx, pcy, pcz);
+        rot3(a.cam.camrot, G.lx - a.cam.campos[0], G.ly - a.cam.campos[1], G.lz - a.cam.campos[2], false, scx, scy, scz);
+        ppx = pcx / pcz; ppy = pcy / pcz; spx = scx / scz; spy = scy / scz;
+    }
+    float d0, d1, d2;
+    rot3(a.cam.rw2c, dwx, dwy, dwz, true, d0, d1, d2);
+    const float d3 = ppx * pcz - spx * scz, d4 = ppy * pcz - spy * scz, d5 = pcz - scz;
+    const float da = q == 0 ? d0 : q == 1 ? d1 : q == 2 ? d2 : d3;
+    const float db = q == 0 ? d4 : d5;
+    if constexpr (!HOIST) {
+    const float e[8] = {G.e0.x, G.e0.y, G.e0.z, G.e0.w, G.e1.x, G.e1.y, G.e1.z, G.e1.w};
+    if (MIX) {
+        pn_xq_store4(X, row, EPT * q, e[0], e[1], e[2], e[3]);
+        pn_xq_store4(X, row, EPT * q + 4, e[4], e[5], e[6], e[7]);
+#pragma unroll
+        for (int i = 0; i < 8; i += 2) {
+            const int col = PN_F + (EPT * q + i) * 6;
+            float s0[3], c0[3], s1[3], c1[3];
+            pn_pe_octaves<3>(e[i], s0, c0);
+            pn_pe_octaves<3>(e[i + 1], s1, c1);
+            pn_xq_store4(X, row, col, s0[0], c0[0], s0[1], c0[1]);
+            pn_xq_store4(X, row, col + 4, s0[2], c0[2], s1[0], c1[0]);
+            pn_xq_store4(X, row, col + 8, s1[1], c1[1], s1[2], c1[2]);
+        }
+    } else f_build_emb<HR>(X, row, q, e);
     }
 #pragma unroll
     for (int j = 0; j < 2; ++j) {
@@ -612,6 +621,41 @@
         for (int j = 0; j < 2; ++j)
 #pragma unroll
             for (int r = 0; r < 16; ++r) acc[i][j][r] = 0.f;
+}
+
+__device__ __forceinline__ void f_acc_y1p(const float *__restrict__ y1p, const int (&rs)[2], int wave, int lane, f32x16 (&acc)[PN_NFB][2]) {
+#pragma unroll
+    for (int rb = 0; rb < 2; ++rb) {
+        if (rs[rb] >= 0) {
+            const float *src = y1p + (size_t)rs[rb] * PN_H;
+#pragma unroll
+            for (int fb = 0; fb < PN_NFB; ++fb)
+#pragma unroll
+                for (int g = 0; g < 4; ++g) {
+                    const float4 v = *reinterpret_cast<const float4 *>(src + pn_d_feat(PN_NFB * wave + fb, g, lane));
+                    acc[fb][rb][4 * g] = v.x; acc[fb][rb][4 * g + 1] = v.y; acc[fb][rb][4 * g + 2] = v.z; acc[fb][rb][4 * g + 3] = v.w;
+                }
+        } else {
+#pragma unroll
+            for (int fb = 0; fb < PN_NFB; ++fb)
+#pragma unroll
+                for (int r = 0; r < 16; ++r) acc[fb][rb][r] = 0.f;
+        }
+    }
+}
+__device__ __forceinline__ void f_acc_add_bias(const float *__restrict__ bias, int wave, int lane, f32x16 (&acc)[PN_NFB][2]) {
+#pragma unroll
+    for (int fb = 0; fb < PN_NFB; ++fb)
+#pragma unroll
+        for (int g = 0; g < 4; ++g) {
+            const float4 b = *reinterpret_cast<const float4 *>(bias + pn_d_feat(PN_NFB * wave + fb, g, lane));
+#pragma unroll
+            for (int rb = 0; rb < 2; ++rb) { acc[fb][rb][4 * g] += b.x; acc[fb][rb][4 * g + 1] += b.y; acc[fb][rb][4 * g + 2] += b.z; acc[fb][rb][4 * g + 3] += b.w; }
+        }
+}
+__device__ __forceinline__ void f_row_slots(const int *__restrict__ rowslot, long long gtile, int lane, int (&rs)[2]) {
+#pragma unroll
+    for (int rb = 0; rb < 2; ++rb) rs[rb] = rowslot[gtile * PN_TILE + 32 * rb + (lane & 31)];
 }
 
 __device__ __forceinline__ float pn_softplus(float x) {
@@ -692,8 +736,9 @@
 #ifdef PN_PHASE_TRACE
 PN_TR_DECL(pn_trace_fwd);
 #endif
-template <bool TRAIN, bool PERS, int NP, bool WG2 = false>
+template <bool TRAIN, bool PERS, int NP, bool WG2 = false, bool HOIST = false>
 __global__ __launch_bounds__(PN_NTHR, PN_NW / 2) void k_agg_forward(FwdArgs a) {
+    static_assert(!HOIST || (!PERS && !WG2 && NP != 4), "instances that materialise all of X0 in the tile keep the per-row layer 1");
     constexpr bool MIX = NP == 4;
     constexpr bool HR = !MIX;
     constexpr bool HC = TRAIN && !WG2;
@@ -729,10 +774,17 @@
         si2 = tile + 2 * stride < tile_last ? f_sample_of(a, tile + 2 * stride, row, Ns, kinv) : -1;
         p0 = si0 >= 0 ? a.pidx[(long long)si0 * a.Kstride + k] : -1;
         p1 = si1 >= 0 ? a.pidx[(long long)si1 * a.Kstride + k] : -1;
-        f_gather<PERS>(a, G, si0, p0, q);
+        f_gather<PERS, HOIST>(a, G, si0, p0, q);
     }
 
     f32x16 acc[PN_NFB][2];
+    int rs[2] = {-1, -1};
+    if constexpr (HOIST) {
+        f_row_slots(a.rowslot, tb + tile, tid0 & 63, rs);
+        f_acc_y1p(a.y1p, rs, __builtin_amdgcn_readfirstlane(tid0 >> 6), tid0 & 63, acc);
+        if (tile + stride < tile_last) f_row_slots(a.rowslot, tb + tile + stride, tid0 & 63, rs);
+        else rs[0] = rs[1] = -1;
+    }
     PN_TR_ITER_DECL;
     for (; tile < tile_last; tile += stride) {
         PN_TR_ITER_NEXT;
@@ -743,12 +795,14 @@
         const long long gtile = tb + tile;
         PN_LDS_BARRIER();
         PN_TR(pn_trace_fwd, 0); PN_TR_HWID(pn_trace_fwd);
-        f_build<PERS, MIX, HR>(a, G, X, exb, wraw, sidx, si0, p0, row, q);
-        f_acc_bias(P + PO_B1, wave, lane, acc);
-        PnGemmW<18, 8, PN_NFB, PN_WPF, NPC> W1;
+        f_build<PERS, MIX, HR, HOIST>(a, G, X, exb, wraw, sidx, si0, p0, row, q);
+        constexpr int NC1 = HOIST ? 4 : 18, C1 = HOIST ? 14 : 0;
+        if constexpr (HOIST) f_acc_add_bias(P + PO_B1, wave, lane, acc);
+        else f_acc_bias(P + PO_B1, wave, lane, acc);
+        PnGemmW<NC1, 8, PN_NFB, PN_WPF, NPC> W1;
         PnMixW<PN_MIX_NS, 2, 8, PN_NFB> M1;
         if constexpr (MIX) M1.prefetch(img + PKM_F1, PN_NFB * wave, lane);
-        else W1.prefetch(reinterpret_cast<const uint4 *>(img + PKH_F1), PN_NFB * wave, lane);
+        else W1.prefetch(reinterpret_cast<const uint4 *>(img + PKH_F1), PN_NFB * wave, lane, C1);
         PN_LDS_BARRIER();
         if (q == 0) {
             const int ls = pn_row_div(row, kinv);
@@ -767,10 +821,10 @@
         PN_TR(pn_trace_fwd, 1);
         PN_TR(pn_trace_fwd, 2);
         if constexpr (MIX) pn_gemm_mix_run<PN_MIX_NS, 2, 8, PN_NFB>(X, M1, lane, acc);
-        else pn_gemm_f16x3_run<18, 8, PN_NFB, PN_WPF, NPC>(X, W1, lane, acc);
+        else pn_gemm_f16x3_run<NC1, 8, PN_NFB, PN_WPF, NPC>(X, W1, lane, acc, C1);
         if (TRAIN) {
             if (HC) {
-                if (a.save_x0) pn_copy_out_kmajor_h<PN_NF1>(X, a.sv.x0k, gtile * 8, tid);
+                if (!HOIST && a.save_x0) pn_copy_out_kmajor_h<PN_NF1>(X, a.sv.x0k, gtile * 8, tid);
                 else pn_copy_out_kmajor_cols64_h<224>(X, a.sv.x0k, gtile * 8, tid);
             } else if (WG2) pn_copy_out_kmajor<PN_NF1, true>(X, a.sv.x0k, gtile * 8, tid, a.sv.x0m);
             else if (a.save_x0) pn_copy_out_kmajor<PN_NF1, false>(X, a.sv.x0k, gtile * 8, tid);
@@ -848,12 +902,17 @@
         const float cf_cur = G.cf;
         (void)cf_cur;
         const int si_next = si1, p_next = p1;
-        if (tile + stride < tile_last) f_gather<PERS>(a, G, si1, p1, q);
+        if (tile + stride < tile_last) f_gather<PERS, HOIST>(a, G, si1, p1, q);
         const int p2 = si2 >= 0 ? a.pidx[(long long)si2 * a.Kstride + k] : -1;
         const int si3 = tile + 3 * stride < tile_last ? f_sample_of(a, tile + 3 * stride, row, Ns, kinv) : -1;
         PN_LDS_BARRIER();
         PN_TR(pn_trace_fwd, 13);
         f_epilogue<false>(acc, X, wave, lane, mask);
+        if constexpr (HOIST) {
+            f_acc_y1p(a.y1p, rs, wave, lane, acc);
+            if (tile + 2 * stride < tile_last) f_row_slots(a.rowslot, tb + tile + 2 * stride, lane, rs);
+            else rs[0] = rs[1] = -1;
+        }
         PN_LDS_BARRIER();
         PN_TR(pn_trace_fwd, 14);
         if (K == 8 || K == 4 || K == 2 || K == 1) {
@@ -1032,6 +1091,160 @@
         }
     }
 }
+
+struct HoistArgs {
+    const float *emb; const float4 *packed;
+    const int *pidx, *valid_list, *counters, *cls_list, *cls_info;
+    int *flags, *slot, *list, *count, *rowslot;
+    float *y1p;
+    int K, n_valid, n_points;
+};
+
+__global__ __launch_bounds__(256) void k_hoist_mark(HoistArgs h) {
+    const int Ns = h.counters[0] < h.n_valid ? h.counters[0] : h.n_valid;
+    const long long n = (long long)Ns * h.K;
+    for (long long i = (long long)blockIdx.x * 256 + threadIdx.x; i < n; i += (long long)gridDim.x * 256) {
+        const long long vs = i / h.K;
+        const int p = h.pidx[(long long)h.valid_list[vs] * h.K + (int)(i - vs * h.K)];
+        if (p >= 0 && p < h.n_points) h.flags[p] = 1;
+    }
+}
+
+template <int NP>
+__global__ __launch_bounds__(PN_NTHR, PN_NW / 2) void k_point_layer1(HoistArgs h) {
+    pn_mode_saturate();
+    extern __shared__ __attribute__((aligned(16))) char smem_p[];
+    char *X = smem_p;
+    const int n = h.count[0];
+    const long long ntiles = ((long long)n + PN_TILE - 1) / PN_TILE;
+    f32x16 acc[PN_NFB][2];
+    for (long long tile = blockIdx.x; tile < ntiles; tile += gridDim.x) {
+        int tid = threadIdx.x;
+        asm volatile("" : "+v"(tid));
+        const int lane = tid & 63, wave = __builtin_amdgcn_readfirstlane(tid >> 6), row = tid / TPR, q = tid % TPR;
+        const long long i = tile * PN_TILE + row;
+        const int p = i < n ? h.list[i] : -1;
+        float e[8] = {0.f, 0.f, 0.f, 0.f, 0.f, 0.f, 0.f, 0.f};
+        if (p >= 0) {
+            const float *ep = h.emb + (long long)p * PN_F + EPT * q;
+            const float4 e0 = *reinterpret_cast<const float4 *>(ep), e1 = *reinterpret_cast<const float4 *>(ep + 4);
+            e[0] = e0.x; e[1] = e0.y; e[2] = e0.z; e[3] = e0.w; e[4] = e1.x; e[5] = e1.y; e[6] = e1.z; e[7] = e1.w;
+            if (q == 0) h.slot[p] = (int)i;
+        }
+        PN_LDS_BARRIER();
+        f_build_emb<true>(X, row, q, e);
+        f_acc_zero(acc);
+        PnGemmW<14, 8, PN_NFB, PN_WPF, NP> W;
+        W.prefetch(reinterpret_cast<const uint4 *>(reinterpret_cast<const char *>(h.packed) + PKH_F1), PN_NFB * wave, lane);
+        PN_LDS_BARRIER();
+        pn_gemm_f16x3_run<14, 8, PN_NFB, PN_WPF, NP>(X, W, lane, acc);
+#pragma unroll
+        for (int rb = 0; rb < 2; ++rb) {
+            const long long r = tile * PN_TILE + 32 * rb + (lane & 31);
+            if (r < n) {
+#pragma unroll
+                for (int fb = 0; fb < PN_NFB; ++fb)
+#pragma unroll
+                    for (int g = 0; g < 4; ++g) {
+                        pn_f4 t = {acc[fb][rb][4 * g], acc[fb][rb][4 * g + 1], acc[fb][rb][4 * g + 2], acc[fb][rb][4 * g + 3]};
+                        PN_REG_STORE(t, reinterpret_cast<pn_f4 *>(h.y1p + r * PN_H + pn_d_feat(PN_NFB * wave + fb, g, lane)));
+                    }
+            }
+        }
+    }
+}
+
+__global__ __launch_bounds__(256) void k_hoist_rowslot(HoistArgs h, int c, int kc, int ts) {
+    const int Ns = h.cls_info[PN_CI_COUNT + c];
+    const long long vb = h.cls_info[PN_CI_VBASE + c], tb = h.cls_info[PN_CI_TBASE + c];
+    const long long ntiles = ((long long)Ns + ts - 1) / ts, n = ntiles * PN_TILE;
+    const unsigned kinv = pn_kinv(kc);
+    for (long long i = (long long)blockIdx.x * 256 + threadIdx.x; i < n; i += (long long)gridDim.x * 256) {
+        const long long tile = i / PN_TILE;
+        const int row = (int)(i - tile * PN_TILE), ls = pn_row_div(row, kinv), k = row - ls * kc;
+        const long long vs = tile * ts + ls;
+        int sl = -1;
+        if (ls < ts && vs < Ns) {
+            const int p = h.pidx[(long long)h.cls_list[vb + vs] * h.K + k];
+            if (p >= 0 && p < h.n_points) sl = h.slot[p];
+        }
+        h.rowslot[(tb + tile) * PN_TILE + row] = sl;
+    }
+}
+}
+
+struct PnHoist { int *flags, *slot, *list, *count, *scan, *rowslot; float *y1p; long long cap_points; };
+static size_t pn_hoist_layout(long long n_points, long long n_valid, int K, size_t off[6], long long *cap_out) {
+    long long rows;
+    pn_saved_bytes(n_valid, K, &rows, nullptr);
+    const long long np = n_points > 0 ? n_points : 0;
+    long long T = n_valid * K < np ? n_valid * K : np;
+    T = (T + PN_TILE - 1) / PN_TILE * PN_TILE + PN_TILE;
+    size_t b = 0;
+    off[0] = b; b += pn_align((size_t)(np + 1) * 4);
+    off[1] = b; b += pn_align((size_t)(np + 1) * 4);
+    off[2] = b; b += pn_align((size_t)T * 4);
+    off[3] = b; b += pn_align(8 * 4) + pn_align(pn_scan_scratch_ints(np) * 4);
+    off[4] = b; b += pn_align((size_t)rows * 4);
+    off[5] = b; b += pn_align((size_t)T * PN_H * 4);
+    if (cap_out) *cap_out = T;
+    return b;
+}
+static PnHoist pn_hoist_carve(void *base, long long n_points, long long n_valid, int K) {
+    size_t off[6];
+    PnHoist h;
+    pn_hoist_layout(n_points, n_valid, K, off, &h.cap_points);
+    char *b = (char *)base;
+    h.flags = (int *)(b + off[0]); h.slot = (int *)(b + off[1]); h.list = (int *)(b + off[2]); h.count = (int *)(b + off[3]);
+    h.scan = (int *)(b + off[3] + pn_align(8 * 4)); h.rowslot = (int *)(b + off[4]); h.y1p = (float *)(b + off[5]);
+    return h;
+}
+extern "C" size_t pnerf_hoist_bytes(int32_t n_points, int64_t n_valid_max, int K) {
+    if (K <= 0 || K > PNERF_MAX_K || n_valid_max < 0 || n_points < 0) return 0;
+    size_t off[6];
+    return pn_hoist_layout(n_points, n_valid_max, K, off, nullptr);
+}
+extern "C" int pnerf_hoist_layout(int32_t n_points, int64_t n_valid_max, int K, int64_t *offsets) {
+    if (K <= 0 || K > PNERF_MAX_K || n_valid_max < 0 || n_points < 0 || !offsets) return PNERF_E_INVAL;
+    size_t off[6];
+    pn_hoist_layout(n_points, n_valid_max, K, off, nullptr);
+    for (int i = 0; i < 6; ++i) offsets[i] = (int64_t)off[i];
+    return 0;
+}
+
+static int pn_hoist_points(HoistArgs &h, const PnHoist &hb, int np, int ncu, hipStream_t s) {
+    h.flags = hb.flags; h.slot = hb.slot; h.list = hb.list; h.count = hb.count; h.rowslot = hb.rowslot; h.y1p = hb.y1p;
+    {
+        PnProfScope prof(PNK_POINT_LIST, s);
+        if (hipMemsetAsync(hb.flags, 0, (size_t)h.n_points * sizeof(int), s) != hipSuccess) return PNERF_E_LAUNCH;
+        const long long blocks = ((long long)h.n_valid * h.K + 255) / 256;
+        hipLaunchKernelGGL(k_hoist_mark, dim3((unsigned)(blocks < 8192 ? (blocks > 0 ? blocks : 1) : 8192)), dim3(256), 0, s, h);
+        int rc = pn_compact_gt0_i32(hb.flags, h.n_points, hb.list, hb.count, hb.scan, s);
+        if (rc) return rc;
+    }
+    using PtKernel = void (*)(HoistArgs);
+    const PtKernel pfn = np == 2 ? k_point_layer1<2> : k_point_layer1<3>;
+    if (hipFuncSetAttribute(reinterpret_cast<const void *>(pfn), hipFuncAttributeMaxDynamicSharedMemorySize, (int)PN_XBYTES) != hipSuccess) return PNERF_E_LAUNCH;
+    const long long tiles = hb.cap_points / PN_TILE;
+    PnProfScope prof(PNK_POINT_L1, s);
+    hipLaunchKernelGGL(pfn, dim3((unsigned)(tiles < 2LL * ncu ? (tiles > 0 ? tiles : 1) : 2LL * ncu)), dim3(PN_NTHR), PN_XBYTES, s, h);
+    PN_CHECK_LAUNCH();
+    return 0;
+}
+
+extern "C" int pnerf_debug_point_hoist(const pnerf_points *pts, const void *d_packed_mlp, const int32_t *d_sample_pidx, const int32_t *d_valid_list,
+                                       const int32_t *d_counters, int64_t n_valid_max, int K, int products, void *d_hoist, size_t hoist_bytes, void *stream) {
+    if (!pts || !pts->embedding || !d_packed_mlp || !d_sample_pidx || !d_valid_list || !d_counters || !d_hoist) return PNERF_E_INVAL;
+    if (pts->feat_dim != PN_F) return PNERF_E_UNSUP;
+    if (K <= 0 || K > PNERF_MAX_K || n_valid_max < 0 || pts->n <= 0 || (products != 2 && products != 3)) return PNERF_E_INVAL;
+    if (hoist_bytes < pnerf_hoist_bytes(pts->n, n_valid_max, K)) return PNERF_E_WS;
+    int dev = 0, ncu = 256;
+    if (hipGetDevice(&dev) != hipSuccess) return PNERF_E_LAUNCH;
+    if (hipDeviceGetAttribute(&ncu, hipDeviceAttributeMultiprocessorCount, dev) != hipSuccess) ncu = 256;
+    HoistArgs h = {};
+    h.emb = pts->embedding; h.packed = (const float4 *)d_packed_mlp; h.pidx = d_sample_pidx; h.valid_list = d_valid_list; h.counters = d_counters;
+    h.K = K; h.n_valid = (int)n_valid_max; h.n_points = pts->n;
+    return pn_hoist_points(h, pn_hoist_carve(d_hoist, pts->n, n_valid_max, K), products, ncu, (hipStream_t)stream);
 }
 
 static int pn_inference_products = 3;
@@ -1083,7 +1296,7 @@
                           const int32_t *d_sample_pidx,
                           const int32_t *d_valid_list, const int32_t *d_counters, int R, int SR, int K,
                           float *d_decoded, float *d_weight, const PnSaved &sv, long long cap_samples, bool train, bool save_x0,
-                          hipStream_t s) {
+                          void *d_hoist, hipStream_t s) {
     FwdArgs a;
     const bool wg2 = train && sv.wg2;
     if (wg2) save_x0 = true;
@@ -1105,7 +1318,10 @@
     const bool np2 = !train && pn_inference_products == 2;
     const bool mix = !wg2 && !np2 && (pn_mix_mask() & (train ? 2 : 1));
     using FwdKernel = void (*)(FwdArgs);
-    const FwdKernel kfn = wg2   ? (pers ? k_agg_forward<true, true, 3, true> : k_agg_forward<true, false, 3, true>)
+    const bool hoist = d_hoist && !wg2 && !mix && !pers && !save_x0 && pts->n > 0;
+    const FwdKernel kfn = hoist ? (train ? k_agg_forward<true, false, 3, false, true>
+                                         : np2 ? k_agg_forward<false, false, 2, false, true> : k_agg_forward<false, false, 3, false, true>)
+                        : wg2   ? (pers ? k_agg_forward<true, true, 3, true> : k_agg_forward<true, false, 3, true>)
                         : mix   ? (train ? (pers ? k_agg_forward<true, true, 4> : k_agg_forward<true, false, 4>)
                                          : (pers ? k_agg_forward<false, true, 4> : k_agg_forward<false, false, 4>))
                         : train ? (pers ? k_agg_forward<true, true, 3> : k_agg_forward<true, false, 3>)
@@ -1119,6 +1335,21 @@
     a.cls_list = sv.cls_list; a.cls_info = sv.cls_info; a.Kstride = K;
     int kc[PN_NCLS];
     const int ncls = pn_class_slots(K, kc);
+    a.rowslot = nullptr; a.y1p = nullptr;
+    if (hoist) {
+        HoistArgs h = {};
+        h.emb = pts->embedding; h.packed = a.packed; h.pidx = d_sample_pidx; h.valid_list = d_valid_list; h.counters = d_counters;
+        h.cls_list = sv.cls_list; h.cls_info = sv.cls_info; h.K = K; h.n_valid = (int)cap_samples; h.n_points = pts->n;
+        rc = pn_hoist_points(h, pn_hoist_carve(d_hoist, pts->n, cap_samples, K), np2 ? 2 : 3, ncu, s);
+        if (rc) return rc;
+        PnProfScope prof(PNK_POINT_LIST, s);
+        for (int j = 0; j < ncls; ++j) {
+            const int ts = pn_tile_samples(kc[j]);
+            const long long blocks = ((cap_samples + ts - 1) / ts * PN_TILE + 255) / 256;
+            hipLaunchKernelGGL(k_hoist_rowslot, dim3((unsigned)(blocks < 8192 ? (blocks > 0 ? blocks : 1) : 8192)), dim3(256), 0, s, h, j, kc[j], ts);
+        }
+        a.rowslot = h.rowslot; a.y1p = h.y1p;
+    }
     {
         PnProfScope prof(PNK_AGG_FWD, s);
         for (int j = 0; j < ncls; ++j) {
diff --git a/pointnerf_amd/csrc/pn_common.h b/pointnerf_amd/csrc/pn_common.h
--- a/pointnerf_amd/csrc/pn_common.h
+++ b/pointnerf_amd/csrc/pn_common.h
@@ -26,7 +26,7 @@
 };
 
 enum PnKernelId { PNK_GRID = 0, PNK_PROBE, PNK_NEIGHBORS, PNK_COMPACT, PNK_PACK, PNK_AGG_FWD, PNK_COLOR_FWD, PNK_RAYMARCH_FWD,
-                  PNK_RAYMARCH_BWD, PNK_COLOR_BWD, PNK_AGG_BWD, PNK_WGRAD, PNK_WGRAD_REDUCE, PNK_GATHER, PNK_ADAM, PNK_COUNT };
+                  PNK_RAYMARCH_BWD, PNK_COLOR_BWD, PNK_AGG_BWD, PNK_WGRAD, PNK_WGRAD_REDUCE, PNK_GATHER, PNK_ADAM, PNK_POINT_LIST, PNK_POINT_L1, PNK_COUNT };
 extern int pn_prof_enabled;
 void pn_prof_mark(int id, bool begin, hipStream_t s);
 struct PnProfScope {
diff --git a/pointnerf_amd/csrc/prof.hip b/pointnerf_amd/csrc/prof.hip
--- a/pointnerf_amd/csrc/prof.hip
+++ b/pointnerf_amd/csrc/prof.hip
@@ -15,7 +15,7 @@
 }
 const char *kNames[PNK_COUNT] = {"grid_build", "probe", "neighbors", "compact", "mlp_pack", "agg_forward", "color_forward",
                                  "raymarch_forward", "raymarch_backward", "color_backward", "agg_backward", "wgrad",
-                                 "wgrad_reduce", "gather", "adam"};
+                                 "wgrad_reduce", "gather", "adam", "point_list", "point_layer1"};
 }
 
 void pn_prof_mark(int id, bool begin, hipStream_t s) {
diff --git a/pointnerf_amd/csrc/render.hip b/pointnerf_amd/csrc/render.hip
--- a/pointnerf_amd/csrc/render.hip
+++ b/pointnerf_amd/csrc/render.hip
@@ -5,7 +5,7 @@
                           const int32_t *d_sample_pidx,
                           const int32_t *d_valid_list, const int32_t *d_counters, int R, int SR, int K,
                           float *d_decoded, float *d_weight, const PnSaved &sv, long long cap_samples, bool train, bool save_x0,
-                          hipStream_t s);
+                          void *d_hoist, hipStream_t s);
 int pn_agg_backward_launch(const pnerf_camera *cam, const pnerf_points *pts, const float *d_params, const void *d_packed,
                            const float *d_raydir, const float *d_sample_loc, const int32_t *d_sample_pidx,
                            const int32_t *d_valid_list, const int32_t *d_counters, int R, int SR, int K,
@@ -463,15 +463,17 @@
     return 0;
 }
 
-extern "C" int pnerf_render_forward(const pnerf_camera *cam, const pnerf_points *pts, const void *d_packed_mlp, const float *d_params,
-                                    const float *d_raydir, const float *d_sample_loc, const int32_t *d_sample_pidx,
-                                    const int32_t *d_sample_nn, const int32_t *d_valid_list, const int32_t *d_counters,
-                                    int R, int SR, int K,
-                                    float *d_decoded, float *d_weight, float *d_ray_color, float *d_opacity,
-                                    float *d_bg_trans, float *d_blend_w,
-                                    void *d_saved, int64_t n_valid_max, void *d_ws, size_t ws_bytes, void *stream) {
+extern "C" int pnerf_render_forward_hoisted(const pnerf_camera *cam, const pnerf_points *pts, const void *d_packed_mlp, const float *d_params,
+                                            const float *d_raydir, const float *d_sample_loc, const int32_t *d_sample_pidx,
+                                            const int32_t *d_sample_nn, const int32_t *d_valid_list, const int32_t *d_counters,
+                                            int R, int SR, int K,
+                                            float *d_decoded, float *d_weight, float *d_ray_color, float *d_opacity,
+                                            float *d_bg_trans, float *d_blend_w,
+                                            void *d_saved, int64_t n_valid_max, void *d_ws, size_t ws_bytes,
+                                            void *d_hoist, size_t hoist_bytes, void *stream) {
     int rc = check_common(cam, pts, R, SR, K);
     if (rc) return rc;
+    if (d_hoist && hoist_bytes < pnerf_hoist_bytes(pts->n, n_valid_max, K)) return PNERF_E_WS;
     if (!d_packed_mlp || !d_params || !d_raydir || !d_sample_loc || !d_sample_pidx || !d_sample_nn || !d_valid_list || !d_counters) return PNERF_E_INVAL;
     if (!d_decoded || !d_weight || !d_ray_color || !d_opacity || !d_bg_trans || !d_blend_w) return PNERF_E_INVAL;
     if (R == 0) return 0;
@@ -490,7 +492,7 @@
     if (hipMemsetAsync(d_weight, 0, (size_t)R * SR * K * sizeof(float), s) != hipSuccess) return PNERF_E_LAUNCH;
     if (n_valid_max > 0) {
         rc = pn_agg_forward_launch(cam, pts, d_params, d_packed_mlp, d_raydir, d_sample_loc, nullptr, nullptr, d_sample_pidx, d_valid_list, d_counters,
-                                   R, SR, K, d_decoded, d_weight, sv, n_valid_max, train, false, s);
+                                   R, SR, K, d_decoded, d_weight, sv, n_valid_max, train, false, d_hoist, s);
         if (rc) return rc;
     }
     RmArgs ra;
@@ -499,6 +501,18 @@
     hipLaunchKernelGGL(k_raymarch_forward, dim3(pn_cdiv(R, TPB / 64)), dim3(TPB), 0, s, ra, d_ray_color, d_opacity, d_bg_trans, d_blend_w, (float *)nullptr); }
     PN_CHECK_LAUNCH();
     return 0;
+}
+
+extern "C" int pnerf_render_forward(const pnerf_camera *cam, const pnerf_points *pts, const void *d_packed_mlp, const float *d_params,
+                                    const float *d_raydir, const float *d_sample_loc, const int32_t *d_sample_pidx,
+                                    const int32_t *d_sample_nn, const int32_t *d_valid_list, const int32_t *d_counters,
+                                    int R, int SR, int K,
+                                    float *d_decoded, float *d_weight, float *d_ray_color, float *d_opacity,
+                                    float *d_bg_trans, float *d_blend_w,
+                                    void *d_saved, int64_t n_valid_max, void *d_ws, size_t ws_bytes, void *stream) {
+    return pnerf_render_forward_hoisted(cam, pts, d_packed_mlp, d_params, d_raydir, d_sample_loc, d_sample_pidx, d_sample_nn, d_valid_list, d_counters,
+                                        R, SR, K, d_decoded, d_weight, d_ray_color, d_opacity, d_bg_trans, d_blend_w, d_saved, n_valid_max,
+                                        d_ws, ws_bytes, nullptr, 0, stream);
 }
 
 extern "C" int pnerf_render_backward(const pnerf_camera *cam, const pnerf_points *pts, const void *d_packed_mlp, const float *d_params,
@@ -572,7 +586,7 @@
     if (hipMemsetAsync(d_weight, 0, (size_t)R * SR * K * sizeof(float), s) != hipSuccess) return PNERF_E_LAUNCH;
     if (n_valid_max == 0) return 0;
     return pn_agg_forward_launch(cam, pts, d_params, d_packed_mlp, d_raydir, d_sample_loc, d_xyz_pers, d_loc_pers, d_sample_pidx,
-                                 d_valid_list, d_counters, R, SR, K, d_decoded, d_weight, sv, n_valid_max, train, train, s);
+                                 d_valid_list, d_counters, R, SR, K, d_decoded, d_weight, sv, n_valid_max, train, train, nullptr, s);
 }
 
 extern "C" int pnerf_agg_backward(const pnerf_camera *cam, const pnerf_points *pts, const void *d_packed_mlp, const float *d_params,
diff --git a/pointnerf_amd/ops.py b/pointnerf_amd/ops.py
--- a/pointnerf_amd/ops.py
+++ b/pointnerf_amd/ops.py
@@ -280,6 +280,18 @@
     del t
 
 
+_HOIST = {}
+
+
+def hoist_scratch(nbytes, device):
+    t = _HOIST.get(device)
+    if t is None or t.numel() < nbytes:
+        _HOIST.pop(device, None)
+        t = None
+        t = _HOIST[device] = torch.empty(int(nbytes * 1.15) + 256, dtype=torch.uint8, device=device)
+    return t
+
+
 def render_forward(cam, pts, packed, flat, raydir, dense, R, SR, K, n_valid, train):
     dev = raydir.device
     lib = L.lib()
@@ -294,11 +306,13 @@
     else:
         nws = lib.pnerf_agg_workspace_bytes(n_valid, K)
         ws = torch.empty(nws, dtype=torch.uint8, device=dev)
-    L.check(lib.pnerf_render_forward(ctypes.byref(cam), ctypes.byref(pts), _ptr(packed), _ptr(flat), _ptr(raydir),
-                                     _ptr(dense["sample_loc"]), _ptr(dense["sample_pidx"]), _ptr(dense["sample_nn"]),
-                                     _ptr(dense["valid_list"]), _ptr(dense["counters"]), R, SR, K,
-                                     _ptr(decoded), _ptr(weight), _ptr(ray_color), _ptr(opacity), _ptr(bg_trans), _ptr(blend_w),
-                                     _ptr(saved), n_valid, _ptr(ws), nws, _stream()), "pnerf_render_forward")
+    nh = lib.pnerf_hoist_bytes(int(pts.n), n_valid, K)
+    hoist = hoist_scratch(nh, dev)
+    L.check(lib.pnerf_render_forward_hoisted(ctypes.byref(cam), ctypes.byref(pts), _ptr(packed), _ptr(flat), _ptr(raydir),
+                                             _ptr(dense["sample_loc"]), _ptr(dense["sample_pidx"]), _ptr(dense["sample_nn"]),
+                                             _ptr(dense["valid_list"]), _ptr(dense["counters"]), R, SR, K,
+                                             _ptr(decoded), _ptr(weight), _ptr(ray_color), _ptr(opacity), _ptr(bg_trans), _ptr(blend_w),
+                                             _ptr(saved), n_valid, _ptr(ws), nws, _ptr(hoist), nh, _stream()), "pnerf_render_forward_hoisted")
     return dict(decoded=decoded, weight=weight, ray_color=ray_color, opacity=opacity, bg_trans=bg_trans,
                 blend_w=blend_w, saved=saved)
 
```

Result: no change. 2.102 million (-0.0%).
